# MathThyMod/GP_emu_UQSA

Hardware: AMD Instinct MI355X
Metric: log-marginal-likelihood evals/sec at n=16384 d=10 fp64; 1/2/4/8 GPU (higher is better)
Workload: dtype f64

## Files before the change

gp_emu_uqsa_amd/csrc/gpemu.hip:

```cpp
#include <hip/hip_runtime.h>

#include <algorithm>
#include <array>
#include <atomic>
#include <map>
#include <cmath>
#include <cstdio>
#include <cstdlib>
#include <cstring>
#include <limits>
#include <string>
#include <type_traits>
#include <utility>
#include <vector>

#include "../../include/gpemu.h"
#include "gpemu_kernels.hpp"
#include "gpemu_gemm_sched.hpp"
#include "gpemu_chol_sched.hpp"
#include "gpemu_objective.hpp"
#include "gpemu_chunk_pipe.hpp"
#include "gpemu_tiny.hpp"
#include "gpemu_snb.hpp"
#include "gpemu_ozaki.hpp"
#include "gpemu_pivchol.hpp"
#include "gpemu_imse.hpp"
#include "gpemu_postgrad.hpp"
#include "gpemu_postmean.hpp"
#include "gpemu_postmean_multi.hpp"
#include "gpemu_postgroup.hpp"
#include "gpemu_hm.hpp"
#include "gpemu_host_alloc.hpp"

using namespace gpe;

namespace {

thread_local std::string g_create_error;

constexpr int MAX_PROBS = 1 << 16;
constexpr int AUX_DESC_BASE = 1 << 15;
constexpr int ADHOC_DESC_BASE = MAX_PROBS - 64;

enum AdhocSlot {
  ADHOC_POST_V = ADHOC_DESC_BASE + 0,
  ADHOC_COV = ADHOC_DESC_BASE + 1,
  ADHOC_NOISE = ADHOC_DESC_BASE + 3,
  ADHOC_PIVCHOL = ADHOC_DESC_BASE + 4,
  ADHOC_POST_U = ADHOC_DESC_BASE + 5,
  ADHOC_IMSE = ADHOC_DESC_BASE + 7,
  ADHOC_TEST = ADHOC_DESC_BASE + 8,
  ADHOC_BENCH = ADHOC_DESC_BASE + 16,
};

constexpr int OZ_CHOL_MIN = 8192;
constexpr int OZ_CHOL_NEST_MIN = 12288;


struct Fact {
  long long n_pad = 0;
  int NB = 0;
  double* A = nullptr;
  double* B = nullptr;
  size_t cap = 0;
  double* logdet = nullptr;
  int* flags = nullptr;
  int* tflags = nullptr;
  bool aug = false;
  double* Faug = nullptr;
  double* part = nullptr;
  int* tcnt = nullptr;
  bool xdone[2] = {false, false};
  int xh = 0;
  int x11 = 0;
  bool t_ahead = false;
  void xclear(int h = 0) { xdone[0] = xdone[1] = t_ahead = false; x11 = 0; xh = h; }
  int desc_base = 0;
  Plan plan;
};

}

struct gpe_ctx {
  int device = 0;
  hipStream_t stream = nullptr;
  std::string err;

  long long n = 0, n_pad = 0;
  int d = 0, q = 0, NB = 0;
  bool has_r = false;

  double* dX = nullptr;
  double* dXw = nullptr;
  double* dF = nullptr;
  double* dr = nullptr;
  Fact tr;
  Fact aux;

  int* dinfo = nullptr;
  double* dinvdelta = nullptr;
  double* dZ = nullptr;
  double* dR2 = nullptr;
  double* dWa = nullptr;
  double* dskp = nullptr;
  size_t skp_cap = 0;
  double* dgpart = nullptr;
  double* dgram = nullptr;
  double* dT2 = nullptr;
  double* dcpart = nullptr;
  size_t cpart_cap = 0;
  size_t invd_cap = 0, csum_cap = 0, gram_cap = 0, t2_cap = 0;
  double* dcsum = nullptr;
  GemmProb* dprobs = nullptr;
  unsigned* dtiles = nullptr;
  size_t tiles_cap = 0;

  double* dW1 = nullptr;
  double* dW2 = nullptr;
  size_t w1_cap = 0, w2_cap = 0;
  double* dW3 = nullptr;
  size_t w3_cap = 0;
  double* dXs = nullptr;
  double* dXsw = nullptr;
  size_t xs_cap = 0, xsw_cap = 0;
  double* dsmall = nullptr;
  double* dtiny = nullptr;
  int tiny_ek = 0, tiny_eg = 0;
  bool tiny_dirty = true;
  double* dsnb = nullptr;
  long long snb_np = 0;
  int snb_hc = 0, snb_mf = 0;
  bool snb_dirty = true;
  double onel_tag = 0.0;
  int oz_on = 1, oz_nmod = OZ_MAXMOD;
  int oz_min_np = 6144;
  int oz_np2 = 0, oz_list_len = 0;
  long long oz_npad = 0;
  OzConst oz_c{};
  int8_t* dozp = nullptr;
  int8_t* dozr = nullptr;
  int* dozx = nullptr;
  unsigned* dozl = nullptr;
  double* dozt = nullptr;
  hipEvent_t ev_oz = nullptr;
  std::vector<OzTriPair> oz_tri;
  int oz_tri_min = 8192;
  double oz_lauum_ops = 0.0;
  int oz_chol = 1, oz_chol_min = OZ_CHOL_MIN;
  int tri_ahead_on = 1;
  hipEvent_t ev_l11 = nullptr, ev_schur = nullptr;
  OzTriPair oz_chol_q{};
  long long oz_chol_loff = 0;
  int oz_chol_llen = 0;
  double oz_chol_ops = 0.0;
  bool oz_chol_ready = false;
  int oz_nest = 1, oz_nest_min = OZ_CHOL_NEST_MIN;
  OzCholNest oz_nest_q{};
  long long oz_nest_loff = 0;
  int oz_nest_llen = 0;
  double oz_nest_ops = 0.0;
  bool oz_nest_ready = false;
  bool oz_l21_valid = false;
  std::vector<hipEvent_t> oev;
  size_t oev_used = 0;
  double oz_ms = 0.0, oz_launches = 0.0, oz_ops = 0.0, oz_flops64 = 0.0;
  int dbg_skip_wait = -1;
  size_t small_cap = 0;

  double* hpin = nullptr;
  size_t hpin_cap = 0;

  float* dX32 = nullptr;
  size_t x32_cap = 0;
  bool x32_valid = false;
  float* dK32 = nullptr;
  size_t k32_cap = 0;
  hipEvent_t ev_pipe[2] = {nullptr, nullptr};
  int8_t* dpxp = nullptr;
  int* dpxe = nullptr;
  int8_t* dpkp = nullptr;
  int* dpke = nullptr;
  int8_t* dpres = nullptr;
  unsigned* dpl = nullptr;
  size_t pxp_cap = 0, pxe_cap = 0, pkp_cap = 0, pke_cap = 0, pres_cap = 0, pl_cap = 0;
  int px_nmod = 0, pl_nti = 0, pl_ntj = 0, pl_len = 0;
  bool px_valid = false;

  double* dSU = nullptr;
  double* dSZ = nullptr;
  double* dSW = nullptr;
  double* dSpart = nullptr;
  double* dSout = nullptr;
  size_t su_cap = 0, sz_cap = 0, sw_cap = 0, spart_cap = 0, sout_cap = 0;

  double* dRn = nullptr;
  size_t rn_cap = 0;
  double* dVall = nullptr;
  double* dXall = nullptr;
  double* dTall = nullptr;
  size_t vall_cap = 0, xall_cap = 0, tall_cap = 0;
  double* dNU = nullptr;
  size_t nu_cap = 0;
  double* dPc = nullptr;
  double* dPcL = nullptr;
  size_t pc_cap = 0, pcl_cap = 0;
  double* dIm = nullptr;
  double* dImC = nullptr;
  size_t im_cap = 0, imc_cap = 0;
  double* dPg = nullptr;
  size_t pg_cap = 0;
  double* dPm = nullptr;
  size_t pm_cap = 0;
  long long mean_chunk = 65536;
  int mo_p = 0;
  double* dFm = nullptr;
  double* dZm = nullptr;
  double* dR2m = nullptr;
  double* dWm = nullptr;
  size_t fm_cap = 0, zm_cap = 0, r2m_cap = 0, wm_cap = 0;
  double* dPmm = nullptr;
  size_t pmm_cap = 0;
  double* dPgc = nullptr;
  size_t pgc_cap = 0;

// ... 517 lines not shown
  if (P <= SK_PMAX)
    hipLaunchKernelGGL(k_apply_small, g, dim3(256), 0, c->stream, Z, ldz, P, T, Pout, Y, ldy, nrows, abort_flag);
  else
    hipLaunchKernelGGL(k_apply_big, g, dim3(256), 0, c->stream, Z, ldz, P, T, Pout, Y, ldy, nrows, abort_flag);
  HIPCHK(c, hipGetLastError());
  return GPE_OK;
}

inline int gram_pairs(int P) {
  const int nch = (P + SK_PMAX - 1) / SK_PMAX;
  return nch * (nch + 1) / 2;
}

int gram(gpe_ctx* c, const double* Z, long long ldz, int P, int nrows, double* host_out) {
  const int nblk = (nrows + 255) / 256;
  const size_t need = (size_t)nblk * P * P;
  CHK(ensure_small(c, need + P * P));
  hipLaunchKernelGGL(k_gram, dim3(nblk, gram_pairs(P)), dim3(256), 0, c->stream, Z, ldz, P, nrows, c->dsmall,
                     c->dinfo);
  HIPCHK(c, hipGetLastError());
  hipLaunchKernelGGL(k_reduce_rows, dim3(P * P), dim3(256), 0, c->stream, c->dsmall, nblk, P * P,
                     c->dgram);
  HIPCHK(c, hipGetLastError());
  CHK(ensure_pinned(c, (size_t)P * P + 8));
  HIPCHK(c, hipMemcpyAsync(c->hpin, c->dgram, (size_t)P * P * sizeof(double), hipMemcpyDeviceToHost,
                           c->stream));
  HIPCHK(c, hipStreamSynchronize(c->stream));
  std::memcpy(host_out, c->hpin, (size_t)P * P * sizeof(double));
  return GPE_OK;
}

int gram_async(gpe_ctx* c, const double* Z, long long ldz, int P, int nrows) {
  const int nblk = (nrows + 255) / 256;
  const size_t need = (size_t)nblk * P * P;
  CHK(ensure_small(c, need + P * P));
  hipLaunchKernelGGL(k_gram, dim3(nblk, gram_pairs(P)), dim3(256), 0, c->stream, Z, ldz, P, nrows, c->dsmall,
                     c->dinfo);
  HIPCHK(c, hipGetLastError());
  hipLaunchKernelGGL(k_reduce_rows, dim3(P * P), dim3(256), 0, c->stream, c->dsmall, nblk, P * P,
                     c->dgram);
  HIPCHK(c, hipGetLastError());
  HIPCHK(c, hipMemcpyAsync(c->hpin, c->dgram, (size_t)P * P * sizeof(double), hipMemcpyDeviceToHost,
                           c->stream));
  return GPE_OK;
}

int read_info_logdet(gpe_ctx* c, const Fact& F, int* info, double* logdetA) {
  CHK(ensure_pinned(c, (size_t)F.NB + 8));
  HIPCHK(c, hipMemcpyAsync(c->hpin, F.logdet, F.NB * sizeof(double), hipMemcpyDeviceToHost, c->stream));
  HIPCHK(c, hipMemcpyAsync(c->hpin + F.NB, c->dinfo, sizeof(int), hipMemcpyDeviceToHost, c->stream));
  HIPCHK(c, hipStreamSynchronize(c->stream));
  std::memcpy(info, c->hpin + F.NB, sizeof(int));
  if (*info == GEMM_WAIT_TIMEOUT)
    return fail(c, GPE_ERR_HIP, "internal error: Cholesky panel wait timed out");
  double s = 0.0;
  for (int k = 0; k < F.NB; ++k) s += c->hpin[k];
  *logdetA = 2.0 * s;
  return GPE_OK;
}

int check_ready(gpe_ctx* c) {
  if (!c) return GPE_ERR_ARG;
  if (c->n <= 0) return fail(c, GPE_ERR_STATE, "gpe_set_data has not been called");
  HIPCHK(c, hipSetDevice(c->device));
  return GPE_OK;
}

void ev_rec(gpe_ctx* c, int i) {
  if (c->prof) hipEventRecord(c->ev[i], c->stream);
}

struct Cols {
  const double* F;
  int P;
  double* Z;
};
int z_from_factor(gpe_ctx* c, const Cols* cols = nullptr, bool cols_in_aug = false);
int trsv_lower(gpe_ctx* c, Fact& F, const double* R, long long ldr, int P, double* Y, long long ldy);

int factor_and_invert(gpe_ctx* c, int kernel, const double* delta, double nu, double s2,
                      double rscale, bool invert = true, bool objective = false, const Cols* cols = nullptr) {
  c->linv_valid = false;
  c->oz_l21_valid = false;
  HIPCHK(c, hipStreamSynchronize(c->stream2));
  HIPCHK(c, hipMemsetAsync(c->dinfo, 0, sizeof(int), c->stream));
  CHK(build_plan(c, c->tr));
  ev_rec(c, 0);
  CHK(scale_training(c, delta));
  CHK(kbuild(c, kernel, nu, s2, rscale));
  const int P = cols ? cols->P : c->q + 1;
  const bool aug = !invert && c->tr.plan.aug && P <= TILE;
  c->zaug_valid = aug && !cols;
  if (aug) {
    const long long tot = c->n_pad * TILE;
    hipLaunchKernelGGL(k_aug_init, dim3((unsigned)((tot + 255) / 256)), dim3(256), 0, c->stream,
                       cols ? cols->F : c->dF, c->n_pad, P, c->n_pad, c->tr.Faug);
    HIPCHK(c, hipGetLastError());
  }
  ev_rec(c, 1);
  CHK(build_plan(c, c->tr));
  CHK(potrf(c, c->tr, aug, objective && (invert || c->oz_chol >= 2), objective && invert,
            objective && (invert || c->oz_chol == 3)));
  if (kernel_fam(kernel) != FAM_GAUSS) {
    double coff, cdiag;
    kernel_consts(kernel, nu, true, &coff, &cdiag);
    const double floor_rel = 4.0 * (double)c->n_pad * std::numeric_limits<double>::epsilon();
    const double* r = (c->has_r && rscale != 0.0) ? c->dr : nullptr;
    hipLaunchKernelGGL(k_pivot_floor, dim3((unsigned)((c->n + 255) / 256)), dim3(256), 0, c->stream, c->tr.A,
                       c->n_pad, (int)c->n, floor_rel, s2 * cdiag, r, rscale, c->dinfo);
    HIPCHK(c, hipGetLastError());
  }
  ev_rec(c, 2);
  if (invert) {
    CHK(trtri(c, c->tr, true));
    c->linv_valid = true;
  }
  CHK(z_from_factor(c, cols, aug));
  ev_rec(c, 3);
  return GPE_OK;
}

int z_from_factor(gpe_ctx* c, const Cols* cols, bool cols_in_aug) {
  const int P = cols ? cols->P : c->q + 1;
  const double* F = cols ? cols->F : c->dF;
  double* Z = cols ? cols->Z : c->dZ;
  const long long np = c->n_pad;
  if (cols ? cols_in_aug : c->zaug_valid) {
    const long long tot = np * P;
    hipLaunchKernelGGL(k_aug_to_cols, dim3((unsigned)((tot + 255) / 256)), dim3(256), 0, c->stream,
                       c->tr.Faug, P, np, Z, np);
    HIPCHK(c, hipGetLastError());
    return GPE_OK;
  }
  if (c->linv_valid) return skinny(c, false, c->tr.B, np, c->NB, c->NB, true, F, np, P, Z, np);
  return trsv_lower(c, c->tr, F, np, P, Z, np);
}

int ensure_linv(gpe_ctx* c) {
  if (c->linv_valid) return GPE_OK;
  CHK(trtri(c, c->tr));
  c->linv_valid = true;
  c->x32_valid = false;
  c->px_valid = false;
  return GPE_OK;
}

int trsv_lower(gpe_ctx* c, Fact& F, const double* R, long long ldr, int P, double* Y, long long ldy) {
  CHK(ensure_xdiag(c, F));
  for (int c0 = 0; c0 < P; c0 += TS_PM) {
    const int pc = std::min(TS_PM, P - c0);
    HIPCHK(c, hipMemsetAsync(F.tflags, 0, 2 * sizeof(int), c->stream));
    hipLaunchKernelGGL(k_trsv_lower, dim3(F.NB), dim3(512), 0, c->stream, F.A, (long long)F.n_pad, F.B,
                       R + (long long)c0 * ldr, ldr, Y + (long long)c0 * ldy, ldy, pc, F.tflags, F.tflags + 1,
                       c->dinfo);
    HIPCHK(c, hipGetLastError());
  }
  return GPE_OK;
}

constexpr int OZ_MIN_NP = 6144, OZ_POST_MIN_NP = 4096, OZ_MAX_NP = 65536, OZ_POST_MAX_NP = 32768;
static_assert(OZ_MAX_NP % OZ_T == 0 && OZ_MAX_NP <= OZ_MAX_K && OZ_POST_MAX_NP <= OZ_MAX_K, "int8 sums too long");
bool oz_use(const gpe_ctx* c) { return c->oz_on && c->n_pad >= c->oz_min_np && c->n_pad <= OZ_MAX_NP; }

int oz_chol_split(const gpe_ctx* c, const Fact& F) {
  if (!c->oz_chol || !oz_use(c) || F.n_pad != c->n_pad || F.NB < 2) return 0;
  int h = 1;
  while (2 * h < F.NB) h *= 2;
  return (F.NB - h) * TILE >= c->oz_chol_min ? h : 0;
}

int oz_chol_nest_split(const gpe_ctx* c, const Fact& F, int h) {
  if (!c->oz_nest || h < 4 || (h / 2) % 2) return 0;
  return (F.NB - h / 2) * TILE >= c->oz_nest_min ? h / 2 : 0;
}

bool oz_tri_level(const gpe_ctx* c, const std::vector<std::array<int, 3>>& prs) {
  return oz_use(c) && !prs.empty() && (prs[0][1] - prs[0][0]) * TILE >= c->oz_tri_min;
}

int oz_prepare(gpe_ctx* c, Fact& F) {
  const int np2 = (int)(((c->n_pad + OZ_T - 1) / OZ_T) * OZ_T);
  if (c->n_pad == c->oz_npad && np2 == c->oz_np2 && c->oz_c.nmod == c->oz_nmod) return GPE_OK;
  c->oz_np2 = 0;
  c->oz_npad = 0;
  c->oz_chol_ready = false;
  c->oz_nest_ready = false;
  c->oz_l21_valid = false;
  CHK(build_plan(c, F));
  const int N = c->oz_nmod;
  size_t planes = (size_t)oz_plane_bytes(np2) * N;
  size_t resid = (size_t)oz_lauum_shape(np2).res_bytes() * N;
  size_t scratch = 0, nex = (size_t)np2;
  std::vector<unsigned> all = oz_lauum_shape(np2).list();
  c->oz_list_len = (int)all.size();
  c->oz_lauum_ops = oz_lauum_shape(np2).ops(N);
  c->oz_tri.clear();
  for (const auto& prs : F.plan.tri_pairs) {
    if (!oz_tri_level(c, prs)) continue;
    for (const auto& pr : prs) {
      const OzTriPair q = oz_tri_pair_plan(pr[0], pr[1], pr[2], N, all);
      planes = std::max(planes, q.planes_bytes(N));
      resid = std::max(resid, q.resid_bytes(N));
      scratch = std::max(scratch, (size_t)q.Pa * q.Pb);
      nex = std::max(nex, (size_t)(q.Pa + q.Pb));
      c->oz_tri.push_back(q);
    }
  }
  if (const int hs = (&F == &c->tr) ? F.plan.split_h : 0) {
    const OzTriPair* have = nullptr;
    for (const OzTriPair& q : c->oz_tri)
      if (q.t0 == 0 && q.h == hs && q.t1 == F.NB) have = &q;
    const OzTriPair q = have ? *have : oz_tri_pair_plan(0, hs, F.NB, N, all);
    const std::vector<unsigned> ls = q.shape_schur().list();
    c->oz_chol_q = q;
    c->oz_chol_loff = (long long)all.size();
    c->oz_chol_llen = (int)ls.size();
    all.insert(all.end(), ls.begin(), ls.end());
    c->oz_chol_ops = q.shape_schur().ops(N);
    planes = std::max(planes, (size_t)N * q.Pb * q.Pa);
    resid = std::max(resid, (size_t)q.shape_schur().res_bytes() * N);
    nex = std::max(nex, (size_t)q.Pb);
    c->oz_chol_ready = true;
    if (const int qs = F.plan.split_q) {
      const OzCholNest nq = oz_chol_nest_plan(qs, hs, F.NB);
      const std::vector<unsigned> ln = nq.shape().list();
      c->oz_nest_q = nq;
      c->oz_nest_loff = (long long)all.size();
      c->oz_nest_llen = (int)ln.size();
      all.insert(all.end(), ln.begin(), ln.end());
      c->oz_nest_ops = nq.shape().ops(N);
      planes = std::max(planes, nq.planes_bytes(N));
      resid = std::max(resid, nq.resid_bytes(N));
      nex = std::max(nex, (size_t)nq.Pb);
      c->oz_nest_ready = true;
    }
  }
  CHK(dalloc(c, &c->dozp, planes));
  CHK(dalloc(c, &c->dozr, resid));
  CHK(dalloc(c, &c->dozx, nex));
  CHK(dalloc(c, &c->dozt, scratch));
  CHK(dalloc(c, &c->dozl, all.size()));
  HIPCHK(c, hipMemcpy(c->dozl, all.data(), all.size() * sizeof(unsigned), hipMemcpyHostToDevice));
  c->oz_c = oz_consts(N, np2);
  c->oz_np2 = np2;
  c->oz_npad = c->n_pad;
  return GPE_OK;
}

int oz_gemm_crt(gpe_ctx* c, const OzConst& k, const OzProduct& p, double ops, double flops64,
                hipStream_t st = nullptr) {
  if (!st) st = c->stream;
  hipEvent_t e0 = nullptr, e1 = nullptr;
  if (c->prof) {
    while (c->oev_used + 2 > c->oev.size()) {
      hipEvent_t e;
      HIPCHK(c, hipEventCreate(&e));
      c->oev.push_back(e);
    }
    e0 = c->oev[c->oev_used];
    e1 = c->oev[c->oev_used + 1];
  }
  HIPCHK(c, oz_product_launch(st, k, p, e0, e1));
  if (c->prof) {
    c->oev_used += 2;
    c->oz_launches += 1.0;
    c->oz_ops += ops;
    c->oz_flops64 += flops64;
  }
  return GPE_OK;
}

int chol_schur(gpe_ctx* c, Fact& F, hipStream_t st, bool with_aug, int at) {
  const Plan& pl = F.plan;
  if (at != pl.split_h) {
    const OzCholNest& n = c->oz_nest_q;
    if (!c->oz_nest_ready || at != pl.split_q || n.q != at || n.h != pl.split_h)
      return fail(c, GPE_ERR_STATE, "internal error: nested split Cholesky without an int8 plan");
    if (with_aug) CHK(launch_gemm_range(c, pl.launches[pl.aug_q], st));
    const long long ld = F.n_pad;
    c->oz_l21_valid = false;
    oz_operand(st, c->oz_c, n.src(F.A + (long long)n.q * TILE, ld), n.Pb, n.K, c->dozx, c->dozp);
    HIPCHK(c, hipGetLastError());
    const OzShape s = n.shape();
    const OzOpnd l{c->dozp, (long long)n.Pb * n.K, n.K, 0};
    return oz_gemm_crt(c, c->oz_c,
                       OzProduct{s, l, l, c->dozl + c->oz_nest_loff, c->oz_nest_llen, c->dozr, s.res_bytes(),
                                 OzOut{c->dozx, c->dozx, F.A + (long long)n.q * TILE * (ld + 1), ld, n.Rb, n.cols, 1, -1.0, 1}},
                       c->oz_nest_ops, (double)n.cols * (2.0 * n.Rb - n.cols) * n.K, st);
  }
  const OzTriPair& q = c->oz_chol_q;
  if (!c->oz_chol_ready || q.h != pl.split_h) return fail(c, GPE_ERR_STATE, "internal error: split Cholesky without an int8 plan");
  if (with_aug) CHK(launch_gemm_range(c, pl.launches[pl.aug_mid], st));
  const long long ld = F.n_pad;
  oz_operand(st, c->oz_c, q.l21(F.A + (long long)q.h * TILE, ld), q.Pb, q.Pa, c->dozx, c->dozp);
  HIPCHK(c, hipGetLastError());
  const OzShape s = q.shape_schur();
  const OzOpnd l21{c->dozp, (long long)q.Pb * q.Pa, q.Pa, 0};
  CHK(oz_gemm_crt(c, c->oz_c,
                  OzProduct{s, l21, l21, c->dozl + c->oz_chol_loff, c->oz_chol_llen, c->dozr, s.res_bytes(),
                            OzOut{c->dozx, c->dozx, F.A + (long long)q.h * TILE * (ld + 1), ld, q.Rb, q.Rb, 1, -1.0, 1}},
                  c->oz_chol_ops, (double)q.Rb * q.Rb * q.Ra, st));
  c->oz_l21_valid = true;
  return GPE_OK;
}

int lauum_ozaki(gpe_ctx* c, Fact& F) {
  CHK(oz_prepare(c, F));
  const int np = (int)F.n_pad, np2 = c->oz_np2;
  c->oz_l21_valid = false;
  oz_operand_packed(c->stream, c->oz_c, F.B, (long long)F.n_pad, np, np2, c->dozx, c->dozp);
  const OzShape s = oz_lauum_shape(np2);
  const OzOpnd x{c->dozp, oz_plane_bytes(np2), 0, np2};
  return oz_gemm_crt(c, c->oz_c,
                     OzProduct{s, x, x, c->dozl, c->oz_list_len, c->dozr, s.res_bytes(),
                               OzOut{c->dozx, c->dozx, F.A, (long long)F.n_pad, np, np, 1, 1.0}},
                     c->oz_lauum_ops, (double)np * np * np / 3.0);
}

const OzTriPair* oz_pair(const gpe_ctx* c, int t0, int h, int t1) {
  for (const OzTriPair& q : c->oz_tri)
    if (q.t0 == t0 && q.h == h && q.t1 == t1) return &q;
  return nullptr;
}

int oz_l21(gpe_ctx* c, Fact& F, const OzTriPair& q, hipStream_t st) {
  c->oz_l21_valid = false;
  oz_operand(st, c->oz_c, q.l21(F.A + (long long)q.h * TILE + (long long)q.t0 * TILE * F.n_pad, F.n_pad), q.Pb, q.Pa,
             c->dozx, c->dozp);
  HIPCHK(c, hipGetLastError());
  return GPE_OK;
}

int oz_l21_ahead(gpe_ctx* c, Fact& F, int t0, int h, int t1) {
  CHK(oz_prepare(c, F));
  const OzTriPair* q = oz_pair(c, t0, h, t1);
  if (!q) return fail(c, GPE_ERR_STATE, "internal error: TRTRI pair without an int8 plan");
  if (!c->ev_oz) HIPCHK(c, hipEventCreateWithFlags(&c->ev_oz, hipEventDisableTiming));
  HIPCHK(c, hipEventRecord(c->ev_fork, c->stream));
  HIPCHK(c, hipStreamWaitEvent(c->stream2, c->ev_fork, 0));
  CHK(oz_l21(c, F, *q, c->stream2));
  HIPCHK(c, hipEventRecord(c->ev_oz, c->stream2));
  return GPE_OK;
}

int trtri_pair_ozaki(gpe_ctx* c, Fact& F, int t0, int h, int t1, int l21, int part) {
  CHK(oz_prepare(c, F));
  const OzTriPair* qp = oz_pair(c, t0, h, t1);
  if (!qp) return fail(c, GPE_ERR_STATE, "internal error: TRTRI pair without an int8 plan");
  const long long ld = F.n_pad;
  auto tile = [&](double* M, int i, int j) { return M + (long long)i * TILE + (long long)j * TILE * ld; };
  if (l21 == 1) HIPCHK(c, hipStreamWaitEvent(c->stream, c->ev_oz, 0));
  if (part != 1) c->oz_l21_valid = false;
  int rc = GPE_OK;
  oz_tri_pair_launches(c->stream, c->oz_c, *qp, c->dozl, tile(F.A, h, t0), tile(F.B, t0, t0), tile(F.B, h, h),
                       tile(F.B, h, t0), ld, c->dozt, c->dozp, c->dozr, c->dozx, l21 != 0,
                       [&](const OzProduct& p, double ops, double fl) {
                         if (rc == GPE_OK) rc = oz_gemm_crt(c, c->oz_c, p, ops, fl);
                       }, part);
  CHK(rc);
  HIPCHK(c, hipGetLastError());
  return GPE_OK;
}

}

bool create_priority_stream(hipStream_t* st) {
  int lo = 0, hi = 0;
  if (hipDeviceGetStreamPriorityRange(&lo, &hi) != hipSuccess) return false;
  return hipStreamCreateWithPriority(st, hipStreamNonBlocking, hi) == hipSuccess;
}

extern "C" {

#ifdef GEMM_TRACE
int gpe_debug_trace(uint64_t* out, int32_t n) {
  if (n > 8 * 4096) n = 8 * 4096;
  return hipMemcpyFromSymbol(out, HIP_SYMBOL(gemm_trace), (size_t)n * 8) == hipSuccess ? 0 : -2;
}
#endif

#ifdef GEMM_TTRACE
int gpe_debug_ttrace(uint64_t* out, int32_t n) {
  if (n > 8 * (int)GEMM_TTRACE_MAX) n = 8 * (int)GEMM_TTRACE_MAX;
  return hipMemcpyFromSymbol(out, HIP_SYMBOL(gemm_ttrace), (size_t)n * 8) == hipSuccess ? 0 : -2;
}
int gpe_debug_ttrace_count(int32_t reset) {
  unsigned n = 0;
  if (hipMemcpyFromSymbol(&n, HIP_SYMBOL(gemm_ttrace_n), sizeof(n)) != hipSuccess) return -2;
  if (reset) {
    const unsigned z = 0;
    if (hipMemcpyToSymbol(HIP_SYMBOL(gemm_ttrace_n), &z, sizeof(z)) != hipSuccess) return -2;
    void* tt = nullptr;
    if (hipGetSymbolAddress(&tt, HIP_SYMBOL(gemm_ttrace)) != hipSuccess ||
        hipMemset(tt, 0, sizeof(unsigned long long) * 8 * GEMM_TTRACE_MAX) != hipSuccess) return -2;
  }
  return (int)n;
}
#endif

int gpe_abi_version(void) { return GPE_ABI_VERSION; }

#ifndef GPE_SOURCE_HASH
#define GPE_SOURCE_HASH "unknown"
#endif
const char* gpe_build_id(void) { return GPE_SOURCE_HASH; }

int gpe_device_count(void) {
  int n = 0;
  if (hipGetDeviceCount(&n) != hipSuccess) return 0;
  return n;
}

int gpe_device_synchronize(int32_t device) {
  if (hipSetDevice(device) != hipSuccess) return GPE_ERR_HIP;
  return hipDeviceSynchronize() == hipSuccess ? GPE_OK : GPE_ERR_HIP;
}

gpe_ctx* gpe_create(int32_t device) {
  int ndev = 0;
  hipError_t e = hipGetDeviceCount(&ndev);
  if (e != hipSuccess || ndev <= 0) {
    g_create_error = std::string("no HIP device available: ") + hipGetErrorString(e);
    return nullptr;
  }
  if (device < 0 || device >= ndev) {
    g_create_error = "device index out of range";
    return nullptr;
  }
  gpe_ctx* c = new gpe_ctx();
  c->device = device;
  c->aux.desc_base = AUX_DESC_BASE;
  {
    const char* ea = std::getenv("GPEMU_AUG");
    c->tr.aug = !(ea && std::string(ea) == "0");
  }
  {
    const char* e2 = std::getenv("GPEMU_POTRF");
    if (e2) {
      const std::string m(e2);
      c->sched.group = m == "group" || m == "auto";
      c->potrf_mode = m == "group" ? 1 : (m == "auto" ? 0 : 2);
    }
    if (const char* eg = std::getenv("GPEMU_GROUP_P0")) c->sched.grp_p0 = std::max(1, std::atoi(eg));
    if (const char* eg = std::getenv("GPEMU_GROUP_STRIDE")) c->sched.grp_stride = std::max(0, std::atoi(eg));
    if (const char* ep = std::getenv("GPEMU_CHOL_PRIO")) c->chol_prio = std::atoi(ep) != 0;
    if (const char* et = std::getenv("GPEMU_TINY")) c->tiny = std::atoi(et) != 0;
    if (const char* ed = std::getenv("GPEMU_DEBUG_SKIP_WAIT")) c->dbg_skip_wait = std::atoi(ed);
    if (const char* em = std::getenv("GPEMU_MEAN_CHUNK")) c->mean_chunk = std::max(1, std::atoi(em) / 128) * 128LL;
    if (const char* eo = std::getenv("GPEMU_OZAKI")) c->oz_on = std::atoi(eo) != 0;
    if (const char* en = std::getenv("GPEMU_OZAKI_MIN_NP")) c->oz_min_np = std::max(512, std::atoi(en));
    if (const char* em = std::getenv("GPEMU_OZAKI_MODULI")) c->oz_nmod = std::max(8, std::min(OZ_MAXMOD, std::atoi(em)));
    if (const char* et = std::getenv("GPEMU_OZAKI_TRI_MIN")) c->oz_tri_min = std::max(512, std::atoi(et));
    if (const char* ec = std::getenv("GPEMU_OZAKI_CHOL")) c->oz_chol = std::max(0, std::min(3, std::atoi(ec)));
    if (const char* ec = std::getenv("GPEMU_OZAKI_CHOL_MIN")) c->oz_chol_min = std::max(256, std::atoi(ec));
    if (const char* ec = std::getenv("GPEMU_OZAKI_CHOL_NEST")) c->oz_nest = std::atoi(ec) != 0;
    if (const char* ec = std::getenv("GPEMU_OZAKI_CHOL_NEST_MIN")) c->oz_nest_min = std::max(256, std::atoi(ec));
    if (const char* ea = std::getenv("GPEMU_TRTRI_AHEAD")) c->tri_ahead_on = std::atoi(ea) != 0;
    if (const char* es = std::getenv("GPEMU_POTRF_SB")) {
      c->sched.sb = std::max(1, std::min(8, std::atoi(es)));
      if (const char* colon = std::strchr(es, ':')) c->sched.sb_min = std::max(0, std::atoi(colon + 1));
    }
    if (const char* e3 = std::getenv("GPEMU_POTRF_W")) {
      c->sched.groups.clear();
      std::string spec(e3);
      size_t pos = 0;
      while (pos < spec.size()) {
        size_t end = spec.find(',', pos);
        if (end == std::string::npos) end = spec.size();
        const std::string item = spec.substr(pos, end - pos);
        const size_t colon = item.find(':');
        const int w = std::atoi(item.substr(0, colon).c_str());
        const int lim = colon == std::string::npos ? 0 : std::atoi(item.substr(colon + 1).c_str());
        if (w >= 1 && w <= 8) c->sched.groups.push_back({w, lim});
        pos = end + 1;
      }
    }
  }
  if (hipSetDevice(device) != hipSuccess || hipStreamCreateWithFlags(&c->stream, hipStreamNonBlocking) != hipSuccess ||
      !create_priority_stream(&c->stream2) ||
      hipEventCreateWithFlags(&c->ev_fork, hipEventDisableTiming) != hipSuccess ||
      hipEventCreateWithFlags(&c->ev_join, hipEventDisableTiming) != hipSuccess ||
      hipEventCreateWithFlags(&c->ev_l11, hipEventDisableTiming) != hipSuccess ||
      hipEventCreateWithFlags(&c->ev_schur, hipEventDisableTiming) != hipSuccess ||
      hipEventCreateWithFlags(&c->ev_host, hipEventDisableTiming) != hipSuccess) {
    g_create_error = "failed to initialise device/stream";
    delete c;
    return nullptr;
  }
  bool ok = dalloc(c, &c->dinfo, 12) == GPE_OK && dalloc(c, &c->dprobs, MAX_PROBS) == GPE_OK &&
            ensure_shape_bufs(c, GPE_MAX_DIMS, GPE_MAX_COLS) == GPE_OK;
  for (int i = 0; i < 16 && ok; ++i) ok = hipEventCreate(&c->ev[i]) == hipSuccess;
  if (ok) {
    const int gl = G_LDS_DOUBLES * (int)sizeof(double);
    ok = hipFuncSetAttribute((const void*)k_gemm<false, false, false, true>, hipFuncAttributeMaxDynamicSharedMemorySize, gl) == hipSuccess &&
         hipFuncSetAttribute((const void*)k_gemm<true, false, false, true>, hipFuncAttributeMaxDynamicSharedMemorySize, gl) == hipSuccess &&
         hipFuncSetAttribute((const void*)k_gemm<true, true, false, true>, hipFuncAttributeMaxDynamicSharedMemorySize, gl) == hipSuccess &&
         hipFuncSetAttribute((const void*)k_gemm<false, true, false, true>, hipFuncAttributeMaxDynamicSharedMemorySize, gl) == hipSuccess &&
         hipFuncSetAttribute((const void*)k_gemm<false, false, true, true>, hipFuncAttributeMaxDynamicSharedMemorySize, gl) == hipSuccess &&
         hipFuncSetAttribute((const void*)k_gemm<false, false>, hipFuncAttributeMaxDynamicSharedMemorySize, gl) == hipSuccess &&
         hipFuncSetAttribute((const void*)k_gemm<true, false>, hipFuncAttributeMaxDynamicSharedMemorySize, gl) == hipSuccess &&
         hipFuncSetAttribute((const void*)k_gemm<true, true>, hipFuncAttributeMaxDynamicSharedMemorySize, gl) == hipSuccess &&
         hipFuncSetAttribute((const void*)k_gemm<false, true>, hipFuncAttributeMaxDynamicSharedMemorySize, gl) == hipSuccess &&
         hipFuncSetAttribute((const void*)k_gemm<false, false, true>, hipFuncAttributeMaxDynamicSharedMemorySize, gl) == hipSuccess &&
         hipFuncSetAttribute((const void*)k_xasm, hipFuncAttributeMaxDynamicSharedMemorySize,
                             (int)(DB_LDS_DOUBLES * sizeof(double))) == hipSuccess;
    const int tl = (G_LDS_LAUNCH_DOUBLES + 2 * TILE * TINY_ZP) * (int)sizeof(double);
    const RegWidths w;
    ok = ok && onel_lds_attr<FAM_GAUSS>(w, tl, SNB_LDS_DOUBLES * 8) && onel_lds_attr<FAM_MATERN32>(w, tl, SNB_LDS_DOUBLES * 8) &&
         onel_lds_attr<FAM_MATERN52>(w, tl, SNB_LDS_DOUBLES * 8);
    if (!ok) c->err = "hipFuncSetAttribute(max dynamic LDS) failed";
  }
  if (!ok) {
    g_create_error = c->err;
    gpe_destroy(c);
    return nullptr;
  }
  return c;
}

void gpe_destroy(gpe_ctx* c) {
  if (!c) return;
  (void)hipSetDevice(c->device);
  if (c->stream) hipStreamSynchronize(c->stream);
  double* bufs[] = {c->dSU, c->dSZ, c->dSW, c->dSpart, c->dSout,
                    c->dX, c->dXw, c->dF, c->dr, c->tr.A, c->tr.B, c->tr.logdet, c->aux.A, c->aux.B,
                    c->aux.logdet, c->dinvdelta, c->dZ,
                    c->dR2, c->dWa, c->dskp, c->dgpart, c->dgram, c->dT2, c->dcpart, c->dcsum,
                    c->dW1, c->dW2, c->dW3, c->dXs, c->dXsw, c->dsmall, c->dtiny, c->dsnb, c->dRn, c->dNU,
                    c->dVall, c->dXall, c->dTall, c->dPc, c->dPcL, c->dIm, c->dImC, c->dPg, c->dPm, c->dPgc,
                    c->dFm, c->dZm, c->dR2m, c->dWm, c->dPmm};
  for (double* b : bufs)
    if (b) hipFree(b);
  if (c->dinfo) hipFree(c->dinfo);
  if (c->dX32) hipFree(c->dX32);
  if (c->dK32) hipFree(c->dK32);
  for (void* b : {(void*)c->dpxp, (void*)c->dpxe, (void*)c->dpkp, (void*)c->dpke, (void*)c->dpres, (void*)c->dpl})
    if (b) hipFree(b);
  if (c->tr.flags) hipFree(c->tr.flags);
  if (c->aux.flags) hipFree(c->aux.flags);
  for (Fact* F : {&c->tr, &c->aux}) {
    if (F->part) hipFree(F->part);
    if (F->tcnt) hipFree(F->tcnt);
  }
  if (c->tr.tflags) hipFree(c->tr.tflags);
  if (c->dozp) hipFree(c->dozp);
  if (c->dozr) hipFree(c->dozr);
  if (c->dozx) hipFree(c->dozx);
  if (c->dozl) hipFree(c->dozl);
  if (c->dozt) hipFree(c->dozt);
  if (c->ev_oz) hipEventDestroy(c->ev_oz);
  for (hipEvent_t e : c->oev) hipEventDestroy(e);
  if (c->tr.Faug) hipFree(c->tr.Faug);
  if (c->aux.tflags) hipFree(c->aux.tflags);
  if (c->dprobs) hipFree(c->dprobs);
  if (c->dtiles) hipFree(c->dtiles);
  if (c->hpin) hipHostFree(c->hpin);
  for (auto& e : c->ev)
    if (e) hipEventDestroy(e);
  for (auto& e : c->gev) (void)hipEventDestroy(e);
  if (c->ev_fork) (void)hipEventDestroy(c->ev_fork);
  for (hipEvent_t e : c->ev_pipe)
    if (e) (void)hipEventDestroy(e);
  if (c->ev_join) (void)hipEventDestroy(c->ev_join);
  if (c->ev_l11) (void)hipEventDestroy(c->ev_l11);
  if (c->ev_schur) (void)hipEventDestroy(c->ev_schur);
  if (c->ev_host) (void)hipEventDestroy(c->ev_host);
  if (c->stream2) {
    (void)hipStreamSynchronize(c->stream2);
    (void)hipStreamDestroy(c->stream2);
  }
  if (c->stream) (void)hipStreamDestroy(c->stream);
  delete c;
}

const char* gpe_last_error(const gpe_ctx* c) {
  if (!c) return g_create_error.c_str();
  return c->err.c_str();
}

int gpe_set_data(gpe_ctx* c, int64_t n, int32_t d, int32_t q, const double* X, const double* f,
                 const double* H, const double* r) {
  if (!c) return GPE_ERR_ARG;
  if (n <= 0 || d <= 0 || q <= 0 || !X || !f || !H) return fail(c, GPE_ERR_ARG, "bad data arguments");
  if (n > (1LL << 20)) return fail(c, GPE_ERR_UNSUPPORTED, "n too large");
  HIPCHK(c, hipSetDevice(c->device));
  HIPCHK(c, hipStreamSynchronize(c->stream));
  CHK(ensure_shape_bufs(c, d, q + 1));
  const long long n_pad = ((n + TILE - 1) / TILE) * TILE;
  const bool resize = (n_pad != c->n_pad) || (d != c->d) || (q != c->q);
  c->n = n; c->d = d; c->q = q; c->n_pad = n_pad; c->NB = (int)(n_pad / TILE);
  c->mo_p = 0;
  c->factor_valid = false;
  c->ainv_valid = false;
  c->x32_valid = false;
  c->px_valid = false;
  c->zaug_valid = false;
  c->linv_valid = false;
  c->oz_l21_valid = false;
  if (resize) {
    CHK(ensure_fact(c, c->tr, n_pad));
    CHK(dalloc(c, &c->dX, (size_t)n_pad * d));
    CHK(dalloc(c, &c->dXw, (size_t)n_pad * d));
    CHK(dalloc(c, &c->dF, (size_t)n_pad * (q + 1)));
    CHK(dalloc(c, &c->dr, (size_t)n_pad));
    const size_t cols = (size_t)std::max(SK_PMAX, q + 1);
    CHK(dalloc(c, &c->dZ, (size_t)n_pad * cols));
    CHK(dalloc(c, &c->dR2, (size_t)n_pad * cols));
    CHK(dalloc(c, &c->dWa, (size_t)n_pad * cols));
    const size_t cp = (size_t)c->NB * (c->NB + 1) / 2 * (d + 3) * 4;
    CHK(dalloc(c, &c->dcpart, cp));
    c->cpart_cap = cp;
  }
  const size_t nx = (size_t)n_pad * d, nf = (size_t)n_pad * (q + 1);
  CHK(ensure_pinned(c, std::max(nx, nf) + n_pad));
  std::memset(c->hpin, 0, nx * sizeof(double));
  std::memcpy(c->hpin, X, (size_t)n * d * sizeof(double));
  HIPCHK(c, hipMemcpy(c->dX, c->hpin, nx * sizeof(double), hipMemcpyHostToDevice));
  std::memset(c->hpin, 0, nf * sizeof(double));
  for (long long i = 0; i < n; ++i) {
    c->hpin[i] = f[i];
    for (int p = 0; p < q; ++p) c->hpin[i + (long long)(p + 1) * n_pad] = H[i * q + p];
  }
  HIPCHK(c, hipMemcpy(c->dF, c->hpin, nf * sizeof(double), hipMemcpyHostToDevice));
  c->has_r = (r != nullptr);
  std::memset(c->hpin, 0, n_pad * sizeof(double));
  if (r) std::memcpy(c->hpin, r, (size_t)n * sizeof(double));
  HIPCHK(c, hipMemcpy(c->dr, c->hpin, n_pad * sizeof(double), hipMemcpyHostToDevice));
  return GPE_OK;
}

int gpe_set_profiling(gpe_ctx* c, int32_t on) {
  if (!c) return GPE_ERR_ARG;
  c->prof = on != 0;
  return GPE_OK;
}

int gpe_phase_times(gpe_ctx* c, double* ms_out, int32_t n) {
  if (!c || !ms_out) return GPE_ERR_ARG;
  for (int i = 0; i < n && i < 8; ++i) ms_out[i] = c->phase_ms[i];
  return GPE_OK;
}

int gpe_ozaki_stats(gpe_ctx* c, double* ms_out, double* launches_out, double* int8_ops_out, double* fp64_flops_out) {
  if (!c) return GPE_ERR_ARG;
  if (ms_out) *ms_out = c->oz_ms;
  if (launches_out) *launches_out = c->oz_launches;
  if (int8_ops_out) *int8_ops_out = c->oz_ops;
  if (fp64_flops_out) *fp64_flops_out = c->oz_flops64;
  return GPE_OK;
}

int gpe_gemm_stats(gpe_ctx* c, double* ms_out, double* launches_out, double* flops_out) {
  if (!c) return GPE_ERR_ARG;
  if (ms_out) *ms_out = c->gemm_ms;
  if (launches_out) *launches_out = c->gemm_launches;
  if (flops_out) *flops_out = c->gemm_flops;
  return GPE_OK;
}

}

namespace {

template <class Args>
int onel_prologue(gpe_ctx* c, const ObjArgs& o, int kernel, const double* hp, bool want_grad, size_t pinned, Args& a) {
  const int d = c->d;
  const int bad = inv_length_scales(hp, d, a.invd);
  if (bad >= 0) return fail(c, GPE_NOT_PD, bad_length_scale(bad));
  for (int k = d; k < TINY_DM; ++k) a.invd[k] = 0.0;
  c->linv_valid = false;
  c->zaug_valid = false;
  c->tr.xclear();
  HIPCHK(c, hipStreamSynchronize(c->stream2));
  CHK(ensure_pinned(c, pinned));
  a.X = c->dX; a.F = c->dF; a.xw = c->dXw; a.small = c->hpin;
  a.r = (c->has_r && o.rscale != 0.0) ? c->dr : nullptr;
  a.rdiag = (o.gp4ml && !kernel_alt(kernel) && c->has_r) ? c->dr : nullptr;
  a.n = (int)c->n; a.d = d; a.P = c->q + 1; a.want_grad = want_grad ? 1 : 0; a.mucm = o.gp4ml ? 0 : 1;
  a.s2 = o.s2; a.rscale = o.rscale;
  a.dbg_skip = c->dbg_skip_wait;
  a.tag = ++c->onel_tag;
  kernel_consts(kernel, o.nu, true, &a.coff, &a.cdiag);
  a.floor_rel = 4.0 * (double)c->n_pad * std::numeric_limits<double>::epsilon();
  return GPE_OK;
}

int onel_epilogue(gpe_ctx* c, const ObjArgs& o, int kernel, int n_hp, bool want_grad, const OneLaunchResult& r,
                  bool std_r, double* llh_out, double* grad_out, double* sigma2_out) {
  HIPCHK(c, hipGetLastError());
  HIPCHK(c, hipStreamSynchronize(c->stream));
  CHK(r.status(&c->err));
  const SmallAlgebra sa = small_from_gram(std::vector<double>(r.h, r.h + (size_t)r.P * r.P), r.P);
  if (!sa.ok) return fail(c, GPE_NOT_PD, Q_NOT_PD);
  const ObjValue v = objective_value(sa, r.logdetA(), (double)c->n, c->q, o.gp4ml, o.s2);
  *llh_out = v.llh;
  if (sigma2_out) *sigma2_out = v.sig2;
  if (want_grad) {
    if (r.q_refused()) return fail(c, GPE_NOT_PD, Q_NOT_PD);
    double red[TINY_DM + 3];
    CHK(r.sums(red, &c->err));
    objective_grad(red, r.d, kernel, o.nu, o.fitnug, o.gp4ml, v.gscale, o.s2, n_hp, grad_out, std_r);
  }
  if (c->prof) {
    ev_rec(c, 7);
    HIPCHK(c, hipStreamSynchronize(c->stream));
    float ms = 0.f;
    (void)hipEventElapsedTime(&ms, c->ev[0], c->ev[7]);
    for (int i = 0; i < 8; ++i) c->phase_ms[i] = 0.0;
    c->phase_ms[6] = ms;
  }
  return GPE_OK;
}

int tiny_objective(gpe_ctx* c, const ObjArgs& o, int kernel, const double* hp, int n_hp, bool want_grad,
                   double* llh_out, double* grad_out, double* sigma2_out) {
  const int d = c->d, P = c->q + 1;
  TinyArgs a;
  CHK(onel_prologue(c, o, kernel, hp, want_grad, (size_t)P * P + 2 * d + 64 + TINY_NH * 64, a));
  constexpr size_t tiny_doubles = 36 * DB_BS + TILE * 32;
  if (!c->dtiny) CHK(dalloc(c, &c->dtiny, tiny_doubles));
  if (c->tiny_dirty || c->tiny_ek > (1 << 26)) {
    HIPCHK(c, hipMemsetAsync(c->dinfo + 1, 0, (TINY_SYNC_INTS + 1) * sizeof(int), c->stream));
    c->tiny_ek = c->tiny_eg = 0;
    c->tiny_dirty = false;
  }
  ev_rec(c, 0);
  a.L = c->tr.A; a.Xo = c->tr.B; a.Z = c->dZ; a.abort_flag = c->dinfo + 1 + TINY_SYNC_INTS;
  a.K = c->tr.A; a.Xp = c->dtiny; a.Wg = c->dtiny + 36 * DB_BS; a.sync = c->dinfo + 1;
  a.ek = ++c->tiny_ek;
  a.eg = want_grad ? ++c->tiny_eg : c->tiny_eg;
  const size_t lds = (G_LDS_LAUNCH_DOUBLES + 2 * TILE * TINY_ZP) * sizeof(double);
  c->hpin[P * P + 1] = -2.0;
  c->tiny_dirty = true;
  with_fam(kernel_fam(kernel), [&](auto F) { launch_tiny_fam<decltype(F)::value>(d, lds, c->stream, a); });
  CHK(onel_epilogue(c, o, kernel, n_hp, want_grad, OneLaunchResult{c->hpin, P, d, 1, TINY_NH, a.tag, "k_tiny"},
                    a.rdiag != nullptr, llh_out, grad_out, sigma2_out));
  c->tiny_dirty = false;
  return GPE_OK;
}

int snb_objective(gpe_ctx* c, const ObjArgs& o, int kernel, const double* hp, int n_hp, bool want_grad,
                  double* llh_out, double* grad_out, double* sigma2_out) {
  const int d = c->d, P = c->q + 1, NB = c->NB;
  const long long np = c->n_pad;
  SnbArgs a;
  CHK(onel_prologue(c, o, kernel, hp, want_grad, (size_t)P * P + NB + 2 * d + 64 + SNB_NH * 64, a));
  if (c->snb_np != np) {
    c->snb_np = 0;
    CHK(dalloc(c, &c->dsnb, (size_t)np * np + 3 * 32 * (size_t)np + TINY_DM * TINY_ZP + TILE * TILE));
    c->snb_np = np;
  }
  if (c->snb_dirty || c->snb_hc > (1 << 24)) {
    HIPCHK(c, hipMemsetAsync(c->dinfo + 8, 0, (SNB_SYNC_INTS + 1) * sizeof(int), c->stream));
    c->snb_hc = c->snb_mf = 0;
    c->snb_dirty = false;
  }
  ev_rec(c, 0);
  a.A = c->tr.A; a.Lb = c->tr.B; a.Xt = c->dsnb;
  a.Zt = a.Xt + np * np; a.Zo = a.Zt + 32 * np; a.Wg = a.Zo + 32 * np; a.T2g = a.Wg + 32 * np;
  a.Xscr = a.T2g + TINY_DM * TINY_ZP;
  a.sync = c->dinfo + 8; a.abort_flag = c->dinfo + 8 + SNB_SYNC_INTS;
  a.np = (int)np; a.NB = NB;
  a.hcb = c->snb_hc; a.mfb = c->snb_mf;
  const size_t lds = SNB_LDS_DOUBLES * sizeof(double);
  c->hpin[P * P + NB] = -2.0;
  c->snb_dirty = true;
  with_fam(kernel_fam(kernel), [&](auto F) { launch_snb_fam<decltype(F)::value>(d, lds, c->stream, a); });
  CHK(onel_epilogue(c, o, kernel, n_hp, want_grad, OneLaunchResult{c->hpin, P, d, NB, SNB_NH, a.tag, "k_snb"},
                    a.rdiag != nullptr, llh_out, grad_out, sigma2_out));
  c->snb_hc += want_grad ? 4 * NB - 1 : 2 * NB;
  c->snb_mf += NB + (want_grad ? 1 : 0);
  c->snb_dirty = false;
  return GPE_OK;
}

int objective_phase_times(gpe_ctx* c) {
  if (!c->prof) return GPE_OK;
  HIPCHK(c, hipStreamSynchronize(c->stream));
  float ms;
  const int pairs[7][2] = {{0, 1}, {1, 2}, {2, 3}, {4, 5}, {3, 4}, {5, 7}, {0, 7}};
  for (int i = 0; i < 7; ++i) {
    ms = 0.f;
    (void)hipEventElapsedTime(&ms, c->ev[pairs[i][0]], c->ev[pairs[i][1]]);
    c->phase_ms[i] = ms;
  }
  double g = 0.0;
  for (size_t i = 0; i + 1 < c->gev_used; i += 2) {
    ms = 0.f;
    (void)hipEventElapsedTime(&ms, c->gev[i], c->gev[i + 1]);
    g += ms;
  }
  c->gemm_ms = g;
  g = 0.0;
  for (size_t i = 0; i + 1 < c->oev_used; i += 2) {
    ms = 0.f;
    (void)hipEventElapsedTime(&ms, c->oev[i], c->oev[i + 1]);
    g += ms;
  }
  c->oz_ms = g;
  return GPE_OK;
}

}

extern "C" {

int gpe_objective(gpe_ctx* c, int32_t variant, int32_t kernel, const double* hp, int32_t n_hp,
                  double nu_fixed, int32_t want_grad, double* llh_out, double* grad_out,
                  double* sigma2_out) {
  CHK(check_ready(c));
  const InflightGuard inflight(c->device);
  if (!hp || !llh_out) return fail(c, GPE_ERR_ARG, "null output");
  const int d = c->d, q = c->q;
  ObjArgs o;
  CHK(objective_args(variant, kernel, d, hp, n_hp, nu_fixed, &o, &c->err));
  if (!kernel_ok(kernel)) return fail(c, GPE_ERR_ARG, "bad kernel");
  if (want_grad && !grad_out) return fail(c, GPE_ERR_ARG, "grad_out is NULL");
  c->factor_valid = false;
  c->ainv_valid = false;
  c->x32_valid = false;
  c->px_valid = false;
  if (c->prof) {
    c->gev_used = 0;
    c->gemm_launches = c->gemm_flops = c->gemm_ms = 0.0;
    c->oev_used = 0;
    c->oz_ms = c->oz_launches = c->oz_ops = c->oz_flops64 = 0.0;
  }
  const bool one_launch = c->tiny;
  if (one_launch && c->NB == 1 && d <= TINY_DM && q + 1 <= TINY_DM)
    return tiny_objective(c, o, kernel, hp, n_hp, want_grad != 0, llh_out, grad_out, sigma2_out);
  if (one_launch && c->NB >= 2 && c->NB <= SNB_MAXNB && d <= TINY_DM && q + 1 <= TINY_DM)
    return snb_objective(c, o, kernel, hp, n_hp, want_grad != 0, llh_out, grad_out, sigma2_out);

  CHK(factor_and_invert(c, kernel, hp, o.nu, o.s2, o.rscale, want_grad != 0, true));
  const int P = q + 1;
  const long long np = c->n_pad;
  const int NBt = c->tr.NB;
  CHK(ensure_pinned(c, (size_t)P * P + NBt + 64));
  CHK(gram_async(c, c->dZ, np, P, (int)np));
  HIPCHK(c, hipMemcpyAsync(c->hpin + P * P, c->tr.logdet, NBt * sizeof(double), hipMemcpyDeviceToHost, c->stream));
  HIPCHK(c, hipMemcpyAsync(c->hpin + P * P + NBt, c->dinfo, sizeof(int), hipMemcpyDeviceToHost, c->stream));
  HIPCHK(c, hipEventRecord(c->ev_host, c->stream));
  ev_rec(c, 4);
  if (want_grad) CHK(oz_use(c) ? lauum_ozaki(c, c->tr) : lauum(c, c->tr));
  ev_rec(c, 5);
  HIPCHK(c, hipEventSynchronize(c->ev_host));
  std::vector<double> G(c->hpin, c->hpin + (size_t)P * P);
  int info = 0;
  std::memcpy(&info, c->hpin + P * P + NBt, sizeof(int));
  if (info == GEMM_WAIT_TIMEOUT) return fail(c, GPE_ERR_HIP, "internal error: Cholesky panel wait timed out");
  double logdetA = 0.0;
  for (int k = 0; k < NBt; ++k) logdetA += c->hpin[P * P + k];
  logdetA *= 2.0;
  if (info != 0) return fail(c, GPE_NOT_PD, not_pd_pivot(info));
  const SmallAlgebra sa = small_from_gram(G, P);
  if (!sa.ok) return fail(c, GPE_NOT_PD, Q_NOT_PD);
  const ObjValue v = objective_value(sa, logdetA, (double)c->n, q, o.gp4ml, o.s2);
  *llh_out = v.llh;
  if (sigma2_out) *sigma2_out = v.sig2;
  if (!want_grad) {
    ev_rec(c, 6);
    ev_rec(c, 7);
    goto done;
  }
  {
    CHK(ensure_pinned(c, (size_t)P * P + 8));
    const std::vector<double> T2 = small_t2(sa, q, v.cfac);
    std::memcpy(c->hpin, T2.data(), T2.size() * sizeof(double));
    HIPCHK(c, hipMemcpyAsync(c->dT2, c->hpin, T2.size() * sizeof(double), hipMemcpyHostToDevice, c->stream));
    CHK(apply_small(c, c->dZ, np, P, c->dT2, P, c->dR2, np, (int)np, c->dinfo));
    CHK(skinny(c, true, c->tr.B, np, c->NB, c->NB, true, c->dR2, np, P, c->dWa, np));
    ev_rec(c, 6);
    const double* rdiag = (o.gp4ml && !kernel_alt(kernel) && c->has_r) ? c->dr : nullptr;
    const int nblk = c->NB * (c->NB + 1) / 2;
    int cs = 1;
    if (!(d > 32 || P > 33))
      while (cs < 4 && nblk * cs * 2 <= 512) cs *= 2;
    const dim3 gc(nblk * cs);
    with_fam(kernel_fam(kernel), [&](auto F) { launch_contract<decltype(F)::value>(c, d, P, gc, nblk, rdiag, cs, c->dWa); });
    HIPCHK(c, hipGetLastError());
    hipLaunchKernelGGL(k_reduce_rows, dim3(d + 3), dim3(256), 0, c->stream, c->dcpart, nblk * cs, d + 3, c->dcsum);
    HIPCHK(c, hipGetLastError());
    ev_rec(c, 7);
    HIPCHK(c, hipMemcpyAsync(c->hpin, c->dcsum, (d + 3) * sizeof(double), hipMemcpyDeviceToHost, c->stream));
    HIPCHK(c, hipStreamSynchronize(c->stream));
    objective_grad(c->hpin, d, kernel, o.nu, o.fitnug, o.gp4ml, v.gscale, o.s2, n_hp, grad_out, rdiag != nullptr);
  }
done:
  return objective_phase_times(c);
}

int gpe_set_outputs(gpe_ctx* c, int32_t p, const double* F) {
  CHK(check_ready(c));
  const int q = c->q;
  const long long n = c->n, np = c->n_pad;
  if (p < 1 || p > PMM_MAXP || !F) return fail(c, GPE_ERR_ARG, "bad outputs (1 <= p <= 64, F not NULL)");
  if (n < (long long)p + q + 3) return fail(c, GPE_ERR_ARG, "p outputs need n >= p + q + 3 training points");
  HIPCHK(c, hipStreamSynchronize(c->stream));
  c->mo_p = 0;
  const int P = p + q;
  const size_t cols = (size_t)np * std::max(SK_PMAX, P);
  CHK(ensure_shape_bufs(c, c->d, P));
  CHK(grow_buf(c, &c->dFm, &c->fm_cap, (size_t)np * P));
  CHK(grow_buf(c, &c->dZm, &c->zm_cap, cols));
  CHK(grow_buf(c, &c->dR2m, &c->r2m_cap, cols));
  CHK(grow_buf(c, &c->dWm, &c->wm_cap, cols));
  const size_t nf = (size_t)np * p;
  CHK(ensure_pinned(c, nf));
  std::memset(c->hpin, 0, nf * sizeof(double));
  for (long long i = 0; i < n; ++i)
    for (int a = 0; a < p; ++a) c->hpin[i + (long long)a * np] = F[i * p + a];
  HIPCHK(c, hipMemcpy(c->dFm, c->hpin, nf * sizeof(double), hipMemcpyHostToDevice));
  HIPCHK(c, hipMemcpy(c->dFm + nf, c->dF + np, (size_t)np * q * sizeof(double), hipMemcpyDeviceToDevice));
  c->mo_p = p;
  return GPE_OK;
}

int gpe_objective_multi(gpe_ctx* c, int32_t kernel, const double* hp, int32_t n_hp, double nu_fixed,
                        int32_t want_grad, double* llh_out, double* grad_out, double* Sigma_out, double* B_out) {
  CHK(check_ready(c));
  if (!c->mo_p) return fail(c, GPE_ERR_STATE, "gpe_set_outputs has not been called for this data");
  const InflightGuard inflight(c->device);
  if (!hp || !llh_out || !Sigma_out) return fail(c, GPE_ERR_ARG, "null output");
  const int d = c->d, q = c->q, p = c->mo_p, P = p + q;
  ObjArgs o;
  CHK(objective_args(GPE_MUCM, kernel, d, hp, n_hp, nu_fixed, &o, &c->err));
  if (!kernel_ok(kernel)) return fail(c, GPE_ERR_ARG, "bad kernel");
  if (want_grad && !grad_out) return fail(c, GPE_ERR_ARG, "grad_out is NULL");
  c->factor_valid = false;
  c->ainv_valid = false;
  c->x32_valid = false;
  c->px_valid = false;
  if (c->prof) {
    c->gev_used = 0;
    c->gemm_launches = c->gemm_flops = c->gemm_ms = 0.0;
    c->oev_used = 0;
    c->oz_ms = c->oz_launches = c->oz_ops = c->oz_flops64 = 0.0;
  }
  const Cols cols{c->dFm, P, c->dZm};
  CHK(factor_and_invert(c, kernel, hp, o.nu, o.s2, o.rscale, want_grad != 0, true, &cols));
  const long long np = c->n_pad;
  const int NBt = c->tr.NB;
  CHK(ensure_pinned(c, (size_t)P * P + NBt + 64));
  CHK(gram_async(c, c->dZm, np, P, (int)np));
  HIPCHK(c, hipMemcpyAsync(c->hpin + P * P, c->tr.logdet, NBt * sizeof(double), hipMemcpyDeviceToHost, c->stream));
  HIPCHK(c, hipMemcpyAsync(c->hpin + P * P + NBt, c->dinfo, sizeof(int), hipMemcpyDeviceToHost, c->stream));
  HIPCHK(c, hipEventRecord(c->ev_host, c->stream));
  ev_rec(c, 4);
  if (want_grad) CHK(oz_use(c) ? lauum_ozaki(c, c->tr) : lauum(c, c->tr));
  ev_rec(c, 5);
  HIPCHK(c, hipEventSynchronize(c->ev_host));
  const std::vector<double> G(c->hpin, c->hpin + (size_t)P * P);
  int info = 0;
  std::memcpy(&info, c->hpin + P * P + NBt, sizeof(int));
  if (info == GEMM_WAIT_TIMEOUT) return fail(c, GPE_ERR_HIP, "internal error: Cholesky panel wait timed out");
  double logdetA = 0.0;
  for (int k = 0; k < NBt; ++k) logdetA += c->hpin[P * P + k];
  logdetA *= 2.0;
  if (info != 0) return fail(c, GPE_NOT_PD, not_pd_pivot(info));
  const SmallMulti sm = small_multi_from_gram(G, p, q);
  if (!sm.ok()) return fail(c, GPE_NOT_PD, sm.refused == 1 ? Q_NOT_PD : S_NOT_PD);
  const ObjValueMulti v = objective_value_multi(sm, logdetA, (double)c->n);
  *llh_out = v.llh;
  std::memcpy(Sigma_out, v.Sigma.data(), v.Sigma.size() * sizeof(double));
  if (B_out) std::memcpy(B_out, sm.B.data(), sm.B.size() * sizeof(double));
  if (!want_grad) {
    ev_rec(c, 6);
    ev_rec(c, 7);
    return objective_phase_times(c);
  }
  CHK(ensure_pinned(c, (size_t)P * P + 8));
  const std::vector<double> T2 = small_multi_t2(sm, v.cfac);
  std::memcpy(c->hpin, T2.data(), T2.size() * sizeof(double));
  HIPCHK(c, hipMemcpyAsync(c->dT2, c->hpin, T2.size() * sizeof(double), hipMemcpyHostToDevice, c->stream));
  CHK(apply_small(c, c->dZm, np, P, c->dT2, P, c->dR2m, np, (int)np, c->dinfo));
  CHK(skinny(c, true, c->tr.B, np, c->NB, c->NB, true, c->dR2m, np, P, c->dWm, np));
  ev_rec(c, 6);
  const int nblk = c->NB * (c->NB + 1) / 2;
  int cs = 1;
  if (!(d > 32 || P > 33))
    while (cs < 4 && nblk * cs * 2 <= 512) cs *= 2;
  const dim3 gc(nblk * cs);
  with_fam(kernel_fam(kernel),
           [&](auto F) { launch_contract<decltype(F)::value>(c, d, P, gc, nblk, nullptr, cs, c->dWm); });
  HIPCHK(c, hipGetLastError());
  hipLaunchKernelGGL(k_reduce_rows, dim3(d + 3), dim3(256), 0, c->stream, c->dcpart, nblk * cs, d + 3, c->dcsum);
  HIPCHK(c, hipGetLastError());
  ev_rec(c, 7);
  HIPCHK(c, hipMemcpyAsync(c->hpin, c->dcsum, (d + 3) * sizeof(double), hipMemcpyDeviceToHost, c->stream));
  HIPCHK(c, hipStreamSynchronize(c->stream));
  objective_grad(c->hpin, d, kernel, o.nu, o.fitnug, false, v.gscale, 1.0, n_hp, grad_out, false);
  return objective_phase_times(c);
}

int gpe_factor(gpe_ctx* c, int32_t kernel, const double* delta, double nu, double s2, double r_scale) {
  CHK(check_ready(c));
  if (!delta) return fail(c, GPE_ERR_ARG, "null delta");
  if (!kernel_ok(kernel)) return fail(c, GPE_ERR_ARG, "bad kernel");
  c->factor_valid = false;
  c->ainv_valid = false;
  c->x32_valid = false;
  c->px_valid = false;
  CHK(factor_and_invert(c, kernel, delta, nu, s2, r_scale, false, c->oz_chol == 3));
  int info = 0;
  double logdet = 0.0;
  CHK(read_info_logdet(c, c->tr, &info, &logdet));
  if (info != 0) return fail(c, GPE_NOT_PD, not_pd_pivot(info));
  c->factor_valid = true;
  c->x32_valid = false;
  c->px_valid = false;
  c->f_kernel = kernel;
  c->f_delta.assign(delta, delta + c->d);
  c->f_nu = nu;
  c->f_rscale = r_scale;
  return GPE_OK;
}

static int posterior_nmod(int np2, bool f32) {
  if (!f32) return OZ_MAXMOD;
  int bits = 24;
// ... 1509 lines not shown
  HIPCHK(c, hipMemcpy(F.A, c->hpin, tot * sizeof(double), hipMemcpyHostToDevice));
  HIPCHK(c, hipMemsetAsync(c->dinfo, 0, sizeof(int), c->stream));
  CHK(potrf(c, F));
  int info = 0;
  double logdet = 0.0;
  CHK(read_info_logdet(c, F, &info, &logdet));
  if (info != 0) return fail(c, GPE_NOT_PD, not_pd_pivot(info));
  if (logdet_out) *logdet_out = logdet;
  auto fetch_lower = [&](const double* dsrc, double* out, bool full_sym) -> int {
    HIPCHK(c, hipMemcpy(c->hpin, dsrc, tot * sizeof(double), hipMemcpyDeviceToHost));
    for (long long i = 0; i < m; ++i)
      for (long long j = 0; j < m; ++j) {
        double v;
        if (j <= i) v = c->hpin[i + j * mp];
        else v = full_sym ? c->hpin[j + i * mp] : 0.0;
        out[i * m + j] = v;
      }
    return GPE_OK;
  };
  if (L_out) CHK(fetch_lower(F.A, L_out, false));
  if (Linv_out || Ainv_out) {
    CHK(trtri(c, F));
    if (Linv_out) {
      HIPCHK(c, hipStreamSynchronize(c->stream));
      CHK(fetch_lower(F.B, Linv_out, false));
    }
    if (Ainv_out) {
      CHK(lauum(c, F));
      HIPCHK(c, hipStreamSynchronize(c->stream));
      CHK(fetch_lower(F.A, Ainv_out, true));
    }
  }
  HIPCHK(c, hipStreamSynchronize(c->stream));
  return GPE_OK;
}

int gpe_test_gemm(gpe_ctx* c, int32_t trans_a, int32_t trans_b, int64_t M, int64_t N, int64_t K,
                  const double* A, const double* B, double* C, double alpha, double beta) {
  if (!c) return GPE_ERR_ARG;
  if (M <= 0 || N <= 0 || K <= 0 || M % TILE || N % TILE || K % GK || !A || !B || !C)
    return fail(c, GPE_ERR_ARG, "gpe_test_gemm: M, N must be multiples of 128 and K of 16");
  HIPCHK(c, hipSetDevice(c->device));
  double *da = nullptr, *db = nullptr, *dc = nullptr;
  int rc = dalloc(c, &da, (size_t)M * K);
  if (rc == GPE_OK) rc = dalloc(c, &db, (size_t)K * N);
  if (rc == GPE_OK) rc = dalloc(c, &dc, (size_t)M * N);
  if (rc == GPE_OK) {
    std::vector<double> ha((size_t)M * K), hb((size_t)K * N), hc((size_t)M * N);
    long long lda, ldb;
    if (trans_a) { for (long long m = 0; m < M; ++m) for (long long k = 0; k < K; ++k) ha[k + m * K] = A[m * K + k]; lda = K; }
    else { for (long long m = 0; m < M; ++m) for (long long k = 0; k < K; ++k) ha[m + k * M] = A[m * K + k]; lda = M; }
    if (trans_b) { for (long long k = 0; k < K; ++k) for (long long n = 0; n < N; ++n) hb[k + n * K] = B[k * N + n]; ldb = K; }
    else { for (long long k = 0; k < K; ++k) for (long long n = 0; n < N; ++n) hb[n + k * N] = B[k * N + n]; ldb = N; }
    for (long long m = 0; m < M; ++m) for (long long n = 0; n < N; ++n) hc[m + n * M] = C[m * N + n];
    copy_checked(c, rc, da, ha.data(), ha.size() * sizeof(double), hipMemcpyHostToDevice);
    copy_checked(c, rc, db, hb.data(), hb.size() * sizeof(double), hipMemcpyHostToDevice);
    copy_checked(c, rc, dc, hc.data(), hc.size() * sizeof(double), hipMemcpyHostToDevice);
    const GemmProb p = mkprob(da, lda, db, ldb, dc, M, (int)(M / TILE), (int)(N / TILE), (int)K, 0, alpha, beta);
    const GemmKind kind = gemm_kind(trans_a != 0, trans_b != 0);
    GemmLaunch L{};
    if (rc == GPE_OK) rc = adhoc_gemm(c, ADHOC_TEST, {{kind, p}}, &L, true);
    HIPCHK(c, hipMemsetAsync(c->dinfo, 0, sizeof(int), c->stream));
    if (rc == GPE_OK) rc = launch_gemm_range(c, L);
    if (rc == GPE_OK) {
      hipError_t e = hipStreamSynchronize(c->stream);
      if (e != hipSuccess) rc = fail(c, GPE_ERR_HIP, hipGetErrorString(e));
    }
    if (rc == GPE_OK) {
      copy_checked(c, rc, hc.data(), dc, hc.size() * sizeof(double), hipMemcpyDeviceToHost);
      for (long long m = 0; m < M; ++m) for (long long n = 0; n < N; ++n) C[m * N + n] = hc[m + n * M];
    }
  }
  if (da) (void)hipFree(da);
  if (db) (void)hipFree(db);
  if (dc) (void)hipFree(dc);
  return rc;
}

struct OzTestBufs {
  double *sa = nullptr, *sb = nullptr, *C = nullptr;
  int *exa = nullptr, *exb = nullptr;
  int8_t *pa = nullptr, *pb = nullptr, *res = nullptr;
  unsigned* list = nullptr;
  ~OzTestBufs() {
    for (void* p : {(void*)sa, (void*)sb, (void*)C, (void*)exa, (void*)exb, (void*)pa, (void*)pb, (void*)res, (void*)list})
      if (p) (void)hipFree(p);
  }
};

static long long oz_test_extent(const gpe_oz_operand& o, int R, int Kv) {
  if (!o.src || o.len <= 0 || o.offset < 0 || o.ld < 1 || R < 1 || Kv < 1) return 0;
  const long long ext = o.trans ? (long long)(Kv - 1) * o.ld + R : (long long)(R - 1) * o.ld + Kv;
  return ext <= o.len - o.offset ? ext : 0;
}

static int oz_test_operand(gpe_ctx* c, const gpe_oz_operand& o, const OzConst& k, int P, int Kp, double** dsrc, int** dex,
                           int8_t** dpl) {
  CHK(dalloc(c, dsrc, (size_t)o.len));
  CHK(dalloc(c, dex, (size_t)P));
  CHK(dalloc(c, dpl, (size_t)k.nmod * P * Kp));
  HIPCHK(c, hipMemcpy(*dsrc, o.src, (size_t)o.len * sizeof(double), hipMemcpyHostToDevice));
  oz_operand(c->stream, k, OzSrc{*dsrc + o.offset, (long long)o.ld, o.R, o.Kv, o.mask, o.trans != 0}, P, Kp, *dex, *dpl);
  HIPCHK(c, hipGetLastError());
  return GPE_OK;
}

static int oz_test_product(gpe_ctx* c, const gpe_oz_operand& a, const gpe_oz_operand* b, gpe_oz_params p, double* C,
                           int32_t* exa_out, int32_t* exb_out, int8_t* res_out) {
  const auto bad = [&](const char* what) { return fail(c, GPE_ERR_ARG, std::string("gpe_test_oz_product: ") + what); };
  if (p.nmod < 6 || p.nmod > OZ_MAXMOD) return bad("nmod outside [6, 16]");
  if (res_out && (p.res_mod < 0 || p.res_mod >= p.nmod)) return bad("res_mod is not a modulus number");
  if (a.R < 1 || a.R > (1 << 20)) return bad("bad operand rows");
  const int Pa = (a.R + OZ_T - 1) / OZ_T * OZ_T;
  int Pb = Pa;
  if (p.packed) {
    if (a.R % TILE || (a.offset & 1) || (a.ld & 1) || a.ld < a.R || !oz_test_extent(a, 1, 1) ||
        (long long)(a.R - 1) * a.ld + a.R > a.len - a.offset)
      return bad("packed: X is R x R, R a multiple of 128, ld >= R and offset even, inside src");
    p.K = Pa; p.kbeg = 1; p.kend = 0; p.kdiv = 1; p.ti0 = 0; p.tri = 1; p.lower128 = 1;
    p.rows = p.cols = a.R;
    b = nullptr;
  } else {
    if (p.K < OZ_SK || p.K % OZ_SK || p.K > OZ_MAX_K) return bad("K is not a multiple of 64 in [64, 2^17 - 128]");
    if (a.mask < 0 || a.mask > 2 || a.Kv > p.K || !oz_test_extent(a, a.R, a.Kv)) return bad("operand A outside its source");
    if (b) {
      if (b->R < 1 || b->R > (1 << 20) || b->mask < 0 || b->mask > 2 || b->Kv > p.K || !oz_test_extent(*b, b->R, b->Kv))
        return bad("operand B outside its source");
      Pb = (b->R + OZ_T - 1) / OZ_T * OZ_T;
    }
    if (p.kbeg < 0 || p.kbeg > 3 || p.kend < 0 || p.kend > 1 || p.kdiv < 1) return bad("bad kbeg / kend / kdiv");
    if (p.ti0 < 0 || p.ti0 >= Pa / OZ_T) return bad("ti0 past the last tile row");
    if (p.tri && Pb < Pa && p.ti0 != 0) return bad("tri: B has fewer tile rows than A and ti0 > 0");
  }
  if (p.rows <= OZ_T * p.ti0 || p.rows > Pa || p.cols < 1 || p.cols > Pb) return bad("rows / cols outside the product");
  if (!C || p.ldc < 1 || p.c_len < 1 || (long long)(p.rows - 1 - OZ_T * p.ti0) + (long long)(p.cols - 1) * p.ldc >= p.c_len)
    return bad("C too small for rows x cols at ldc");
  const int K = p.K, ti0 = p.ti0, nti = Pa / OZ_T - ti0, ntj = Pb / OZ_T;
  const OzConst k = oz_consts(p.nmod, K);
  const OzShape s{nti, p.tri ? (Pb < Pa ? ntj : 0) : ntj, ti0, p.tri ? 1 : 0, K, p.kbeg, p.kend, p.kdiv};
  OzTestBufs d;
  hipStream_t st = c->stream;
  OzOpnd oa, ob;
  if (p.packed) {
    CHK(dalloc(c, &d.sa, (size_t)a.len));
    CHK(dalloc(c, &d.exa, (size_t)Pa));
    CHK(dalloc(c, &d.pa, (size_t)k.nmod * oz_plane_bytes(Pa)));
    HIPCHK(c, hipMemcpy(d.sa, a.src, (size_t)a.len * sizeof(double), hipMemcpyHostToDevice));
    oz_operand_packed(st, k, d.sa + a.offset, (long long)a.ld, a.R, Pa, d.exa, d.pa);
    HIPCHK(c, hipGetLastError());
    oa = ob = OzOpnd{d.pa, oz_plane_bytes(Pa), 0, Pa};
  } else {
    CHK(oz_test_operand(c, a, k, Pa, K, &d.sa, &d.exa, &d.pa));
    oa = ob = OzOpnd{d.pa, (long long)Pa * K, K, 0};
    if (b) {
      CHK(oz_test_operand(c, *b, k, Pb, K, &d.sb, &d.exb, &d.pb));
      ob = OzOpnd{d.pb, (long long)Pb * K, K, 0};
    }
  }
  const std::vector<unsigned> list = s.list();
  const long long rb = s.res_bytes();
  CHK(dalloc(c, &d.list, list.size()));
  CHK(dalloc(c, &d.res, (size_t)k.nmod * rb));
  CHK(dalloc(c, &d.C, (size_t)p.c_len));
  HIPCHK(c, hipMemcpy(d.list, list.data(), list.size() * sizeof(unsigned), hipMemcpyHostToDevice));
  HIPCHK(c, hipMemcpy(d.C, C, (size_t)p.c_len * sizeof(double), hipMemcpyHostToDevice));
  HIPCHK(c, hipMemsetAsync(d.res, 0, (size_t)k.nmod * rb, st));
  const OzOut out{d.exa, b ? d.exb : d.exa, d.C, (long long)p.ldc, p.rows, p.cols, p.lower128 ? 1 : 0, p.alpha, p.acc ? 1 : 0};
  CHK(oz_gemm_crt(c, k, OzProduct{s, oa, ob, d.list, (int)list.size(), d.res, rb, out}, 0.0, 0.0));
  HIPCHK(c, hipStreamSynchronize(st));
  HIPCHK(c, hipMemcpy(C, d.C, (size_t)p.c_len * sizeof(double), hipMemcpyDeviceToHost));
  if (exa_out) HIPCHK(c, hipMemcpy(exa_out, d.exa, (size_t)Pa * sizeof(int), hipMemcpyDeviceToHost));
  if (exb_out) HIPCHK(c, hipMemcpy(exb_out, b ? d.exb : d.exa, (size_t)Pb * sizeof(int), hipMemcpyDeviceToHost));
  if (res_out) {
    std::vector<int8_t> h((size_t)rb);
    HIPCHK(c, hipMemcpy(h.data(), d.res + (long long)p.res_mod * rb, (size_t)rb, hipMemcpyDeviceToHost));
    std::memset(res_out, 0, (size_t)nti * OZ_T * Pb);
    for (const unsigned ent : list) {
      if (ent == 0xffffffffu) continue;
      const int ti = (int)(ent >> 16), tj = (int)(ent & 0xffffu);
      const int8_t* t = h.data() + s.res_tile(ti, tj) * (OZ_T * OZ_T);
      for (int u = 0; u < OZ_T * OZ_T / 16; ++u) {
        const int wave = u >> 10, blk = (u >> 6) & 15, lane = u & 63;
        const long long gm = OZ_T * (ti - ti0) + (wave >> 1) * 128 + 32 * (blk >> 2) + (lane & 31);
        const long long gn0 = OZ_T * tj + (wave & 1) * 128 + 32 * (blk & 3) + 4 * (lane >> 5);
        for (int q = 0; q < 16; ++q) res_out[gm * Pb + gn0 + (q & 3) + 8 * (q >> 2)] = t[(long long)u * 16 + q];
      }
    }
  }
  return GPE_OK;
}

int gpe_test_oz_product(gpe_ctx* c, const gpe_oz_operand* a, const gpe_oz_operand* b, const gpe_oz_params* p, double* C,
                        int32_t* exa_out, int32_t* exb_out, int8_t* res_out) {
  if (!c) return GPE_ERR_ARG;
  if (!a || !p) return fail(c, GPE_ERR_ARG, "gpe_test_oz_product: NULL operand or parameters");
  HIPCHK(c, hipSetDevice(c->device));
  const bool prof = c->prof;
  c->prof = false;
  const int rc = oz_test_product(c, *a, b, *p, C, exa_out, exb_out, res_out);
  c->prof = prof;
  return rc;
}

static int oz_test_planes(gpe_ctx* c, const gpe_oz_operand& a, int packed, int K, int nmod, int32_t* ex_out, int8_t* planes_out) {
  const auto bad = [&](const char* what) { return fail(c, GPE_ERR_ARG, std::string("gpe_test_oz_planes: ") + what); };
  if (nmod < 6 || nmod > OZ_MAXMOD) return bad("nmod outside [6, 16]");
  if (a.R < 1 || a.R > (1 << 20)) return bad("bad operand rows");
  if (!ex_out || !planes_out) return bad("NULL output");
  const int P = (a.R + OZ_T - 1) / OZ_T * OZ_T;
  if (packed) {
    if (a.R % TILE || (a.offset & 1) || (a.ld & 1) || a.ld < a.R || !oz_test_extent(a, 1, 1) ||
        (long long)(a.R - 1) * a.ld + a.R > a.len - a.offset)
      return bad("packed: X is R x R, R a multiple of 128, ld >= R and offset even, inside src");
    K = P;
  } else {
    if (K < OZ_SK || K % OZ_SK || K > OZ_MAX_K) return bad("K is not a multiple of 64 in [64, 2^17 - 128]");
    if (a.mask < 0 || a.mask > 2 || a.Kv > K || !oz_test_extent(a, a.R, a.Kv)) return bad("operand outside its source");
  }
  const OzConst k = oz_consts(nmod, K);
  OzTestBufs d;
  if (packed) {
    const long long pb = oz_plane_bytes(P);
    CHK(dalloc(c, &d.sa, (size_t)a.len));
    CHK(dalloc(c, &d.exa, (size_t)P));
    CHK(dalloc(c, &d.pa, (size_t)nmod * pb));
    HIPCHK(c, hipMemcpy(d.sa, a.src, (size_t)a.len * sizeof(double), hipMemcpyHostToDevice));
    HIPCHK(c, hipMemsetAsync(d.pa, 0x55, (size_t)nmod * pb, c->stream));
    oz_operand_packed(c->stream, k, d.sa + a.offset, (long long)a.ld, a.R, P, d.exa, d.pa);
    HIPCHK(c, hipGetLastError());
    HIPCHK(c, hipStreamSynchronize(c->stream));
    std::vector<int8_t> h((size_t)nmod * pb);
    HIPCHK(c, hipMemcpy(h.data(), d.pa, h.size(), hipMemcpyDeviceToHost));
    std::memset(planes_out, 0, (size_t)nmod * P * P);
    for (int l = 0; l < nmod; ++l)
      for (int j = 0; j < P; ++j) {
        const int r0 = j / OZ_T * OZ_T;
        std::memcpy(planes_out + ((size_t)l * P + j) * P + r0,
                    h.data() + (size_t)l * pb + oz_panel_off(j / OZ_T, P) + (long long)(j - r0) * (P - r0), (size_t)(P - r0));
      }
  } else {
    CHK(dalloc(c, &d.sa, (size_t)a.len));
    CHK(dalloc(c, &d.exa, (size_t)P));
    CHK(dalloc(c, &d.pa, (size_t)nmod * P * K));
    HIPCHK(c, hipMemcpy(d.sa, a.src, (size_t)a.len * sizeof(double), hipMemcpyHostToDevice));
    HIPCHK(c, hipMemsetAsync(d.pa, 0x55, (size_t)nmod * P * K, c->stream));
    oz_operand(c->stream, k, OzSrc{d.sa + a.offset, (long long)a.ld, a.R, a.Kv, a.mask, a.trans != 0}, P, K, d.exa, d.pa);
    HIPCHK(c, hipGetLastError());
    HIPCHK(c, hipStreamSynchronize(c->stream));
    HIPCHK(c, hipMemcpy(planes_out, d.pa, (size_t)nmod * P * K, hipMemcpyDeviceToHost));
  }
  HIPCHK(c, hipMemcpy(ex_out, d.exa, (size_t)P * sizeof(int), hipMemcpyDeviceToHost));
  return GPE_OK;
}

int gpe_test_oz_planes(gpe_ctx* c, const gpe_oz_operand* a, int32_t packed, int32_t K, int32_t nmod, int32_t* ex_out,
                       int8_t* planes_out) {
  if (!c) return GPE_ERR_ARG;
  if (!a) return fail(c, GPE_ERR_ARG, "gpe_test_oz_planes: NULL operand");
  HIPCHK(c, hipSetDevice(c->device));
  return oz_test_planes(c, *a, packed, K, nmod, ex_out, planes_out);
}

struct GemmGroupBufs {
  gpe_ctx* c;
  GemmProb* ctx_probs;
  unsigned* ctx_tiles;
  bool prof;
  std::vector<double*> dev, keep;
  GemmProb* probs = nullptr;
  unsigned* tiles = nullptr;
  double* part = nullptr;
  int* tcnt = nullptr;
  explicit GemmGroupBufs(gpe_ctx* ctx) : c(ctx), ctx_probs(ctx->dprobs), ctx_tiles(ctx->dtiles), prof(ctx->prof) {}
  ~GemmGroupBufs() {
    c->dprobs = ctx_probs;
    c->dtiles = ctx_tiles;
    c->prof = prof;
    for (double* p : dev) if (p) (void)hipFree(p);
    for (double* p : keep) if (p) (void)hipFree(p);
    for (void* p : {(void*)probs, (void*)tiles, (void*)part, (void*)tcnt}) if (p) (void)hipFree(p);
  }
};
// ... 445 lines not shown
```

gp_emu_uqsa_amd/csrc/gpemu_ozaki.hpp:

```cpp
#pragma once
#include <algorithm>
#include <array>
#include <cmath>
#include <cstdlib>
#include <cstring>
#include <type_traits>
#include <utility>
#include <vector>

namespace gpe {

constexpr int OZ_T = 256;
constexpr int OZ_SK = 64;
constexpr int OZ_NBUF = 4;
constexpr int OZ_OPND = OZ_T * OZ_SK;
constexpr int OZ_LDS = OZ_NBUF * 2 * OZ_OPND;
constexpr int OZ_MAXMOD = 16;
constexpr int OZ_MAX_K = (1 << 17) - 128;

struct OzConst {
  int m[OZ_MAXMOD];
  int c16[OZ_MAXMOD];
  float inv[OZ_MAXMOD];
  int wlo[OZ_MAXMOD];
  int whi[OZ_MAXMOD];
  double rhi[OZ_MAXMOD];
  double rlo[OZ_MAXMOD];
  double Md;
  int nmod;
  int beta;
};

typedef int oz_v4i __attribute__((ext_vector_type(4)));
typedef int oz_v16i __attribute__((ext_vector_type(16)));

constexpr int OZ_EX_NAN = -(1 << 20), OZ_IL_BAD = 1 << 29;
__device__ __forceinline__ double oz_pmax(double a, double b) { return (a > b || a != a) ? a : b; }
__device__ __forceinline__ int oz_ex_of(double mx, int beta) {
  return !(mx <= 1.7976931348623157e308) ? OZ_EX_NAN : (mx > 0.0 ? (beta - 1) - ilogb(mx) : 0);
}

__host__ __device__ __forceinline__ long long oz_panel_off(int cb, int np2) {
  return (long long)OZ_T * ((long long)cb * np2 - (long long)OZ_T * cb * (cb - 1) / 2);
}
__host__ __device__ __forceinline__ long long oz_plane_bytes(int np2) { return oz_panel_off(np2 / OZ_T, np2); }

struct OzDigits {
  int lo, hi;
};
__host__ __device__ __forceinline__ OzDigits oz_digits(double x) {
  const unsigned long long c = 0x0080808080808080ull;
  const unsigned long long b = ((unsigned long long)(long long)x + c) ^ c;
  return OzDigits{(int)(unsigned)b, (int)(unsigned)(b >> 32)};
}
__host__ __device__ __forceinline__ int oz_dot4(int a, int b, int c) {
#if __HIP_DEVICE_COMPILE__
  return __builtin_amdgcn_sdot4(a, b, c, false);
#else
  for (int i = 0; i < 4; ++i) c += (int)(int8_t)((unsigned)a >> (8 * i)) * (int)(int8_t)((unsigned)b >> (8 * i));
  return c;
#endif
}
__host__ __device__ __forceinline__ int oz_mul24(int a, int b) {
#if __HIP_DEVICE_COMPILE__
  return __mul24(a, b);
#else
  const int a24 = (int)((unsigned)a << 8) >> 8, b24 = (int)((unsigned)b << 8) >> 8;
  return (int)((unsigned)a24 * (unsigned)b24);
#endif
}
__host__ __device__ __forceinline__ int oz_float_bits(float f) {
#if __HIP_DEVICE_COMPILE__
  return __float_as_int(f);
#else
  int i;
  std::memcpy(&i, &f, sizeof i);
  return i;
#endif
}
__host__ __device__ __forceinline__ int oz_digit_sum(OzDigits d, int wlo, int whi) {
  return oz_dot4(d.lo, wlo, oz_dot4(d.hi, whi, 0));
}
__host__ __device__ __forceinline__ unsigned oz_reduce(int t, float inv, int nm) {
#pragma clang fp contract(off)
  const float qf = (float)t * inv + 12582912.0f;
  return (unsigned)(oz_mul24(oz_float_bits(qf), nm) + t);
}
__host__ __device__ __forceinline__ unsigned oz_pack4(unsigned v0, unsigned v1, unsigned v2, unsigned v3) {
#if __HIP_DEVICE_COMPILE__
  return __builtin_amdgcn_perm(__builtin_amdgcn_perm(v3, v2, 0x0c0c0400u), __builtin_amdgcn_perm(v1, v0, 0x0c0c0400u),
                               0x05040100u);
#else
  return (v0 & 0xffu) | (v1 & 0xffu) << 8 | (v2 & 0xffu) << 16 | v3 << 24;
#endif
}
__host__ __device__ inline void oz_residues(double x, const OzConst& cst, int8_t* out) {
  const OzDigits d = oz_digits(x);
  for (int l = 0; l < cst.nmod; ++l)
    out[l] = (int8_t)(oz_reduce(oz_digit_sum(d, cst.wlo[l], cst.whi[l]), cst.inv[l], -cst.m[l]) & 0xffu);
}
__host__ __device__ __forceinline__ uint2 oz_residues8(const OzDigits (&d)[8], const OzConst& cst, int l) {
  const int wlo = cst.wlo[l], whi = cst.whi[l], nm = -cst.m[l];
  const float inv = cst.inv[l];
  unsigned v[8];
#pragma unroll
  for (int u = 0; u < 8; ++u) v[u] = oz_reduce(oz_digit_sum(d[u], wlo, whi), inv, nm);
  return make_uint2(oz_pack4(v[0], v[1], v[2], v[3]), oz_pack4(v[4], v[5], v[6], v[7]));
}

static __global__ void __launch_bounds__(256) k_oz_colexp(const double* __restrict__ X, long long ldx, int np,
                                                          int np2, int beta, int* __restrict__ ex) {
  const int lane = threadIdx.x & 63, j = blockIdx.x * 4 + (threadIdx.x >> 6);
  if (j >= np2) return;
  double mx = 0.0;
  if (j < np)
    for (int k = j + lane; k < np; k += 64) mx = oz_pmax(mx, fabs(X[k + (long long)j * ldx]));
  for (int off = 32; off > 0; off >>= 1) mx = oz_pmax(mx, __shfl_xor(mx, off, 64));
  if (lane == 0) ex[j] = oz_ex_of(mx, beta);
}

constexpr int OZ_SPLIT_ROWS = 8;
static __global__ void __launch_bounds__(256) k_oz_split(const double* __restrict__ X, long long ldx, int np,
                                                         int np2, const int* __restrict__ ex, int8_t* __restrict__ planes,
                                                         long long plane_bytes, OzConst cst) {
  const int j = blockIdx.x;
  const int cb = j / OZ_T, r0 = cb * OZ_T;
  const int k0 = r0 + OZ_SPLIT_ROWS * ((int)blockIdx.y * 256 + (int)threadIdx.x);
  if (k0 >= np2) return;
  const int e = ex[j];
  const long long ld = np2 - r0;
  int8_t* dst = planes + oz_panel_off(cb, np2) + (long long)(j - r0) * ld + (k0 - r0);
  if (j >= np || k0 >= np || k0 + OZ_SPLIT_ROWS <= j || e == OZ_EX_NAN) {
    for (int l = 0; l < cst.nmod; ++l) *reinterpret_cast<uint2*>(dst + (long long)l * plane_bytes) = make_uint2(0u, 0u);
    return;
  }
  double xs[OZ_SPLIT_ROWS];
  if (k0 + OZ_SPLIT_ROWS <= np && k0 >= j) {
#pragma unroll
    for (int u = 0; u < OZ_SPLIT_ROWS; u += 2) {
      const double2 v = *reinterpret_cast<const double2*>(X + k0 + u + (long long)j * ldx);
      xs[u] = v.x;
      xs[u + 1] = v.y;
    }
  } else {
#pragma unroll
    for (int u = 0; u < OZ_SPLIT_ROWS; ++u) {
      const int k = k0 + u;
      xs[u] = (k >= j && k < np) ? X[k + (long long)j * ldx] : 0.0;
    }
  }
  OzDigits d[OZ_SPLIT_ROWS];
#pragma unroll
  for (int u = 0; u < OZ_SPLIT_ROWS; ++u) d[u] = oz_digits(rint(ldexp(xs[u], e)));
  for (int l = 0; l < cst.nmod; ++l) *reinterpret_cast<uint2*>(dst + (long long)l * plane_bytes) = oz_residues8(d, cst, l);
}

__device__ __forceinline__ void oz_glds16(const int8_t* src, int8_t* dst) {
  __builtin_amdgcn_global_load_lds((const __attribute__((address_space(1))) void*)src,
                                   (__attribute__((address_space(3))) void*)dst, 16, 0, 0);
}
__device__ __forceinline__ const int8_t* oz_uniform(const int8_t* p) {
  const unsigned long long u = (unsigned long long)p;
  const unsigned lo = __builtin_amdgcn_readfirstlane((unsigned)u), hi = __builtin_amdgcn_readfirstlane((unsigned)(u >> 32));
  return (const int8_t*)(((unsigned long long)hi << 32) | lo);
}
template <int N> __device__ __forceinline__ void oz_vmwait() { asm volatile("s_waitcnt vmcnt(%0)" :: "n"(N) : "memory"); }

struct OzOpnd {
  const int8_t* p;
  long long plane_bytes;
  long long ld;
  int np2;
};
__device__ __forceinline__ const int8_t* oz_tile_rows(const OzOpnd& o, int t, int k, long long& ld) {
  if (o.ld == 0) {
    ld = o.np2 - OZ_T * t;
    return o.p + oz_panel_off(t, o.np2) + (k - OZ_T * t);
  }
  ld = o.ld;
  return o.p + (long long)OZ_T * t * o.ld + k;
}

struct OzGemm {
  OzOpnd a, b;
  const unsigned* list;
  int list_len;
  int K, kbeg, kend;
  int tri, ntj;
  int8_t* res;
  long long res_bytes;
  int kdiv = 1;
  int ti0 = 0;
};
__host__ __device__ __forceinline__ long long oz_res_tile(int tri, int ntj, int ti, int tj) {
  if (!tri) return (long long)ti * ntj + tj;
  if (ntj > 0 && ti >= ntj) return (long long)ntj * (ntj + 1) / 2 + (long long)(ti - ntj) * ntj + tj;
  return (long long)ti * (ti + 1) / 2 + tj;
}
__host__ __device__ __forceinline__ void oz_k_range(int kbeg, int kend, int kdiv, int K, int ti, int tj, int& kb, int& ke) {
  kb = kbeg == 1 ? OZ_T * ti : (kbeg == 2 ? OZ_T * tj : (kbeg == 3 ? 128 * ((2 * ti) / kdiv) : 0));
  ke = kend == 1 ? (K < OZ_T * (ti + 1) ? K : OZ_T * (ti + 1)) : K;
}

__device__ __forceinline__ void oz_vmwait_stages(int stages) {
  static_assert(OZ_NBUF <= 5, "one case per stage that can be in flight");
  if (stages >= 4) oz_vmwait<32>();
  else if (stages == 3) oz_vmwait<24>();
  else if (stages == 2) oz_vmwait<16>();
  else if (stages == 1) oz_vmwait<8>();
  else oz_vmwait<0>();
}

template <bool M256>
__device__ __forceinline__ void oz_store_residues(const oz_v16i (&acc)[4][4], int m, int c16, float inv, int8_t* out) {
#pragma clang fp contract(off)
  const int cm = c16 - 65536, nm = -m;
#pragma unroll
  for (int i = 0; i < 4; ++i)
#pragma unroll
    for (int j = 0; j < 4; ++j) {
      unsigned v[16];
#pragma unroll
      for (int r = 0; r < 16; ++r) {
        const int a = acc[i][j][r];
        if constexpr (M256) {
          v[r] = (unsigned)a;
        } else {
          const int t = __mul24(a >> 16, cm) + a;
          const float qf = (float)t * inv + 12582912.0f;
          v[r] = (unsigned)(__mul24(__float_as_int(qf), nm) + t);
        }
      }
      oz_v4i w;
#pragma unroll
      for (int u = 0; u < 4; ++u) {
        const unsigned lo = __builtin_amdgcn_perm(v[4 * u + 1], v[4 * u], 0x0c0c0400u);
        const unsigned hi = __builtin_amdgcn_perm(v[4 * u + 3], v[4 * u + 2], 0x0c0c0400u);
        w[u] = (int)__builtin_amdgcn_perm(hi, lo, 0x05040100u);
      }
      *reinterpret_cast<oz_v4i*>(out + (long long)(4 * i + j) * 64 * 16) = w;
    }
}

static __global__ void __launch_bounds__(256, 1) k_oz_gemm(OzGemm g, OzConst cst) {
  extern __shared__ __attribute__((aligned(16))) double lds_d[];
  int8_t* lds = reinterpret_cast<int8_t*>(lds_d);
  const int l = (int)blockIdx.x / g.list_len;
  const unsigned ent = g.list[(int)blockIdx.x - l * g.list_len];
  if (ent == 0xffffffffu) return;
  const int ti = (int)(ent >> 16), tj = (int)(ent & 0xffffu);
  int kb, ke;
  oz_k_range(g.kbeg, g.kend, g.kdiv, g.K, ti, tj, kb, ke);
  const int tid = threadIdx.x, lane = tid & 63;
  const int wave = __builtin_amdgcn_readfirstlane(tid >> 6);
  const int wm = (wave >> 1) * 128, wn = (wave & 1) * 128;
  OzOpnd oa = g.a, ob = g.b;
  oa.p += (long long)l * oa.plane_bytes;
  ob.p += (long long)l * ob.plane_bytes;
  long long lda, ldb;
  const int kp = (lane & 3) ^ ((lane >> 4) & 3);
  const int8_t* ua = oz_tile_rows(oa, ti, kb, lda);
  const int8_t* ub = oz_tile_rows(ob, tj, kb, ldb);
  unsigned va[4], vb[4];
#pragma unroll
  for (int p = 0; p < 4; ++p) {
    const unsigned row = (unsigned)(16 * wave + (lane >> 2) + 64 * p);
    va[p] = row * (unsigned)lda + 16u * (unsigned)kp;
    vb[p] = row * (unsigned)ldb + 16u * (unsigned)kp;
  }
  auto load1 = [&](int s, int u) {
    int8_t* dst = lds + ((unsigned)s % OZ_NBUF) * 2 * OZ_OPND + (u & 1) * OZ_OPND + 16 * (wave + 4 * (u >> 1)) * OZ_SK;
    const int8_t* src = oz_uniform(((u & 1) ? ub : ua) + (long long)s * OZ_SK);
    oz_glds16(src + ((u & 1) ? vb[u >> 1] : va[u >> 1]), dst);
  };
  oz_v16i acc[4][4];
#pragma unroll
  for (int i = 0; i < 4; ++i)
#pragma unroll
    for (int j = 0; j < 4; ++j) acc[i][j] = oz_v16i{};
  const int ns = max(0, ke - kb) / OZ_SK;
  const int r32 = lane & 31, h = lane >> 5, sw = (r32 >> 2) & 3;
  auto frag1 = [&](int s, int ks, int u, oz_v4i (&af)[4], oz_v4i (&bf)[4]) {
    const int8_t* As = lds + ((unsigned)s % OZ_NBUF) * 2 * OZ_OPND;
    const int8_t* Bs = As + OZ_OPND;
    const int slot = ((2 * ks + h) ^ sw) * 16;
    if (u < 4) af[u] = *reinterpret_cast<const oz_v4i*>(As + (wm + 32 * u + r32) * OZ_SK + slot);
    else bf[u - 4] = *reinterpret_cast<const oz_v4i*>(Bs + (wn + 32 * (u - 4) + r32) * OZ_SK + slot);
  };
  auto frags = [&](int s, int ks, oz_v4i (&af)[4], oz_v4i (&bf)[4]) {
#pragma unroll
    for (int u = 0; u < 8; ++u) frag1(s, ks, u, af, bf);
  };
  auto mfmas = [&](const oz_v4i (&af)[4], const oz_v4i (&bf)[4]) {
#pragma unroll
    for (int i = 0; i < 4; ++i)
#pragma unroll
      for (int j = 0; j < 4; ++j) acc[i][j] = __builtin_amdgcn_mfma_i32_32x32x32_i8(bf[j], af[i], acc[i][j], 0, 0, 0);
  };
  if (ns > 0) {
    oz_v4i ca[4], cb[4], na[4], nb[4];
    auto kstep = [&](const oz_v4i (&xa)[4], const oz_v4i (&xb)[4], auto READ, int rs, int rks, oz_v4i (&ya)[4],
                     oz_v4i (&yb)[4], auto LOAD, int ls, int u0) {
      mfmas(xa, xb);
      if constexpr (decltype(READ)::value) {
        frags(rs, rks, ya, yb);
#pragma unroll
        for (int u = 0; u < 8; ++u) {
          __builtin_amdgcn_sched_group_barrier(0x008, 1, 0);
          __builtin_amdgcn_sched_group_barrier(0x100, 1, 0);
        }
      } else {
        __builtin_amdgcn_sched_group_barrier(0x008, 8, 0);
      }
      if constexpr (decltype(LOAD)::value) {
#pragma unroll
        for (int u = 0; u < 4; ++u) {
          load1(ls, u0 + u);
          __builtin_amdgcn_sched_group_barrier(0x008, 1, 0);
          __builtin_amdgcn_sched_group_barrier(0x020, 1, 0);
          __builtin_amdgcn_sched_group_barrier(0x008, 1, 0);
        }
      } else {
        __builtin_amdgcn_sched_group_barrier(0x008, 8, 0);
      }
      __builtin_amdgcn_sched_barrier(0);
    };
    auto step = [&](int s, auto NEXT, auto LOADA, auto LOADB) {
      kstep(ca, cb, std::true_type{}, s, 1, na, nb, LOADA, s + OZ_NBUF - 1, 4);
      if constexpr (decltype(NEXT)::value) {
        if constexpr (decltype(LOADB)::value) oz_vmwait<8 * (OZ_NBUF - 2)>();
        else oz_vmwait_stages(ns - s - 2);
        asm volatile("s_waitcnt lgkmcnt(0)" ::: "memory");
        __builtin_amdgcn_s_barrier();
        __builtin_amdgcn_sched_barrier(0);
      }
      kstep(na, nb, NEXT, s + 1, 0, ca, cb, LOADB, s + OZ_NBUF, 0);
    };
    constexpr std::true_type Y{};
    constexpr std::false_type N{};
    if (ns < OZ_NBUF) {
      for (int s = 0; s < ns; ++s)
#pragma unroll
        for (int u = 0; u < 8; ++u) load1(s, u);
      oz_vmwait_stages(ns - 1);
    } else {
#pragma unroll
      for (int s = 0; s < OZ_NBUF; ++s)
#pragma unroll
        for (int u = 0; u < (s == OZ_NBUF - 1 ? 4 : 8); ++u) load1(s, u);
      oz_vmwait<8 * (OZ_NBUF - 2) + 4>();
    }
    asm volatile("s_waitcnt lgkmcnt(0)" ::: "memory");
    __builtin_amdgcn_s_barrier();
    frags(0, 0, ca, cb);
    int s = 0;
    for (; s + OZ_NBUF < ns; ++s) step(s, Y, Y, Y);
    if (ns >= OZ_NBUF) step(s++, Y, Y, N);
    for (; s + 1 < ns; ++s) step(s, Y, N, N);
    if (s < ns) step(s, N, N, N);
  }
  const int m = cst.m[l];
  int8_t* out = g.res + (long long)l * g.res_bytes +
                (oz_res_tile(g.tri, g.ntj, ti, tj) - oz_res_tile(g.tri, g.ntj, g.ti0, 0)) * (OZ_T * OZ_T) +
                ((long long)(wave * 16) * 64 + lane) * 16;
  if (m == 256) oz_store_residues<true>(acc, m, 0, 0.0f, out);
  else oz_store_residues<false>(acc, m, cst.c16[l], cst.inv[l], out);
}

struct OzCrt {
  const int8_t* res;
  long long res_bytes;
  int tri, ntj;
  const int* exr;
  const int* exc;
  double* C;
  long long ldc;
  int rows, cols, lower128;
  double alpha;
  int ti0 = 0;
  int acc = 0;
};
template <int NM>
static __global__ void __launch_bounds__(256) k_oz_crt(OzCrt g, OzConst cst) {
  const int nmod = NM ? NM : cst.nmod;
  const int t = (int)blockIdx.x >> 4;
  const int u = ((int)blockIdx.x & 15) * 256 + (int)threadIdx.x;
  int ti, tj;
  if (g.tri) {
    const int ta = t + (int)oz_res_tile(1, g.ntj, g.ti0, 0), cap = g.ntj * (g.ntj + 1) / 2;
    if (g.ntj > 0 && ta >= cap) {
      ti = g.ntj + (ta - cap) / g.ntj;
      tj = (ta - cap) % g.ntj;
    } else {
      ti = g.ti0;
      while ((ti + 1) * (ti + 2) / 2 <= ta) ++ti;
      tj = ta - ti * (ti + 1) / 2;
    }
  } else {
    ti = g.ti0 + t / g.ntj;
    tj = t % g.ntj;
  }
  const int wave = u >> 10, blk = (u >> 6) & 15, lane = u & 63;
  const int i = blk >> 2, j = blk & 3;
  const int gm = OZ_T * ti + (wave >> 1) * 128 + 32 * i + (lane & 31);
  const int gn0 = OZ_T * tj + (wave & 1) * 128 + 32 * j + 4 * (lane >> 5);
  if (gm >= g.rows || gn0 >= g.cols) return;
  const int8_t* src = g.res + (long long)t * (OZ_T * OZ_T) + (long long)u * 16;
  oz_v4i w[OZ_MAXMOD];
#pragma unroll
  for (int l = 0; l < OZ_MAXMOD; ++l)
    if (l < nmod) w[l] = *reinterpret_cast<const oz_v4i*>(src + (long long)l * g.res_bytes);
  const int em = g.exr[gm];
  oz_v4i ec[4];
  const bool ec16 = (reinterpret_cast<uintptr_t>(g.exc) & 15) == 0;
#pragma unroll
  for (int q = 0; q < 4; ++q) {
    const int gn = gn0 + 8 * q;
    if (ec16 && gn + 3 < g.cols) {
      ec[q] = *reinterpret_cast<const oz_v4i*>(g.exc + gn);
    } else {
#pragma unroll
      for (int i = 0; i < 4; ++i) ec[q][i] = gn + i < g.cols ? g.exc[gn + i] : 0;
    }
  }
  double shi[16], slo[16];
#pragma unroll
  for (int r = 0; r < 16; ++r) shi[r] = slo[r] = 0.0;
#pragma unroll
  for (int l = 0; l < OZ_MAXMOD; ++l)
    if (l < nmod) {
      const double rh = cst.rhi[l], rl = cst.rlo[l];
#pragma unroll
      for (int r = 0; r < 16; ++r) {
        const double cv = (double)(int)(int8_t)((unsigned)w[l][r >> 2] >> (8 * (r & 3)));
        shi[r] = fma(cv, rh, shi[r]);
        slo[r] = fma(cv, rl, slo[r]);
      }
    }
  const double sc = g.alpha * cst.Md;
#pragma unroll
  for (int r = 0; r < 16; ++r) {
    const int gn = gn0 + (r & 3) + 8 * (r >> 2);
    if (gn >= g.cols || (g.lower128 && (gm >> 7) < (gn >> 7))) continue;
    const double v = (shi[r] - rint(shi[r])) + slo[r];
    const int en = ec[r >> 2][r & 3];
    double* dst = g.C + (gm - OZ_T * g.ti0 + (long long)gn * g.ldc);
    const double s = ldexp(sc, -(em + en));
    if (em == OZ_EX_NAN || en == OZ_EX_NAN) *dst = __builtin_nan("");
    else *dst = g.acc ? fma(v, s, *dst) : v * s;
  }
}

__device__ __forceinline__ bool oz_keep(int mask, int r, int k) {
  return mask == 1 ? k >= r : (mask == 2 ? k <= r : true);
}

template <bool TRANS>
static __global__ void __launch_bounds__(256) k_oz_rowexp(const double* __restrict__ src, long long ld, int R, int Rp,
                                                          int Kv, int mask, int beta, int* __restrict__ ex) {
  if constexpr (!TRANS) {
    const int lane = threadIdx.x & 63, r = blockIdx.x * 4 + (threadIdx.x >> 6);
    if (r >= Rp) return;
    double mx = 0.0;
    if (r < R)
      for (int k = lane; k < Kv; k += 64)
        if (oz_keep(mask, r, k)) mx = oz_pmax(mx, fabs(src[k + (long long)r * ld]));
    for (int off = 32; off > 0; off >>= 1) mx = oz_pmax(mx, __shfl_xor(mx, off, 64));
    if (lane == 0) ex[r] = oz_ex_of(mx, beta);
  } else {
    __shared__ double red[4][64];
    const int rl = threadIdx.x & 63, q = threadIdx.x >> 6, r = blockIdx.x * 64 + rl;
    const int k0 = blockIdx.y * 256;
    double mx = 0.0;
    if (r < R)
#pragma unroll 8
      for (int u = 0; u < 64; ++u) {
        const int k = k0 + 4 * u + q;
        if (k < Kv && oz_keep(mask, r, k)) mx = oz_pmax(mx, fabs(src[r + (long long)k * ld]));
      }
    red[q][rl] = mx;
    __syncthreads();
    if (q == 0 && r < R) {
      mx = oz_pmax(oz_pmax(red[0][rl], red[1][rl]), oz_pmax(red[2][rl], red[3][rl]));
      if (!(mx <= 1.7976931348623157e308)) atomicMax(ex + r, OZ_IL_BAD);
      else if (mx > 0.0) atomicMax(ex + r, ilogb(mx) + 2048);
    }
  }
}
static __global__ void __launch_bounds__(256) k_oz_il_to_ex(int* __restrict__ ex, int Rp, int beta) {
  const int r = blockIdx.x * 256 + threadIdx.x;
  if (r < Rp) ex[r] = ex[r] >= OZ_IL_BAD ? OZ_EX_NAN : (ex[r] > 0 ? (beta - 1) - (ex[r] - 2048) : 0);
}

template <bool TRANS>
static __global__ void __launch_bounds__(256) k_oz_split_rect(const double* __restrict__ src, long long ld, int R,
                                                              int Kv, int mask, const int* __restrict__ ex,
                                                              int8_t* __restrict__ planes, long long plane_bytes,
                                                              long long ldp, int Kp, OzConst cst) {
  if constexpr (!TRANS) {
    const int r = blockIdx.x;
    const int k0 = ((int)blockIdx.y * 256 + (int)threadIdx.x) * 8;
    if (k0 >= Kp) return;
    const int e = ex[r];
    const double* p = src + k0 + (long long)r * ld;
    const int side = mask == 1 ? (k0 >= r ? 1 : (k0 + 7 < r ? 0 : 2))
                   : (mask == 2 ? (k0 + 7 <= r ? 1 : (k0 > r ? 0 : 2)) : 1);
    int8_t* dst = planes + (long long)r * ldp + k0;
    if (side == 0 || r >= R || k0 >= Kv || e == OZ_EX_NAN) {
      for (int l = 0; l < cst.nmod; ++l) *reinterpret_cast<uint2*>(dst + (long long)l * plane_bytes) = make_uint2(0u, 0u);
      return;
    }
    double xs[8];
    if (k0 + 8 <= Kv && side == 1 && ((reinterpret_cast<uintptr_t>(p) & 15) == 0)) {
#pragma unroll
      for (int u = 0; u < 8; u += 2) {
        const double2 v = *reinterpret_cast<const double2*>(p + u);
        xs[u] = v.x;
        xs[u + 1] = v.y;
      }
    } else {
#pragma unroll
      for (int u = 0; u < 8; ++u) {
        const int k = k0 + u;
        xs[u] = (k < Kv && oz_keep(mask, r, k)) ? p[u] : 0.0;
      }
    }
    OzDigits d[8];
#pragma unroll
    for (int u = 0; u < 8; ++u) d[u] = oz_digits(rint(ldexp(xs[u], e)));
    for (int l = 0; l < cst.nmod; ++l) *reinterpret_cast<uint2*>(dst + (long long)l * plane_bytes) = oz_residues8(d, cst, l);
  } else {
    constexpr int PL = 4;
    __shared__ __attribute__((aligned(16))) unsigned tr[PL][64 * 20];
    const int lane = threadIdx.x & 63, rp = lane & 31, kg = (int)threadIdx.x >> 5;
    const int wr = (int)threadIdx.x >> 2, wp = (int)threadIdx.x & 3;
    int8_t* dst = planes + ((long long)blockIdx.x * 64 + wr) * ldp + (long long)blockIdx.y * 64 + 16 * wp;
    {
      const int rb = (int)blockIdx.x * 64, kb = (int)blockIdx.y * 64;
      if (rb >= R || kb >= Kv || (mask == 1 && kb + 63 < rb) || (mask == 2 && kb > rb + 63)) {
        for (int l = 0; l < cst.nmod; ++l) *reinterpret_cast<uint4*>(dst + (long long)l * plane_bytes) = make_uint4(0u, 0u, 0u, 0u);
        return;
      }
    }
    const int r = (int)blockIdx.x * 64 + 2 * rp;
    const int k0 = (int)blockIdx.y * 64 + 8 * kg;
    const int e0 = ex[r], e1 = ex[r + 1];
    double x0[8], x1[8];
    const double* p = src + r + (long long)k0 * ld;
    const bool vec = r + 1 < R && ((reinterpret_cast<uintptr_t>(src + r) & 15) == 0) && (ld & 1) == 0;
#pragma unroll
    for (int u = 0; u < 8; ++u) {
      const int k = k0 + u;
      double a = 0.0, b = 0.0;
      if (k < Kv) {
        if (vec) {
          const double2 v = *reinterpret_cast<const double2*>(p + (long long)u * ld);
          a = v.x;
          b = v.y;
        } else {
          if (r < R) a = p[(long long)u * ld];
          if (r + 1 < R) b = p[(long long)u * ld + 1];
        }
      }
      x0[u] = oz_keep(mask, r, k) ? a : 0.0;
      x1[u] = oz_keep(mask, r + 1, k) ? b : 0.0;
    }
    OzDigits d0[8], d1[8];
#pragma unroll
    for (int u = 0; u < 8; ++u) {
      d0[u] = oz_digits(e0 == OZ_EX_NAN ? 0.0 : rint(ldexp(x0[u], e0)));
      d1[u] = oz_digits(e1 == OZ_EX_NAN ? 0.0 : rint(ldexp(x1[u], e1)));
    }
    for (int l0 = 0; l0 < cst.nmod; l0 += PL) {
      if (l0 > 0) __syncthreads();
#pragma unroll
      for (int q = 0; q < PL; ++q)
        if (l0 + q < cst.nmod) {
          *reinterpret_cast<uint2*>(tr[q] + (2 * rp) * 20 + 2 * kg) = oz_residues8(d0, cst, l0 + q);
          *reinterpret_cast<uint2*>(tr[q] + (2 * rp + 1) * 20 + 2 * kg) = oz_residues8(d1, cst, l0 + q);
        }
      __syncthreads();
#pragma unroll
      for (int q = 0; q < PL; ++q)
        if (l0 + q < cst.nmod)
          *reinterpret_cast<uint4*>(dst + (long long)(l0 + q) * plane_bytes) =
              *reinterpret_cast<const uint4*>(tr[q] + wr * 20 + 4 * wp);
    }
  }
}


inline OzConst oz_consts(int nmod, int np2) {
  static const int mods[OZ_MAXMOD] = {256, 253, 251, 247, 241, 239, 233, 229, 227, 223, 217, 211, 199, 197, 193, 191};
  OzConst k{};
  k.nmod = nmod;
  double log2M = 0.0, Md = 1.0;
  for (int l = 0; l < nmod; ++l) {
    log2M += std::log2((double)mods[l]);
    Md *= (double)mods[l];
  }
  k.Md = Md;
  k.beta = std::min(53, (int)std::floor((log2M - 1.0 - std::log2((double)np2) - 1e-9) / 2.0));
  for (int l = 0; l < nmod; ++l) {
    const int m = mods[l];
    k.m[l] = m;
    k.c16[l] = 65536 % m;
    k.inv[l] = 1.0f / (float)m;
    unsigned w[2] = {0u, 0u};
    for (int i = 0, p = 1; i < 7; ++i, p = (p * 256) % m) {
      const int wc = p > m / 2 ? p - m : p;
      w[i >> 2] |= ((unsigned)wc & 0xffu) << (8 * (i & 3));
    }
    k.wlo[l] = (int)w[0];
    k.whi[l] = (int)w[1];
    long long Mm = 1;
    for (int j = 0; j < nmod; ++j)
      if (j != l) Mm = (Mm * (mods[j] % m)) % m;
    int y = 1;
    while ((Mm * y) % m != 1) ++y;
    const long long num = (long long)y << 41;
    const long long Q = num / m, R = num - Q * m;
    k.rhi[l] = std::ldexp((double)Q, -41);
    k.rlo[l] = std::ldexp((double)R / (double)m, -41);
  }
  return k;
}

template <class W>
std::vector<unsigned> oz_list(int nti, int ntj, bool lower, W work, int ti0 = 0) {
  static const std::pair<int, int> blk = [] {
    int r = 8, c = 4;
    if (const char* e = std::getenv("GPEMU_OZ_BLOCK")) {
      const int rr = std::atoi(e);
      const char* x = std::strchr(e, 'x');
      if (rr > 0 && x && std::atoi(x + 1) > 0) { r = rr; c = std::atoi(x + 1); }
    }
    return std::make_pair(r, c);
  }();
  const int OZ_BR = blk.first, OZ_BC = blk.second;
  struct Blk { double w; std::vector<unsigned> t; };
  std::vector<Blk> blks;
  for (int r0 = ti0; r0 < ti0 + nti; r0 += OZ_BR)
    for (int c0 = 0; c0 < ntj && (!lower || c0 <= r0 + OZ_BR - 1); c0 += OZ_BC) {
      Blk b{0.0, {}};
      for (int ti = r0; ti < std::min(ti0 + nti, r0 + OZ_BR); ++ti)
        for (int tj = c0; tj < std::min(std::min(lower ? ti + 1 : ntj, ntj), c0 + OZ_BC); ++tj) {
          b.t.push_back(((unsigned)ti << 16) | (unsigned)tj);
          b.w += work(ti, tj);
        }
      if (!b.t.empty()) blks.push_back(std::move(b));
    }
  std::stable_sort(blks.begin(), blks.end(), [](const Blk& x, const Blk& y) { return x.w / x.t.size() > y.w / y.t.size(); });
  std::vector<std::vector<unsigned>> bins(8);
  std::vector<double> load(8, 0.0);
  for (const Blk& b : blks) {
    const int x = (int)(std::min_element(load.begin(), load.end()) - load.begin());
    load[x] += b.w;
    bins[x].insert(bins[x].end(), b.t.begin(), b.t.end());
  }
  size_t longest = 0;
  for (auto& b : bins) longest = std::max(longest, b.size());
  std::vector<unsigned> list(8 * longest, 0xffffffffu);
  for (int x = 0; x < 8; ++x)
    for (size_t q = 0; q < bins[x].size(); ++q) list[8 * q + x] = bins[x][q];
  return list;
}


struct OzSrc {
  const double* src;
  long long ld;
  int R, Kv, mask;
  bool trans;
};
inline void oz_operand_exp(hipStream_t st, const OzConst& k, const OzSrc& o, int P, int* ex) {
  if (o.trans) {
    (void)hipMemsetAsync(ex, 0, (size_t)P * sizeof(int), st);
    hipLaunchKernelGGL(k_oz_rowexp<true>, dim3(P / 64, (o.Kv + 255) / 256), dim3(256), 0, st, o.src, o.ld, o.R, P, o.Kv,
                       o.mask, k.beta, ex);
    hipLaunchKernelGGL(k_oz_il_to_ex, dim3((P + 255) / 256), dim3(256), 0, st, ex, P, k.beta);
  } else {
    hipLaunchKernelGGL(k_oz_rowexp<false>, dim3(P / 4), dim3(256), 0, st, o.src, o.ld, o.R, P, o.Kv, o.mask, k.beta, ex);
  }
}
inline void oz_operand_split(hipStream_t st, const OzConst& k, const OzSrc& o, int P, int Kp, const int* ex, int8_t* planes) {
  if (o.trans)
    hipLaunchKernelGGL(k_oz_split_rect<true>, dim3(P / 64, Kp / 64), dim3(256), 0, st, o.src, o.ld, o.R, o.Kv, o.mask, ex,
                       planes, (long long)P * Kp, (long long)Kp, Kp, k);
  else
    hipLaunchKernelGGL(k_oz_split_rect<false>, dim3(P, (Kp + 2047) / 2048), dim3(256), 0, st, o.src, o.ld, o.R, o.Kv,
                       o.mask, ex, planes, (long long)P * Kp, (long long)Kp, Kp, k);
}
inline void oz_operand(hipStream_t st, const OzConst& k, const OzSrc& o, int P, int Kp, int* ex, int8_t* planes) {
  oz_operand_exp(st, k, o, P, ex);
  oz_operand_split(st, k, o, P, Kp, ex, planes);
}
inline void oz_operand_packed(hipStream_t st, const OzConst& k, const double* X, long long ldx, int np, int np2, int* ex,
                              int8_t* planes) {
  hipLaunchKernelGGL(k_oz_colexp, dim3((np2 + 3) / 4), dim3(256), 0, st, X, ldx, np, np2, k.beta, ex);
  hipLaunchKernelGGL(k_oz_split, dim3(np2, (np2 + 256 * OZ_SPLIT_ROWS - 1) / (256 * OZ_SPLIT_ROWS)), dim3(256), 0, st, X,
                     ldx, np, np2, ex, planes, oz_plane_bytes(np2), k);
}

struct OzShape {
  int nti, ntj, ti0, tri, K, kbeg, kend, kdiv;
  static OzShape lower(int nti, int ti0, int K, int kbeg, int kdiv = 1) { return {nti, 0, ti0, 1, K, kbeg, 0, kdiv}; }
  static OzShape lower_capped(int nti, int cap, int K) { return {nti, cap < nti ? cap : 0, 0, 1, K, 0, 0, 1}; }
  static OzShape rect(int nti, int ntj, int K, int kbeg, int kend) { return {nti, ntj, 0, 0, K, kbeg, kend, 1}; }
  int row_tiles(int ti) const { return tri ? (ntj > 0 ? std::min(ti + 1, ntj) : ti + 1) : ntj; }
  int klen(int ti, int tj) const {
    int kb, ke;
    oz_k_range(kbeg, kend, kdiv, K, ti, tj, kb, ke);
    return std::max(0, ke - kb);
  }
  std::vector<unsigned> list() const {
    return oz_list(nti, tri && ntj == 0 ? ti0 + nti : ntj, tri != 0, [&](int ti, int tj) { return (double)klen(ti, tj); }, ti0);
  }
  long long res_tile(int ti, int tj) const { return oz_res_tile(tri, ntj, ti, tj) - oz_res_tile(tri, ntj, ti0, 0); }
  long long tiles() const { return tri ? oz_res_tile(1, ntj, ti0 + nti, 0) - oz_res_tile(1, ntj, ti0, 0) : (long long)nti * ntj; }
  long long res_bytes() const { return tiles() * OZ_T * OZ_T; }
  double ops(int N) const {
    double s = 0.0;
    for (int ti = ti0; ti < ti0 + nti; ++ti)
      for (int tj = 0; tj < row_tiles(ti); ++tj) s += klen(ti, tj);
    return 2.0 * OZ_T * OZ_T * s * N;
  }
};

inline OzShape oz_lauum_shape(int np2) { return OzShape::lower(np2 / OZ_T, 0, np2, 1); }
inline OzShape oz_slab_shape(int a0, int a1, int Kp, int P) {
  return OzShape::lower((a1 + 1) / 2 - a0 / 2, a0 / 2, Kp, 3, P);
}

struct OzOut {
  const int* exr;
  const int* exc;
  double* C;
  long long ldc;
  int rows, cols, lower128;
  double alpha;
  int acc = 0;
};
struct OzProduct {
  OzShape s;
  OzOpnd a, b;
  const unsigned* list;
  int list_len;
  int8_t* res;
  long long res_bytes;
  OzOut out;
};
inline hipError_t oz_product_launch(hipStream_t st, const OzConst& k, const OzProduct& p, hipEvent_t e0 = nullptr,
                                    hipEvent_t e1 = nullptr) {
  const OzShape& s = p.s;
  const int ntj = s.ntj;
  const OzGemm g{p.a, p.b, p.list, p.list_len, s.K, s.kbeg, s.kend, s.tri, ntj, p.res, p.res_bytes, s.kdiv, s.ti0};
  const OzOut& o = p.out;
  const OzCrt r{p.res, p.res_bytes, s.tri, ntj, o.exr, o.exc, o.C, o.ldc, o.rows, o.cols, o.lower128, o.alpha, s.ti0, o.acc};
  hipError_t e;
  if (e0 && (e = hipEventRecord(e0, st)) != hipSuccess) return e;
  hipLaunchKernelGGL(k_oz_gemm, dim3((unsigned)(k.nmod * g.list_len)), dim3(256), OZ_LDS, st, g, k);
  if (e1 && (e = hipEventRecord(e1, st)) != hipSuccess) return e;
  if (k.nmod == OZ_MAXMOD) hipLaunchKernelGGL(k_oz_crt<OZ_MAXMOD>, dim3((unsigned)(s.tiles() * 16)), dim3(256), 0, st, r, k);
  else hipLaunchKernelGGL(k_oz_crt<0>, dim3((unsigned)(s.tiles() * 16)), dim3(256), 0, st, r, k);
  return hipGetLastError();
}

inline std::vector<std::array<int, 3>> trtri_level_pairs(int NB, int s) {
  std::vector<std::array<int, 3>> prs;
  for (int t0 = 0; t0 < NB; t0 += s) {
    const int h = t0 + s / 2;
    if (h >= NB) continue;
    prs.push_back({t0, h, std::min(t0 + s, NB)});
  }
  return prs;
}

inline std::vector<std::array<int, 3>> trtri_side_pairs(const std::vector<std::array<int, 3>>& prs, int hs, int side) {
  std::vector<std::array<int, 3>> out;
  for (const auto& pr : prs)
    if (!(pr[0] < hs && pr[2] > hs) && (pr[0] >= hs) == (side == 1)) out.push_back(pr);
  return out;
}

struct OzTriPair {
  int t0, h, t1, Ra, Rb, Pa, Pb;
  long long la_off, lb_off;
  int la_len, lb_len;
  double ops_a, ops_b;
  OzShape shape_a() const { return OzShape::rect(Pb / OZ_T, Pa / OZ_T, Pa, 2, 0); }
  OzShape shape_b() const { return OzShape::rect(Pb / OZ_T, Pa / OZ_T, Pb, 0, 1); }
  OzShape shape_schur() const { return OzShape::lower(Pb / OZ_T, 0, Pa, 0); }
  size_t planes_bytes(int N) const { return (size_t)N * Pa * (Pa + Pb); }
  size_t resid_bytes(int N) const { return (size_t)N * shape_a().res_bytes(); }
  OzSrc l21(const double* L21, long long ld) const { return {L21, ld, Rb, Ra, 0, true}; }
};
inline OzTriPair oz_tri_pair_plan(int t0, int h, int t1, int N, std::vector<unsigned>& lists) {
  OzTriPair q;
  q.t0 = t0; q.h = h; q.t1 = t1;
  q.Ra = (h - t0) * TILE;
  q.Rb = (t1 - h) * TILE;
  q.Pa = (q.Ra + OZ_T - 1) / OZ_T * OZ_T;
  q.Pb = (q.Rb + OZ_T - 1) / OZ_T * OZ_T;
  const std::vector<unsigned> la = q.shape_a().list(), lb = q.shape_b().list();
  q.ops_a = q.shape_a().ops(N);
  q.ops_b = q.shape_b().ops(N);
  q.la_off = (long long)lists.size();
  q.la_len = (int)la.size();
  lists.insert(lists.end(), la.begin(), la.end());
  q.lb_off = (long long)lists.size();
  q.lb_len = (int)lb.size();
  lists.insert(lists.end(), lb.begin(), lb.end());
  return q;
}

struct OzCholNest {
  int q, h, NB, Rb, Pb, K, cols;
  OzShape shape() const { return OzShape::lower_capped(Pb / OZ_T, (h - q) / 2, K); }
  OzSrc src(const double* Lq0, long long ld) const { return {Lq0, ld, Rb, K, 0, true}; }
  size_t planes_bytes(int N) const { return (size_t)N * Pb * K; }
  size_t resid_bytes(int N) const { return (size_t)N * shape().res_bytes(); }
};
inline OzCholNest oz_chol_nest_plan(int q, int h, int NB) {
  OzCholNest n;
  n.q = q; n.h = h; n.NB = NB;
  n.Rb = (NB - q) * TILE;
  n.Pb = (n.Rb + OZ_T - 1) / OZ_T * OZ_T;
  n.K = q * TILE;
  n.cols = (h - q) * TILE;
  return n;
}

template <class GC>
void oz_tri_pair_launches(hipStream_t st, const OzConst& k, const OzTriPair& q, const unsigned* lists, const double* L21,
                          const double* X11, const double* X22, double* X21, long long ld, double* T, int8_t* planes,
                          int8_t* res, int* ex, bool l21_done, GC gc, int part = 0) {
  int* exA = ex;
  int* exB = ex + q.Pb;
  int8_t* PA = planes;
  const long long rb = q.shape_a().res_bytes();
  if (part != 2) {
    const long long pA = (long long)q.Pb * q.Pa, pB = (long long)q.Pa * q.Pa;
    int8_t* PB = planes + (size_t)k.nmod * pA;
    if (!l21_done) oz_operand(st, k, q.l21(L21, ld), q.Pb, q.Pa, exA, PA);
    oz_operand(st, k, OzSrc{X11, ld, q.Ra, q.Ra, 1, false}, q.Pa, q.Pa, exB, PB);
    gc(OzProduct{q.shape_a(), OzOpnd{PA, pA, q.Pa, 0}, OzOpnd{PB, pB, q.Pa, 0}, lists + q.la_off, q.la_len, res, rb,
                 OzOut{exA, exB, T, (long long)q.Pb, q.Rb, q.Ra, 0, 1.0}},
       q.ops_a, (double)q.Ra * q.Ra * q.Rb);
  }
  if (part != 1) {
    const long long pA = (long long)q.Pb * q.Pb, pB = (long long)q.Pa * q.Pb;
    int8_t* PB = planes + (size_t)k.nmod * pA;
    const OzSrc x22{X22, ld, q.Rb, q.Rb, 2, true}, t{T, (long long)q.Pb, q.Ra, q.Rb, 0, false};
    oz_operand_exp(st, k, x22, q.Pb, exA);
    oz_operand_exp(st, k, t, q.Pa, exB);
    oz_operand_split(st, k, x22, q.Pb, q.Pb, exA, PA);
    oz_operand_split(st, k, t, q.Pa, q.Pb, exB, PB);
    gc(OzProduct{q.shape_b(), OzOpnd{PA, pA, q.Pb, 0}, OzOpnd{PB, pB, q.Pb, 0}, lists + q.lb_off, q.lb_len, res, rb,
                 OzOut{exA, exB, X21, ld, q.Rb, q.Ra, 0, -1.0}},
       q.ops_b, (double)q.Rb * q.Rb * q.Ra);
  }
}

}
```

gp_emu_uqsa_amd/native.py:

```python
from __future__ import annotations

import ctypes as _ct
import hashlib as _hashlib
import os as _os
import threading as _threading

import numpy as _np

_HERE = _os.path.dirname(_os.path.abspath(__file__))
_DEFAULT_LIB = _os.path.join(_HERE, "libgpemu.so")
LIB_PATH = _os.environ.get("GPEMU_LIB", _DEFAULT_LIB)

GPE_OK = 0
GPE_NOT_PD = 1
KERNEL_STD = 0
KERNEL_ALT_NUG = 1
KERNEL_MATERN32 = 0x10
KERNEL_MATERN52 = 0x20
GP4ML = 0
MUCM = 1

_D = _ct.POINTER(_ct.c_double)
_VP = _ct.c_void_p

class OzOperand(_ct.Structure):
    _fields_ = [("src", _D), ("len", _ct.c_int64), ("offset", _ct.c_int64), ("ld", _ct.c_int64),
                ("trans", _ct.c_int32), ("R", _ct.c_int32), ("Kv", _ct.c_int32), ("mask", _ct.c_int32)]


class OzParams(_ct.Structure):
    _fields_ = [(n, _ct.c_int32) for n in ("packed", "K", "kbeg", "kend", "kdiv", "ti0", "tri", "lower128", "acc",
                                           "nmod", "rows", "cols", "res_mod")] + \
               [("ldc", _ct.c_int64), ("c_len", _ct.c_int64), ("alpha", _ct.c_double)]


class GemmGroupProb(_ct.Structure):
    _fields_ = [(n, _ct.c_int32) for n in ("a_buf", "b_buf", "c_buf", "mt", "nt", "K", "flags", "kti_mul",
                                           "kti_off")] + \
               [(n, _ct.c_int64) for n in ("a_off", "lda", "b_off", "ldb", "c_off", "ldc")] + \
               [("alpha", _ct.c_double), ("beta", _ct.c_double)]


class GemmGroupLaunch(_ct.Structure):
    _fields_ = [(n, _ct.c_int32) for n in ("kind", "split", "listed", "reps")]


G_CLOWER, G_KBEG_TI, G_KEND_TI = 1, 2, 4

SIGNATURES = {
    "gpe_test_gemm_group": (_ct.c_int, [_VP, _ct.c_int32, _ct.POINTER(_D), _ct.POINTER(_ct.c_int64), _ct.c_int32,
                                        _ct.POINTER(GemmGroupProb), _ct.POINTER(GemmGroupLaunch),
                                        _ct.POINTER(_ct.c_int32), _ct.POINTER(_ct.c_int32),
                                        _ct.POINTER(_ct.c_uint32), _ct.c_int64]),
    "gpe_test_oz_product": (_ct.c_int, [_VP, _ct.POINTER(OzOperand), _ct.POINTER(OzOperand),
                                        _ct.POINTER(OzParams), _D, _ct.POINTER(_ct.c_int32),
                                        _ct.POINTER(_ct.c_int32), _ct.POINTER(_ct.c_int8)]),
    "gpe_test_oz_planes": (_ct.c_int, [_VP, _ct.POINTER(OzOperand), _ct.c_int32, _ct.c_int32, _ct.c_int32,
                                       _ct.POINTER(_ct.c_int32), _ct.POINTER(_ct.c_int8)]),
    "gpe_abi_version": (_ct.c_int, []),
    "gpe_build_id": (_ct.c_char_p, []),
    "gpe_device_count": (_ct.c_int, []),
    "gpe_device_synchronize": (_ct.c_int, [_ct.c_int32]),
    "gpe_create": (_VP, [_ct.c_int32]),
    "gpe_destroy": (None, [_VP]),
    "gpe_last_error": (_ct.c_char_p, [_VP]),
    "gpe_set_data": (_ct.c_int, [_VP, _ct.c_int64, _ct.c_int32, _ct.c_int32, _D, _D, _D, _D]),
    "gpe_objective": (_ct.c_int, [_VP, _ct.c_int32, _ct.c_int32, _D, _ct.c_int32, _ct.c_double,
                                  _ct.c_int32, _D, _D, _D]),
    "gpe_factor": (_ct.c_int, [_VP, _ct.c_int32, _D, _ct.c_double, _ct.c_double, _ct.c_double]),
    "gpe_beta": (_ct.c_int, [_VP, _D]),
    "gpe_loo": (_ct.c_int, [_VP, _ct.c_double, _D, _D, _D]),
    "gpe_posterior": (_ct.c_int, [_VP, _ct.c_int64, _D, _D, _D, _ct.c_double, _ct.c_int32, _ct.c_int32,
                                  _D, _D]),
    "gpe_posterior_grad": (_ct.c_int, [_VP, _ct.c_int64, _D, _D, _D, _ct.POINTER(_ct.c_int32), _D, _ct.c_double,
                                       _D, _D, _D, _D]),
    "gpe_posterior_mean": (_ct.c_int, [_VP, _ct.c_int64, _D, _D, _D, _D]),
    "gpe_set_outputs": (_ct.c_int, [_VP, _ct.c_int32, _D]),
    "gpe_objective_multi": (_ct.c_int, [_VP, _ct.c_int32, _D, _ct.c_int32, _ct.c_double, _ct.c_int32, _D, _D, _D,
                                        _D]),
    "gpe_beta_multi": (_ct.c_int, [_VP, _D]),
    "gpe_posterior_mean_multi": (_ct.c_int, [_VP, _ct.c_int64, _D, _D, _D, _D]),
    "gpe_posterior_groups": (_ct.c_int, [_VP, _ct.c_int64, _ct.c_int32, _D, _D, _D, _ct.c_double, _D, _D]),
    "gpe_noise_sample": (_ct.c_int, [_VP, _ct.c_int64, _D, _D, _D, _ct.c_double, _D, _ct.c_double,
                                     _D, _ct.c_int32, _D, _D, _D]),
    "gpe_posterior_pivchol": (_ct.c_int, [_VP, _ct.c_int64, _D, _D, _D, _ct.c_double, _D, _ct.c_double,
                                          _ct.c_int64, _ct.c_double, _D, _ct.POINTER(_ct.c_int64), _D, _D,
                                          _ct.POINTER(_ct.c_int64)]),
    "gpe_posterior_imse": (_ct.c_int, [_VP, _ct.c_int64, _ct.c_int64, _D, _D, _D, _ct.c_double, _D, _ct.c_double,
                                       _D, _ct.c_int64, _ct.c_double, _D, _ct.POINTER(_ct.c_int64), _D, _D, _D,
                                       _ct.POINTER(_ct.c_int64)]),
    "gpe_hm_destroy": (None, [_VP]),
    "gpe_hm_last_error": (_ct.c_char_p, [_VP]),
    "gpe_hm_add": (_ct.c_int, [_VP, _VP, _ct.c_int32, _ct.POINTER(_ct.c_int32), _ct.c_int32,
                               _ct.POINTER(_ct.c_int32), _D, _D, _ct.c_double]),
    "gpe_hm_count": (_ct.c_int, [_VP]),
    "gpe_hm_implausibility": (_ct.c_int, [_VP, _ct.c_int64, _ct.c_int32, _D, _D, _D, _ct.c_int32, _D, _D, _D]),
    "gpe_solve": (_ct.c_int, [_VP, _ct.c_int32, _D, _D]),
    "gpe_sense_pairs": (_ct.c_int, [_VP, _ct.c_int32, _D, _D, _ct.c_int32, _D, _D, _D]),
    "gpe_gauss_transform": (_ct.c_int, [_VP, _ct.c_int64, _ct.c_int32, _ct.POINTER(_ct.c_int32), _D, _D, _D,
                                        _D]),
    "gpe_kernel_var": (_ct.c_int, [_VP, _ct.c_int32, _D, _ct.c_int32, _ct.c_double, _ct.c_int32,
                                   _ct.c_int64, _D, _D, _ct.c_double, _D]),
    "gpe_kernel_covar": (_ct.c_int, [_VP, _ct.c_int32, _D, _ct.c_int32, _ct.c_double, _ct.c_int64,
                                     _D, _ct.c_int64, _D, _D]),
    "gpe_kernel_grad": (_ct.c_int, [_VP, _D, _ct.c_int32, _ct.c_int64, _D, _D, _ct.c_double, _ct.c_double, _D]),
    "gpe_kernel_grad_k": (_ct.c_int, [_VP, _ct.c_int32, _D, _ct.c_int32, _ct.c_int64, _D, _D, _ct.c_double,
                                      _ct.c_double, _D]),
    "gpe_lhc_maximin": (_ct.c_int, [_VP, _ct.c_int32, _ct.c_int64, _ct.c_int32, _D, _ct.c_int64, _D,
                                    _ct.POINTER(_ct.c_int64)]),
    "gpe_cholesky": (_ct.c_int, [_VP, _ct.c_int64, _D, _D, _D, _D, _D]),
    "gpe_test_gemm": (_ct.c_int, [_VP, _ct.c_int32, _ct.c_int32, _ct.c_int64, _ct.c_int64,
                                  _ct.c_int64, _D, _D, _D, _ct.c_double, _ct.c_double]),
    "gpe_bench_gemm": (_ct.c_int, [_VP, _ct.c_int32, _ct.c_int32, _ct.c_int32, _ct.c_int32,
                                   _ct.c_int32, _ct.c_int32, _ct.c_double, _ct.c_int32, _D]),
    "gpe_set_profiling": (_ct.c_int, [_VP, _ct.c_int32]),
    "gpe_phase_times": (_ct.c_int, [_VP, _D, _ct.c_int32]),
    "gpe_gemm_stats": (_ct.c_int, [_VP, _D, _D, _D]),
    "gpe_ozaki_stats": (_ct.c_int, [_VP, _D, _D, _D, _D]),
    "gpe_dist_unique_id": (_ct.c_int, [_ct.c_char_p, _ct.c_int32]),
    "gpe_dist_create": (_VP, [_ct.c_int32, _ct.c_int32, _ct.c_int32, _ct.c_char_p]),
    "gpe_dist_destroy": (None, [_VP]),
    "gpe_dist_last_error": (_ct.c_char_p, [_VP]),
    "gpe_dist_set_data": (_ct.c_int, [_VP, _ct.c_int64, _ct.c_int32, _ct.c_int32, _D, _D, _D, _D]),
    "gpe_dist_objective": (_ct.c_int, [_VP, _ct.c_int32, _ct.c_int32, _D, _ct.c_int32, _ct.c_double,
                                       _ct.c_int32, _D, _D, _D]),
    "gpe_dist_owner": (_ct.c_int32, [_ct.c_int32, _ct.c_int32]),
    "gpe_dist_local_rows": (_ct.c_int32, [_ct.c_int64, _ct.c_int32, _ct.c_int32, _ct.c_int32]),
    "gpe_dist_times": (_ct.c_int, [_VP, _D, _D]),
    "gpe_dist_rank_bytes": (_ct.c_int, [_VP, _ct.c_int32, _ct.POINTER(_ct.c_int64)]),
}

HANDLE_SIGNATURES = {
    "gpe_hm_create": (_VP, [_ct.c_int32]),
}

UNIQUE_ID_BYTES = 128


class NativeUnavailable(RuntimeError):
    """libgpemu.so is missing or no HIP device is visible (no CPU fallback)."""


class NotPositiveDefinite(ArithmeticError):
    """Cholesky met a non-positive / NaN pivot (the reference's LinAlgError)."""


_lib = None
_lib_lock = _threading.Lock()


def load_library(path: str | None = None):
    global _lib
    with _lib_lock:
        if _lib is not None and path is None:
            return _lib
        p = path or LIB_PATH
        if not _os.path.exists(p):
            raise NativeUnavailable(
                f"{p} not found: build it with `python -c 'import __graft_entry__ as g; g.build()'`")
        lib = _ct.CDLL(p)
        for name, (res, args) in list(SIGNATURES.items()) + list(HANDLE_SIGNATURES.items()):
            fn = getattr(lib, name)
            fn.restype = res
            fn.argtypes = args
        from . import buildinfo
        want = buildinfo.source_hash() if p == _DEFAULT_LIB else None
        have = lib.gpe_build_id().decode()
        if want is not None and have != want:
            raise NativeUnavailable(
                f"{p} was built from other sources (build id {have[:12]}, sources {want[:12]}): "
                "rebuild it with `python -c 'import __graft_entry__ as g; g.build()'`")
        if path is None:
            _lib = lib
        return lib


def build_id() -> str:
    return load_library().gpe_build_id().decode()


def _ptr(a):
    if a is None:
        return None
    return a.ctypes.data_as(_D)


def _f64(a, shape=None):
    arr = _np.ascontiguousarray(a, dtype=_np.float64)
    if shape is not None:
        arr = arr.reshape(shape)
    return arr


class Context:

    def __init__(self, device: int = 0):
        self.lib = load_library()
        if self.lib.gpe_device_count() <= 0:
            raise NativeUnavailable("no HIP device visible to libgpemu.so")
        h = self.lib.gpe_create(int(device))
        if not h:
# ... 315 lines not shown
            X = X.reshape(-1, 1)
        m, d = X.shape
        delta = _f64(delta).ravel()
        rr = None if r is None or _np.isscalar(r) else _f64(r, (m,))
        out = _np.zeros((m, m))
        self._check(self.lib.gpe_kernel_var(self._h, int(kernel), _ptr(delta), d, float(nu),
                                            1 if predict else 0, m, _ptr(X), _ptr(rr),
                                            float(r_scale), _ptr(out)), "gpe_kernel_var")
        return out

    def kernel_covar(self, kernel, delta, nu, XT, XV):
        XT = _f64(XT)
        XV = _f64(XV)
        if XT.ndim == 1:
            XT = XT.reshape(-1, 1)
        if XV.ndim == 1:
            XV = XV.reshape(-1, 1)
        n, d = XT.shape
        m = XV.shape[0]
        delta = _f64(delta).ravel()
        out = _np.zeros((n, m))
        self._check(self.lib.gpe_kernel_covar(self._h, int(kernel), _ptr(delta), d, float(nu), n,
                                              _ptr(XT), m, _ptr(XV), _ptr(out)), "gpe_kernel_covar")
        return out

    def kernel_grad(self, delta, X, col, col_scale, pre):
        X = _f64(X)
        if X.ndim == 1:
            X = X.reshape(-1, 1)
        m, d = X.shape
        delta = _f64(delta).ravel()
        cc = None if col is None else _f64(col, (m,))
        out = _np.zeros((m, m))
        self._check(self.lib.gpe_kernel_grad(self._h, _ptr(delta), d, m, _ptr(X), _ptr(cc),
                                             float(col_scale), float(pre), _ptr(out)), "gpe_kernel_grad")
        return out

    def kernel_grad_k(self, kernel, delta, X, col, col_scale, pre):
        X = _f64(X)
        if X.ndim == 1:
            X = X.reshape(-1, 1)
        m, d = X.shape
        delta = _f64(delta).ravel()
        cc = None if col is None else _f64(col, (m,))
        out = _np.zeros((m, m))
        self._check(self.lib.gpe_kernel_grad_k(self._h, int(kernel), _ptr(delta), d, m, _ptr(X), _ptr(cc),
                                               float(col_scale), float(pre), _ptr(out)), "gpe_kernel_grad_k")
        return out

    def lhc_maximin(self, designs, fextra=None):
        designs = _f64(designs)
        N, n, dim = designs.shape
        fe = None if fextra is None else _f64(fextra).reshape(-1, dim)
        ne = 0 if fe is None else fe.shape[0]
        out = _np.zeros(N, dtype=_np.int64)
        self._check(self.lib.gpe_lhc_maximin(self._h, N, n, dim, _ptr(designs), ne, _ptr(fe),
                                             out.ctypes.data_as(_ct.POINTER(_ct.c_int64))), "gpe_lhc_maximin")
        return out

    def cholesky(self, A, want=("L",)):
        A = _f64(A)
        m = A.shape[0]
        outs = {k: _np.zeros((m, m)) for k in want if k in ("L", "Linv", "Ainv")}
        ld = _ct.c_double(0.0)
        self._check(self.lib.gpe_cholesky(self._h, m, _ptr(A), _ptr(outs.get("L")),
                                          _ptr(outs.get("Linv")), _ptr(outs.get("Ainv")),
                                          _ct.byref(ld)), "gpe_cholesky")
        outs["logdet"] = ld.value
        return outs

    def test_gemm(self, A, B, C, alpha=1.0, beta=0.0, trans_a=0, trans_b=0):
        A = _f64(A)
        B = _f64(B)
        C = _f64(C).copy()
        M, K = A.shape
        N = B.shape[1]
        self._check(self.lib.gpe_test_gemm(self._h, int(trans_a), int(trans_b), M, N, K, _ptr(A),
                                           _ptr(B), _ptr(C), float(alpha), float(beta)),
                    "gpe_test_gemm")
        return C

    def test_oz_product(self, a, b=None, *, C, ldc, packed=False, K=0, kbeg=0, kend=0, kdiv=1, ti0=0,
                        tri=False, lower128=False, alpha=1.0, acc=False, nmod=16, rows=0, cols=0,
                        res_mod=None):
        keep = []

        def opnd(o):
            src = _np.ascontiguousarray(o["src"], dtype=_np.float64).ravel()
            keep.append(src)
            return OzOperand(_ptr(src), src.size, int(o.get("offset", 0)), int(o["ld"]), int(o.get("trans", 0)),
                             int(o.get("R", 0)), int(o.get("Kv", 0)), int(o.get("mask", 0)))

        oa = opnd(a)
        ob = opnd(b) if b is not None else None
        pad = lambda r: (r + 255) // 256 * 256
        Pa = pad(oa.R)
        Pb = pad(ob.R) if ob is not None else Pa
        Cc = _np.array(C, dtype=_np.float64).ravel()
        p = OzParams(int(bool(packed)), int(K), int(kbeg), int(kend), int(kdiv), int(ti0), int(bool(tri)),
                     int(bool(lower128)), int(bool(acc)), int(nmod), int(rows), int(cols),
                     -1 if res_mod is None else int(res_mod), int(ldc), Cc.size, float(alpha))
        exa = _np.zeros(max(Pa, 1), dtype=_np.int32)
        exb = _np.zeros(max(Pb, 1), dtype=_np.int32)
        res = None if res_mod is None else _np.zeros((max(Pa - 256 * int(ti0), 1), max(Pb, 1)), dtype=_np.int8)
        i32 = _ct.POINTER(_ct.c_int32)
        self._check(self.lib.gpe_test_oz_product(
            self._h, _ct.byref(oa), _ct.byref(ob) if ob is not None else None, _ct.byref(p), _ptr(Cc),
            exa.ctypes.data_as(i32), exb.ctypes.data_as(i32),
            None if res is None else res.ctypes.data_as(_ct.POINTER(_ct.c_int8))), "gpe_test_oz_product")
        return {"C": Cc, "exa": exa, "exb": exb, "res": res}

    def test_oz_planes(self, a, *, packed=False, K=0, nmod=16):
        src = _np.ascontiguousarray(a["src"], dtype=_np.float64).ravel()
        oa = OzOperand(_ptr(src), src.size, int(a.get("offset", 0)), int(a["ld"]), int(a.get("trans", 0)),
                       int(a.get("R", 0)), int(a.get("Kv", 0)), int(a.get("mask", 0)))
        P = (oa.R + 255) // 256 * 256
        ex = _np.zeros(max(P, 1), dtype=_np.int32)
        planes = _np.zeros((int(nmod), max(P, 1), max(P if packed else int(K), 1)), dtype=_np.int8)
        self._check(self.lib.gpe_test_oz_planes(
            self._h, _ct.byref(oa), int(bool(packed)), int(K), int(nmod), ex.ctypes.data_as(_ct.POINTER(_ct.c_int32)),
            planes.ctypes.data_as(_ct.POINTER(_ct.c_int8))), "gpe_test_oz_planes")
        return {"ex": ex, "planes": planes}

    def test_gemm_group(self, bufs, probs, *, kind, split=False, listed=False, reps=1):
        out = [_np.array(b, dtype=_np.float64).ravel() for b in bufs]
        ptrs = (_D * len(out))(*[_ptr(b) for b in out])
        lens = (_ct.c_int64 * len(out))(*[b.size for b in out])
        ps = (GemmGroupProb * max(len(probs), 1))()
        cap = 0
        for q, p in zip(ps, probs):
            (q.a_buf, q.a_off, q.lda), (q.b_buf, q.b_off, q.ldb), (q.c_buf, q.c_off, q.ldc) = \
                [tuple(int(v) for v in p[k]) for k in ("a", "b", "c")]
            q.mt, q.nt, q.K, q.flags = int(p["mt"]), int(p["nt"]), int(p["K"]), int(p.get("flags", 0))
            q.kti_mul, q.kti_off = int(p.get("kti_mul", 1)), int(p.get("kti_off", 0))
            q.alpha, q.beta = float(p.get("alpha", 1.0)), float(p.get("beta", 0.0))
            if 0 < q.mt <= 4096 and 0 < q.nt <= 4096:
                cap += q.mt * (q.mt + 1) // 2 if q.flags & G_CLOWER else q.mt * q.nt
        gl = GemmGroupLaunch(int(kind), int(split), int(listed), int(reps))
        ksplit = _np.zeros(max(len(probs), 1), dtype=_np.int32)
        info = _np.zeros(3, dtype=_np.int32)
        tiles = _np.zeros(max(cap, 1), dtype=_np.uint32)
        i32 = _ct.POINTER(_ct.c_int32)
        self._check(self.lib.gpe_test_gemm_group(
            self._h, len(out), ptrs, lens, len(probs), ps, _ct.byref(gl), ksplit.ctypes.data_as(i32),
            info.ctypes.data_as(i32), tiles.ctypes.data_as(_ct.POINTER(_ct.c_uint32)), cap), "gpe_test_gemm_group")
        return {"bufs": out, "ksplit": ksplit[:len(probs)], "listed": bool(info[0]), "cdef": bool(info[1]),
                "workgroups": int(info[2]), "tiles": tiles[:cap].copy() if info[0] else None}

    def bench_gemm(self, mt, nt, K, trans_a=0, trans_b=0, lower=False, beta=1.0, reps=5):
        ms = _ct.c_double()
        self._check(self.lib.gpe_bench_gemm(self._h, int(trans_a), int(trans_b), int(mt), int(nt),
                                            int(K), 1 if lower else 0, float(beta), int(reps),
                                            _ct.byref(ms)), "gpe_bench_gemm")
        return ms.value

    def set_profiling(self, on=True):
        self._check(self.lib.gpe_set_profiling(self._h, 1 if on else 0), "gpe_set_profiling")

    def phase_times(self):
        out = _np.zeros(8)
        self._check(self.lib.gpe_phase_times(self._h, _ptr(out), 8), "gpe_phase_times")
        keys = ["kbuild", "cholesky", "trtri", "inverse", "skinny", "contract", "total"]
        return dict(zip(keys, out[:7].tolist()))

    def gemm_stats(self):
        ms, nl, fl = _ct.c_double(), _ct.c_double(), _ct.c_double()
        self._check(self.lib.gpe_gemm_stats(self._h, _ct.byref(ms), _ct.byref(nl), _ct.byref(fl)),
                    "gpe_gemm_stats")
        return {"ms": ms.value, "launches": nl.value, "flops": fl.value}

    def ozaki_stats(self):
        ms, nl, ops, fl = _ct.c_double(), _ct.c_double(), _ct.c_double(), _ct.c_double()
        self._check(self.lib.gpe_ozaki_stats(self._h, _ct.byref(ms), _ct.byref(nl), _ct.byref(ops), _ct.byref(fl)),
                    "gpe_ozaki_stats")
        return {"ms": ms.value, "launches": nl.value, "int8_ops": ops.value, "fp64_flops": fl.value}


_default_ctx = None
_ctx_lock = _threading.Lock()


_tls = _threading.local()
_extra_ctxs: list = []


class EmulatorSet:

    MAX_N, MAX_D, MAX_Q, MAX_EMUL = 512, 32, 16, 32

    def __init__(self, device: int = 0):
        self.lib = load_library()
        if self.lib.gpe_device_count() <= 0:
            raise NativeUnavailable("no HIP device visible to libgpemu.so")
        h = self.lib.gpe_hm_create(int(device))
        if not h:
            raise NativeUnavailable("gpe_hm_create failed: " + self.lib.gpe_hm_last_error(None).decode())
        self._h = h
        self.device = device
        self._maxact = -1

    def close(self):
        if getattr(self, "_h", None):
            self.lib.gpe_hm_destroy(self._h)
            self._h = None

    def __del__(self):
        try:
            self.close()
        except Exception:
            pass

    def __len__(self):
        return int(self.lib.gpe_hm_count(self._h))

    def _check(self, rc, what):
        if rc == GPE_OK:
            return
        msg = self.lib.gpe_hm_last_error(self._h).decode()
        if rc == GPE_NOT_PD:
            raise NotPositiveDefinite(f"{what}: {msg}")
        err = RuntimeError(f"{what} failed ({rc}): {msg}")
        err.status = rc
        raise err

    def add(self, ctx, active, hdim, hval, beta, sigma):
        i32 = _ct.POINTER(_ct.c_int32)
        active = _np.ascontiguousarray(active, dtype=_np.int32).ravel()
        hdim = _np.ascontiguousarray(hdim, dtype=_np.int32).ravel()
        hval = _f64(hval).ravel()
        beta = _f64(beta).ravel()
        if not (hdim.size == hval.size == beta.size):
            raise ValueError("hdim, hval and beta have one entry per basis column")
        rc = self.lib.gpe_hm_add(self._h, ctx._h, active.size, active.ctypes.data_as(i32), hdim.size,
                                 hdim.ctypes.data_as(i32), _ptr(hval), _ptr(beta), float(sigma))
        if rc < 0 or (rc == GPE_NOT_PD and self.lib.gpe_hm_last_error(self._h)):
            self._check(rc, "gpe_hm_add")
        return rc

    def implausibility(self, Xs, z, var_extra, maxno=1, parts=False):
        Xs = _f64(Xs)
        if Xs.ndim == 1:
            Xs = Xs.reshape(-1, 1)
        m, D = Xs.shape
        p = len(self)
        z = _f64(z).ravel()
        ve = _f64(var_extra).ravel()
        if z.size != p or ve.size != p:
            raise ValueError("z and var_extra have one entry per emulator of the set")
        maxno = int(maxno)
        imax = _np.zeros((m, max(maxno, 1)))
        mean = _np.zeros((p, m)) if parts else None
        var = _np.zeros((p, m)) if parts else None
        self._check(self.lib.gpe_hm_implausibility(self._h, m, D, _ptr(Xs), _ptr(z), _ptr(ve), maxno, _ptr(imax),
                                                   _ptr(mean), _ptr(var)), "gpe_hm_implausibility")
        return (imax, mean, var) if parts else imax


def default_context() -> Context:
    bound = getattr(_tls, "ctx", None)
# ... 126 lines not shown
```

include/gpemu.h:

```cpp
#ifndef GPEMU_H
#define GPEMU_H

#include <stdint.h>

#ifdef __cplusplus
extern "C" {
#endif

#define GPE_ABI_VERSION 10

enum gpe_status {
    GPE_OK = 0,
    GPE_NOT_PD = 1,
    GPE_ERR_ARG = -1,
    GPE_ERR_HIP = -2,
    GPE_ERR_ALLOC = -3,
    GPE_ERR_STATE = -4,
    GPE_ERR_UNSUPPORTED = -5
};

enum gpe_kernel {
    GPE_KERNEL_STD = 0,
    GPE_KERNEL_ALT_NUG = 1,
    GPE_KERNEL_MATERN32 = 0x10,
// ... 36 lines not shown
int gpe_posterior_grad(gpe_ctx* ctx, int64_t m, const double* Xs, const double* Hs,
                       const double* dHs, const int32_t* hdim, const double* beta, double sigma,
                       double* mean_out, double* var_out, double* dmean_out, double* dvar_out);

int gpe_posterior_mean(gpe_ctx* ctx, int64_t m, const double* Xs, const double* Hs,
                       const double* beta, double* mean_out);


int gpe_set_outputs(gpe_ctx* ctx, int32_t p, const double* F);

int gpe_objective_multi(gpe_ctx* ctx, int32_t kernel, const double* hp, int32_t n_hp, double nu_fixed,
                        int32_t want_grad, double* llh_out, double* grad_out, double* Sigma_out,
                        double* B_out);

int gpe_beta_multi(gpe_ctx* ctx, double* B_out);

int gpe_posterior_mean_multi(gpe_ctx* ctx, int64_t m, const double* Xs, const double* Hs,
                             const double* B, double* mean_out);

int gpe_posterior_groups(gpe_ctx* ctx, int64_t m, int32_t G, const double* Xs, const double* Hs,
                         const double* beta, double sigma, double* mean_out, double* cov_out);

typedef struct gpe_hm gpe_hm;

gpe_hm* gpe_hm_create(int32_t device);
void gpe_hm_destroy(gpe_hm* set);
const char* gpe_hm_last_error(const gpe_hm* set);

int gpe_hm_add(gpe_hm* set, gpe_ctx* ctx, int32_t d, const int32_t* active, int32_t q,
               const int32_t* hdim, const double* hval, const double* beta, double sigma);
int gpe_hm_count(const gpe_hm* set);

int gpe_hm_implausibility(gpe_hm* set, int64_t m, int32_t D, const double* Xs, const double* z,
                          const double* var_extra, int32_t maxno, double* imax_out,
                          double* mean_out, double* var_out);


int gpe_solve(gpe_ctx* ctx, int32_t ncols, const double* B, double* X);

int gpe_sense_pairs(gpe_ctx* ctx, int32_t J, const double* w, const double* u, int32_t p,
                    const double* Z, double* trace_out, double* quad_out);

int gpe_gauss_transform(gpe_ctx* ctx, int64_t m, int32_t ns, const int32_t* dims,
                        const double* c, const double* Y, const double* a, double* out);

int gpe_kernel_var(gpe_ctx* ctx, int32_t kernel, const double* delta, int32_t d,
                   double nu, int32_t predict, int64_t m, const double* X,
                   const double* r, double r_scale, double* A_out);

int gpe_kernel_grad(gpe_ctx* ctx, const double* delta, int32_t d, int64_t m, const double* X,
                    const double* col, double col_scale, double pre, double* G_out);

int gpe_kernel_grad_k(gpe_ctx* ctx, int32_t kernel, const double* delta, int32_t d, int64_t m,
                      const double* X, const double* col, double col_scale, double pre,
                      double* G_out);

int gpe_lhc_maximin(gpe_ctx* ctx, int32_t N, int64_t n, int32_t dim, const double* designs,
                    int64_t ne, const double* fextra, int64_t* idx_out);

int gpe_kernel_covar(gpe_ctx* ctx, int32_t kernel, const double* delta, int32_t d,
                     double nu, int64_t n, const double* XT, int64_t m,
                     const double* XV, double* C_out);

int gpe_cholesky(gpe_ctx* ctx, int64_t m, const double* A, double* L_out,
                 double* Linv_out, double* Ainv_out, double* logdet_out);

int gpe_test_gemm(gpe_ctx* ctx, int32_t trans_a, int32_t trans_b, int64_t M, int64_t N,
                  int64_t K, const double* A, const double* B, double* C,
                  double alpha, double beta);

typedef struct gpe_oz_operand {
    const double* src;
    int64_t len, offset, ld;
    int32_t trans, R, Kv, mask;
} gpe_oz_operand;
typedef struct gpe_oz_params {
    int32_t packed, K, kbeg, kend, kdiv, ti0, tri, lower128, acc, nmod, rows, cols, res_mod;
    int64_t ldc, c_len;
    double alpha;
} gpe_oz_params;
int gpe_test_oz_product(gpe_ctx* ctx, const gpe_oz_operand* a, const gpe_oz_operand* b,
                        const gpe_oz_params* p, double* C, int32_t* exa_out, int32_t* exb_out,
                        int8_t* res_out);

int gpe_test_oz_planes(gpe_ctx* ctx, const gpe_oz_operand* a, int32_t packed, int32_t K,
                       int32_t nmod, int32_t* ex_out, int8_t* planes_out);

enum { GPE_G_CLOWER = 1, GPE_G_KBEG_TI = 2, GPE_G_KEND_TI = 4 };
typedef struct gpe_gemm_group_prob {
    int32_t a_buf, b_buf, c_buf;
    int32_t mt, nt, K, flags, kti_mul, kti_off;
    int64_t a_off, lda, b_off, ldb, c_off, ldc;
    double alpha, beta;
} gpe_gemm_group_prob;
typedef struct gpe_gemm_group_launch {
    int32_t kind, split, listed, reps;
} gpe_gemm_group_launch;
int gpe_test_gemm_group(gpe_ctx* ctx, int32_t nbuf, double* const* bufs, const int64_t* lens,
                        int32_t nprob, const gpe_gemm_group_prob* probs,
                        const gpe_gemm_group_launch* launch, int32_t* ksplit_out,
                        int32_t* info_out, uint32_t* tiles_out, int64_t tiles_cap);

int gpe_bench_gemm(gpe_ctx* ctx, int32_t trans_a, int32_t trans_b, int32_t mt, int32_t nt,
                   int32_t K, int32_t lower, double beta, int32_t reps, double* ms_out);

int gpe_noise_sample(gpe_ctx* ctx, int64_t m, const double* Xs, const double* Hs,
                     const double* beta, double sigma, const double* r_new, double r_scale,
                     const double* t, int32_t s, const double* U, double* mean_out,
                     double* z_out);

int gpe_posterior_pivchol(gpe_ctx* ctx, int64_t m, const double* Xs, const double* Hs,
                          const double* beta, double sigma, const double* r_new, double r_scale,
                          int64_t k, double tol, double* mean_out, int64_t* piv_out,
                          double* pivvar_out, double* L_out, int64_t* rank_out);

int gpe_posterior_imse(gpe_ctx* ctx, int64_t m, int64_t mc, const double* Xs, const double* Hs,
                       const double* beta, double sigma, const double* r_new, double r_scale,
                       const double* w, int64_t k, double tol, double* mean_out,
                       int64_t* piv_out, double* gain_out, double* pivvar_out,
                       double* imse0_out, int64_t* rank_out);

int gpe_set_profiling(gpe_ctx* ctx, int32_t on);
int gpe_phase_times(gpe_ctx* ctx, double* ms_out, int32_t n);

int gpe_gemm_stats(gpe_ctx* ctx, double* ms_out, double* launches_out,
                   double* flops_out);

int gpe_ozaki_stats(gpe_ctx* ctx, double* ms_out, double* launches_out, double* int8_ops_out,
                    double* fp64_flops_out);

#ifdef __cplusplus
}
#endif

#endif
```

Measured before the change: 19.83.

## Certify Ozaki int8 products to drop one CRT modulus when bound allows

```diff
diff --git a/gp_emu_uqsa_amd/csrc/gpemu.hip b/gp_emu_uqsa_amd/csrc/gpemu.hip
--- a/gp_emu_uqsa_amd/csrc/gpemu.hip
+++ b/gp_emu_uqsa_amd/csrc/gpemu.hip
@@ -54,6 +54,7 @@
 };
 
 constexpr int OZ_CHOL_MIN = 8192;
+constexpr int OZ_CERT_MIN_NP = 4096;
 constexpr int OZ_CHOL_NEST_MIN = 12288;
 
 
@@ -140,6 +141,13 @@
   int8_t* dozp = nullptr;
   int8_t* dozr = nullptr;
   int* dozx = nullptr;
+  int oz_cert_on = 1, oz_cert_min_np = OZ_CERT_MIN_NP;
+  unsigned long long* dozs = nullptr;
+  int* dozf = nullptr;
+  unsigned long long* dozm = nullptr;
+  int oz_flag_cap = 0, oz_cert_used = 0;
+  OzConst oz_c15{};
+  std::vector<std::pair<int, double>> oz_cert_ops;
   unsigned* dozl = nullptr;
   double* dozt = nullptr;
   hipEvent_t ev_oz = nullptr;
@@ -823,6 +831,8 @@
                       double rscale, bool invert = true, bool objective = false, const Cols* cols = nullptr) {
   c->linv_valid = false;
   c->oz_l21_valid = false;
+  c->oz_cert_used = 0;
+  c->oz_cert_ops.clear();
   HIPCHK(c, hipStreamSynchronize(c->stream2));
   HIPCHK(c, hipMemsetAsync(c->dinfo, 0, sizeof(int), c->stream));
   CHK(build_plan(c, c->tr));
@@ -979,6 +989,19 @@
   CHK(dalloc(c, &c->dozp, planes));
   CHK(dalloc(c, &c->dozr, resid));
   CHK(dalloc(c, &c->dozx, nex));
+  c->oz_flag_cap = 0;
+  c->oz_cert_used = 0;
+  if (c->oz_cert_on && N == OZ_MAXMOD && c->n_pad >= c->oz_cert_min_np) {
+    const size_t nflag = 2 * c->oz_tri.size() + 8;
+    CHK(dalloc(c, &c->dozs, nex));
+    CHK(dalloc(c, &c->dozf, nflag));
+    CHK(dalloc(c, &c->dozm, 2 * nflag));
+    HIPCHK(c, hipMemset(c->dozm, 0, 2 * nflag * sizeof(unsigned long long)));
+    HIPCHK(c, hipMemset(c->dozs, 0, nex * sizeof(unsigned long long)));
+    HIPCHK(c, hipMemset(c->dozf, 0, nflag * sizeof(int)));
+    c->oz_flag_cap = (int)nflag;
+    c->oz_c15 = oz_consts_cert(np2);
+  }
   CHK(dalloc(c, &c->dozt, scratch));
   CHK(dalloc(c, &c->dozl, all.size()));
   HIPCHK(c, hipMemcpy(c->dozl, all.data(), all.size() * sizeof(unsigned), hipMemcpyHostToDevice));
@@ -987,6 +1010,13 @@
   c->oz_npad = c->n_pad;
   return GPE_OK;
 }
+
+OzCert oz_cert(gpe_ctx* c, const unsigned long long* sa, int na, const unsigned long long* sb, int nb) {
+  if (!c->oz_flag_cap || c->oz_cert_used >= c->oz_flag_cap) return OzCert{};
+  const int slot = c->oz_cert_used++;
+  return OzCert{sa, na, sb, nb, c->dozf + slot, &c->oz_c15, c->dozm + 2 * slot};
+}
+unsigned long long* oz_sums(gpe_ctx* c) { return c->oz_flag_cap ? c->dozs : nullptr; }
 
 int oz_gemm_crt(gpe_ctx* c, const OzConst& k, const OzProduct& p, double ops, double flops64,
                 hipStream_t st = nullptr) {
@@ -1007,6 +1037,7 @@
     c->oz_launches += 1.0;
     c->oz_ops += ops;
     c->oz_flops64 += flops64;
+    if (p.cert.flag && k.nmod == OZ_MAXMOD) c->oz_cert_ops.emplace_back((int)(p.cert.flag - c->dozf), ops);
   }
   return GPE_OK;
 }
@@ -1020,26 +1051,28 @@
     if (with_aug) CHK(launch_gemm_range(c, pl.launches[pl.aug_q], st));
     const long long ld = F.n_pad;
     c->oz_l21_valid = false;
-    oz_operand(st, c->oz_c, n.src(F.A + (long long)n.q * TILE, ld), n.Pb, n.K, c->dozx, c->dozp);
+    oz_operand(st, c->oz_c, n.src(F.A + (long long)n.q * TILE, ld), n.Pb, n.K, c->dozx, c->dozp, oz_sums(c));
     HIPCHK(c, hipGetLastError());
     const OzShape s = n.shape();
     const OzOpnd l{c->dozp, (long long)n.Pb * n.K, n.K, 0};
     return oz_gemm_crt(c, c->oz_c,
                        OzProduct{s, l, l, c->dozl + c->oz_nest_loff, c->oz_nest_llen, c->dozr, s.res_bytes(),
-                                 OzOut{c->dozx, c->dozx, F.A + (long long)n.q * TILE * (ld + 1), ld, n.Rb, n.cols, 1, -1.0, 1}},
+                                 OzOut{c->dozx, c->dozx, F.A + (long long)n.q * TILE * (ld + 1), ld, n.Rb, n.cols, 1, -1.0, 1},
+                                 oz_cert(c, c->dozs, n.Pb, c->dozs, n.Pb)},
                        c->oz_nest_ops, (double)n.cols * (2.0 * n.Rb - n.cols) * n.K, st);
   }
   const OzTriPair& q = c->oz_chol_q;
   if (!c->oz_chol_ready || q.h != pl.split_h) return fail(c, GPE_ERR_STATE, "internal error: split Cholesky without an int8 plan");
   if (with_aug) CHK(launch_gemm_range(c, pl.launches[pl.aug_mid], st));
   const long long ld = F.n_pad;
-  oz_operand(st, c->oz_c, q.l21(F.A + (long long)q.h * TILE, ld), q.Pb, q.Pa, c->dozx, c->dozp);
+  oz_operand(st, c->oz_c, q.l21(F.A + (long long)q.h * TILE, ld), q.Pb, q.Pa, c->dozx, c->dozp, oz_sums(c));
   HIPCHK(c, hipGetLastError());
   const OzShape s = q.shape_schur();
   const OzOpnd l21{c->dozp, (long long)q.Pb * q.Pa, q.Pa, 0};
   CHK(oz_gemm_crt(c, c->oz_c,
                   OzProduct{s, l21, l21, c->dozl + c->oz_chol_loff, c->oz_chol_llen, c->dozr, s.res_bytes(),
-                            OzOut{c->dozx, c->dozx, F.A + (long long)q.h * TILE * (ld + 1), ld, q.Rb, q.Rb, 1, -1.0, 1}},
+                            OzOut{c->dozx, c->dozx, F.A + (long long)q.h * TILE * (ld + 1), ld, q.Rb, q.Rb, 1, -1.0, 1},
+                            oz_cert(c, c->dozs, q.Pb, c->dozs, q.Pb)},
                   c->oz_chol_ops, (double)q.Rb * q.Rb * q.Ra, st));
   c->oz_l21_valid = true;
   return GPE_OK;
@@ -1049,12 +1082,13 @@
   CHK(oz_prepare(c, F));
   const int np = (int)F.n_pad, np2 = c->oz_np2;
   c->oz_l21_valid = false;
-  oz_operand_packed(c->stream, c->oz_c, F.B, (long long)F.n_pad, np, np2, c->dozx, c->dozp);
+  oz_operand_packed(c->stream, c->oz_c, F.B, (long long)F.n_pad, np, np2, c->dozx, c->dozp, oz_sums(c));
   const OzShape s = oz_lauum_shape(np2);
   const OzOpnd x{c->dozp, oz_plane_bytes(np2), 0, np2};
   return oz_gemm_crt(c, c->oz_c,
                      OzProduct{s, x, x, c->dozl, c->oz_list_len, c->dozr, s.res_bytes(),
-                               OzOut{c->dozx, c->dozx, F.A, (long long)F.n_pad, np, np, 1, 1.0}},
+                               OzOut{c->dozx, c->dozx, F.A, (long long)F.n_pad, np, np, 1, 1.0},
+                               oz_cert(c, c->dozs, np2, c->dozs, np2)},
                      c->oz_lauum_ops, (double)np * np * np / 3.0);
 }
 
@@ -1067,7 +1101,7 @@
 int oz_l21(gpe_ctx* c, Fact& F, const OzTriPair& q, hipStream_t st) {
   c->oz_l21_valid = false;
   oz_operand(st, c->oz_c, q.l21(F.A + (long long)q.h * TILE + (long long)q.t0 * TILE * F.n_pad, F.n_pad), q.Pb, q.Pa,
-             c->dozx, c->dozp);
+             c->dozx, c->dozp, oz_sums(c));
   HIPCHK(c, hipGetLastError());
   return GPE_OK;
 }
@@ -1097,7 +1131,10 @@
                        tile(F.B, h, t0), ld, c->dozt, c->dozp, c->dozr, c->dozx, l21 != 0,
                        [&](const OzProduct& p, double ops, double fl) {
                          if (rc == GPE_OK) rc = oz_gemm_crt(c, c->oz_c, p, ops, fl);
-                       }, part);
+                       }, part, oz_sums(c),
+                       [&](const unsigned long long* sa, int na, const unsigned long long* sb, int nb) {
+                         return oz_cert(c, sa, na, sb, nb);
+                       });
   CHK(rc);
   HIPCHK(c, hipGetLastError());
   return GPE_OK;
@@ -1196,6 +1233,8 @@
     if (const char* ec = std::getenv("GPEMU_OZAKI_CHOL_MIN")) c->oz_chol_min = std::max(256, std::atoi(ec));
     if (const char* ec = std::getenv("GPEMU_OZAKI_CHOL_NEST")) c->oz_nest = std::atoi(ec) != 0;
     if (const char* ec = std::getenv("GPEMU_OZAKI_CHOL_NEST_MIN")) c->oz_nest_min = std::max(256, std::atoi(ec));
+    if (const char* ec = std::getenv("GPEMU_OZAKI_CERT")) c->oz_cert_on = std::atoi(ec) != 0;
+    if (const char* ec = std::getenv("GPEMU_OZAKI_CERT_MIN_NP")) c->oz_cert_min_np = std::max(512, std::atoi(ec));
     if (const char* ea = std::getenv("GPEMU_TRTRI_AHEAD")) c->tri_ahead_on = std::atoi(ea) != 0;
     if (const char* es = std::getenv("GPEMU_POTRF_SB")) {
       c->sched.sb = std::max(1, std::min(8, std::atoi(es)));
@@ -1287,6 +1326,9 @@
   if (c->dozp) hipFree(c->dozp);
   if (c->dozr) hipFree(c->dozr);
   if (c->dozx) hipFree(c->dozx);
+  if (c->dozs) hipFree(c->dozs);
+  if (c->dozf) hipFree(c->dozf);
+  if (c->dozm) hipFree(c->dozm);
   if (c->dozl) hipFree(c->dozl);
   if (c->dozt) hipFree(c->dozt);
   if (c->ev_oz) hipEventDestroy(c->ev_oz);
@@ -1391,6 +1433,40 @@
   return GPE_OK;
 }
 
+int gpe_oz_cert_stats(gpe_ctx* c, int32_t* products_out, int32_t* certified_out) {
+  if (!c) return GPE_ERR_ARG;
+  HIPCHK(c, hipSetDevice(c->device));
+  int cert = 0;
+  if (c->oz_cert_used > 0) {
+    std::vector<int> fl((size_t)c->oz_cert_used);
+    HIPCHK(c, hipStreamSynchronize(c->stream));
+    HIPCHK(c, hipStreamSynchronize(c->stream2));
+    HIPCHK(c, hipMemcpy(fl.data(), c->dozf, fl.size() * sizeof(int), hipMemcpyDeviceToHost));
+    for (const int f : fl) cert += f != 0;
+  }
+  if (products_out) *products_out = c->oz_cert_used;
+  if (certified_out) *certified_out = cert;
+  return GPE_OK;
+}
+
+int gpe_oz_cert_sums(gpe_ctx* c, int32_t cap, uint64_t* a_out, uint64_t* b_out) {
+  if (!c) return GPE_ERR_ARG;
+  if (cap < 0 || (cap > 0 && (!a_out || !b_out))) return fail(c, GPE_ERR_ARG, "gpe_oz_cert_sums: NULL output");
+  HIPCHK(c, hipSetDevice(c->device));
+  const int n = std::min((int)cap, c->oz_cert_used);
+  if (n > 0) {
+    std::vector<unsigned long long> m(2 * (size_t)n);
+    HIPCHK(c, hipStreamSynchronize(c->stream));
+    HIPCHK(c, hipStreamSynchronize(c->stream2));
+    HIPCHK(c, hipMemcpy(m.data(), c->dozm, m.size() * sizeof(unsigned long long), hipMemcpyDeviceToHost));
+    for (int i = 0; i < n; ++i) {
+      a_out[i] = m[2 * (size_t)i];
+      b_out[i] = m[2 * (size_t)i + 1];
+    }
+  }
+  return GPE_OK;
+}
+
 int gpe_gemm_stats(gpe_ctx* c, double* ms_out, double* launches_out, double* flops_out) {
   if (!c) return GPE_ERR_ARG;
   if (ms_out) *ms_out = c->gemm_ms;
@@ -1539,6 +1615,13 @@
     g += ms;
   }
   c->oz_ms = g;
+  if (!c->oz_cert_ops.empty()) {
+    std::vector<int> fl((size_t)c->oz_flag_cap);
+    HIPCHK(c, hipMemcpy(fl.data(), c->dozf, fl.size() * sizeof(int), hipMemcpyDeviceToHost));
+    for (const auto& po : c->oz_cert_ops)
+      if (fl[(size_t)po.first]) c->oz_ops -= po.second / OZ_MAXMOD;
+    c->oz_cert_ops.clear();
+  }
   return GPE_OK;
 }
 
@@ -1566,6 +1649,7 @@
     c->gemm_launches = c->gemm_flops = c->gemm_ms = 0.0;
     c->oev_used = 0;
     c->oz_ms = c->oz_launches = c->oz_ops = c->oz_flops64 = 0.0;
+    c->oz_cert_ops.clear();
   }
   const bool one_launch = c->tiny;
   if (one_launch && c->NB == 1 && d <= TINY_DM && q + 1 <= TINY_DM)
@@ -1677,6 +1761,7 @@
     c->gemm_launches = c->gemm_flops = c->gemm_ms = 0.0;
     c->oev_used = 0;
     c->oz_ms = c->oz_launches = c->oz_ops = c->oz_flops64 = 0.0;
+    c->oz_cert_ops.clear();
   }
   const Cols cols{c->dFm, P, c->dZm};
   CHK(factor_and_invert(c, kernel, hp, o.nu, o.s2, o.rscale, want_grad != 0, true, &cols));
@@ -3352,8 +3437,11 @@
   int *exa = nullptr, *exb = nullptr;
   int8_t *pa = nullptr, *pb = nullptr, *res = nullptr;
   unsigned* list = nullptr;
+  unsigned long long *suma = nullptr, *sumb = nullptr;
+  int* flag = nullptr;
   ~OzTestBufs() {
-    for (void* p : {(void*)sa, (void*)sb, (void*)C, (void*)exa, (void*)exb, (void*)pa, (void*)pb, (void*)res, (void*)list})
+    for (void* p : {(void*)sa, (void*)sb, (void*)C, (void*)exa, (void*)exb, (void*)pa, (void*)pb, (void*)res, (void*)list,
+                    (void*)suma, (void*)sumb, (void*)flag})
       if (p) (void)hipFree(p);
   }
 };
@@ -3365,20 +3453,24 @@
 }
 
 static int oz_test_operand(gpe_ctx* c, const gpe_oz_operand& o, const OzConst& k, int P, int Kp, double** dsrc, int** dex,
-                           int8_t** dpl) {
+                           int8_t** dpl, unsigned long long** dsum = nullptr) {
+  if (dsum) CHK(dalloc(c, dsum, (size_t)P));
   CHK(dalloc(c, dsrc, (size_t)o.len));
   CHK(dalloc(c, dex, (size_t)P));
   CHK(dalloc(c, dpl, (size_t)k.nmod * P * Kp));
   HIPCHK(c, hipMemcpy(*dsrc, o.src, (size_t)o.len * sizeof(double), hipMemcpyHostToDevice));
-  oz_operand(c->stream, k, OzSrc{*dsrc + o.offset, (long long)o.ld, o.R, o.Kv, o.mask, o.trans != 0}, P, Kp, *dex, *dpl);
+  oz_operand(c->stream, k, OzSrc{*dsrc + o.offset, (long long)o.ld, o.R, o.Kv, o.mask, o.trans != 0}, P, Kp, *dex, *dpl,
+             dsum ? *dsum : nullptr);
   HIPCHK(c, hipGetLastError());
   return GPE_OK;
 }
 
 static int oz_test_product(gpe_ctx* c, const gpe_oz_operand& a, const gpe_oz_operand* b, gpe_oz_params p, double* C,
-                           int32_t* exa_out, int32_t* exb_out, int8_t* res_out) {
+                           int32_t* exa_out, int32_t* exb_out, int8_t* res_out, int32_t* nmod_used_out = nullptr) {
   const auto bad = [&](const char* what) { return fail(c, GPE_ERR_ARG, std::string("gpe_test_oz_product: ") + what); };
   if (p.nmod < 6 || p.nmod > OZ_MAXMOD) return bad("nmod outside [6, 16]");
+  const bool cert = nmod_used_out != nullptr;
+  if (cert && p.nmod != OZ_MAXMOD) return bad("a certificate needs nmod = 16");
   if (res_out && (p.res_mod < 0 || p.res_mod >= p.nmod)) return bad("res_mod is not a modulus number");
   if (a.R < 1 || a.R > (1 << 20)) return bad("bad operand rows");
   const int Pa = (a.R + OZ_T - 1) / OZ_T * OZ_T;
@@ -3407,6 +3499,7 @@
     return bad("C too small for rows x cols at ldc");
   const int K = p.K, ti0 = p.ti0, nti = Pa / OZ_T - ti0, ntj = Pb / OZ_T;
   const OzConst k = oz_consts(p.nmod, K);
+  const OzConst k15 = oz_consts_cert(K);
   const OzShape s{nti, p.tri ? (Pb < Pa ? ntj : 0) : ntj, ti0, p.tri ? 1 : 0, K, p.kbeg, p.kend, p.kdiv};
   OzTestBufs d;
   hipStream_t st = c->stream;
@@ -3415,15 +3508,16 @@
     CHK(dalloc(c, &d.sa, (size_t)a.len));
     CHK(dalloc(c, &d.exa, (size_t)Pa));
     CHK(dalloc(c, &d.pa, (size_t)k.nmod * oz_plane_bytes(Pa)));
+    if (cert) CHK(dalloc(c, &d.suma, (size_t)Pa));
     HIPCHK(c, hipMemcpy(d.sa, a.src, (size_t)a.len * sizeof(double), hipMemcpyHostToDevice));
-    oz_operand_packed(st, k, d.sa + a.offset, (long long)a.ld, a.R, Pa, d.exa, d.pa);
+    oz_operand_packed(st, k, d.sa + a.offset, (long long)a.ld, a.R, Pa, d.exa, d.pa, d.suma);
     HIPCHK(c, hipGetLastError());
     oa = ob = OzOpnd{d.pa, oz_plane_bytes(Pa), 0, Pa};
   } else {
-    CHK(oz_test_operand(c, a, k, Pa, K, &d.sa, &d.exa, &d.pa));
+    CHK(oz_test_operand(c, a, k, Pa, K, &d.sa, &d.exa, &d.pa, cert ? &d.suma : nullptr));
     oa = ob = OzOpnd{d.pa, (long long)Pa * K, K, 0};
     if (b) {
-      CHK(oz_test_operand(c, *b, k, Pb, K, &d.sb, &d.exb, &d.pb));
+      CHK(oz_test_operand(c, *b, k, Pb, K, &d.sb, &d.exb, &d.pb, cert ? &d.sumb : nullptr));
       ob = OzOpnd{d.pb, (long long)Pb * K, K, 0};
     }
   }
@@ -3436,8 +3530,19 @@
   HIPCHK(c, hipMemcpy(d.C, C, (size_t)p.c_len * sizeof(double), hipMemcpyHostToDevice));
   HIPCHK(c, hipMemsetAsync(d.res, 0, (size_t)k.nmod * rb, st));
   const OzOut out{d.exa, b ? d.exb : d.exa, d.C, (long long)p.ldc, p.rows, p.cols, p.lower128 ? 1 : 0, p.alpha, p.acc ? 1 : 0};
-  CHK(oz_gemm_crt(c, k, OzProduct{s, oa, ob, d.list, (int)list.size(), d.res, rb, out}, 0.0, 0.0));
+  OzCert ct{};
+  if (cert) {
+    CHK(dalloc(c, &d.flag, (size_t)1));
+    HIPCHK(c, hipMemsetAsync(d.flag, 0, sizeof(int), st));
+    ct = OzCert{d.suma, Pa, b ? d.sumb : d.suma, Pb, d.flag, &k15};
+  }
+  CHK(oz_gemm_crt(c, k, OzProduct{s, oa, ob, d.list, (int)list.size(), d.res, rb, out, ct}, 0.0, 0.0));
   HIPCHK(c, hipStreamSynchronize(st));
+  if (cert) {
+    int fl = 0;
+    HIPCHK(c, hipMemcpy(&fl, d.flag, sizeof(int), hipMemcpyDeviceToHost));
+    *nmod_used_out = fl ? OZ_CERT_NMOD : OZ_MAXMOD;
+  }
   HIPCHK(c, hipMemcpy(C, d.C, (size_t)p.c_len * sizeof(double), hipMemcpyDeviceToHost));
   if (exa_out) HIPCHK(c, hipMemcpy(exa_out, d.exa, (size_t)Pa * sizeof(int), hipMemcpyDeviceToHost));
   if (exb_out) HIPCHK(c, hipMemcpy(exb_out, b ? d.exb : d.exa, (size_t)Pb * sizeof(int), hipMemcpyDeviceToHost));
@@ -3468,6 +3573,18 @@
   const bool prof = c->prof;
   c->prof = false;
   const int rc = oz_test_product(c, *a, b, *p, C, exa_out, exb_out, res_out);
+  c->prof = prof;
+  return rc;
+}
+
+int gpe_test_oz_product_cert(gpe_ctx* c, const gpe_oz_operand* a, const gpe_oz_operand* b, const gpe_oz_params* p, double* C,
+                             int32_t* exa_out, int32_t* exb_out, int8_t* res_out, int32_t* nmod_used_out) {
+  if (!c) return GPE_ERR_ARG;
+  if (!a || !p || !nmod_used_out) return fail(c, GPE_ERR_ARG, "gpe_test_oz_product_cert: NULL operand, parameters or nmod_used_out");
+  HIPCHK(c, hipSetDevice(c->device));
+  const bool prof = c->prof;
+  c->prof = false;
+  const int rc = oz_test_product(c, *a, b, *p, C, exa_out, exb_out, res_out, nmod_used_out);
   c->prof = prof;
   return rc;
 }
diff --git a/gp_emu_uqsa_amd/csrc/gpemu_ozaki.hpp b/gp_emu_uqsa_amd/csrc/gpemu_ozaki.hpp
--- a/gp_emu_uqsa_amd/csrc/gpemu_ozaki.hpp
+++ b/gp_emu_uqsa_amd/csrc/gpemu_ozaki.hpp
@@ -27,6 +27,7 @@
   double rhi[OZ_MAXMOD];
   double rlo[OZ_MAXMOD];
   double Md;
+  double Mlo;
   int nmod;
   int beta;
 };
@@ -108,31 +109,89 @@
   return make_uint2(oz_pack4(v[0], v[1], v[2], v[3]), oz_pack4(v[4], v[5], v[6], v[7]));
 }
 
+constexpr int OZ_CERT_NMOD = OZ_MAXMOD - 1;
+constexpr unsigned long long OZ_T15_HI = 0x1b24e222aafull, OZ_T15_LO = 0xd866408f6fe8ec7eull;
+__host__ __device__ __forceinline__ unsigned long long oz_cert_term(double xr) {
+  const unsigned y = (unsigned)(fabs(xr) * 0x1p-32) + 1u;
+  return (unsigned long long)y * y;
+}
+__host__ __device__ inline bool oz_cert_ok(unsigned long long A, unsigned long long B) {
+  const unsigned long long a0 = A & 0xffffffffull, a1 = A >> 32, b0 = B & 0xffffffffull, b1 = B >> 32;
+  const unsigned long long p00 = a0 * b0, p01 = a0 * b1, p10 = a1 * b0, p11 = a1 * b1;
+  const unsigned long long mid = (p00 >> 32) + (p01 & 0xffffffffull) + (p10 & 0xffffffffull);
+  const unsigned long long lo = (p00 & 0xffffffffull) | (mid << 32);
+  const unsigned long long hi = p11 + (p01 >> 32) + (p10 >> 32) + (mid >> 32);
+  return hi < OZ_T15_HI || (hi == OZ_T15_HI && lo < OZ_T15_LO);
+}
+__device__ __forceinline__ void oz_cert_block_add(unsigned long long v, unsigned long long* __restrict__ sum, int r) {
+  __shared__ unsigned long long part[4];
+  for (int off = 32; off > 0; off >>= 1) v += __shfl_xor(v, off, 64);
+  if ((threadIdx.x & 63) == 0) part[threadIdx.x >> 6] = v;
+  __syncthreads();
+  if (threadIdx.x == 0) {
+    v = part[0] + part[1] + part[2] + part[3];
+    if (v) atomicAdd(sum + r, v);
+  }
+}
+static __global__ void __launch_bounds__(256) k_oz_cert(const unsigned long long* __restrict__ sa, int na,
+                                                        const unsigned long long* __restrict__ sb, int nb,
+                                                        int* __restrict__ flag, unsigned long long* __restrict__ mx) {
+  __shared__ unsigned long long pa[4], pb[4];
+  unsigned long long A = 0, B = 0;
+  for (int r = threadIdx.x; r < na; r += 256) A = sa[r] > A ? sa[r] : A;
+  for (int r = threadIdx.x; r < nb; r += 256) B = sb[r] > B ? sb[r] : B;
+  for (int off = 32; off > 0; off >>= 1) {
+    const unsigned long long oa = __shfl_xor(A, off, 64), ob = __shfl_xor(B, off, 64);
+    A = oa > A ? oa : A;
+    B = ob > B ? ob : B;
+  }
+  if ((threadIdx.x & 63) == 0) {
+    pa[threadIdx.x >> 6] = A;
+    pb[threadIdx.x >> 6] = B;
+  }
+  __syncthreads();
+  if (threadIdx.x == 0) {
+    for (int w = 1; w < 4; ++w) {
+      A = pa[w] > A ? pa[w] : A;
+      B = pb[w] > B ? pb[w] : B;
+    }
+    *flag = oz_cert_ok(A, B) ? 1 : 0;
+    if (mx) {
+      mx[0] = A;
+      mx[1] = B;
+    }
+  }
+}
+
 static __global__ void __launch_bounds__(256) k_oz_colexp(const double* __restrict__ X, long long ldx, int np,
-                                                          int np2, int beta, int* __restrict__ ex) {
+                                                          int np2, int beta, int* __restrict__ ex,
+                                                          unsigned long long* __restrict__ sum) {
   const int lane = threadIdx.x & 63, j = blockIdx.x * 4 + (threadIdx.x >> 6);
   if (j >= np2) return;
   double mx = 0.0;
   if (j < np)
     for (int k = j + lane; k < np; k += 64) mx = oz_pmax(mx, fabs(X[k + (long long)j * ldx]));
   for (int off = 32; off > 0; off >>= 1) mx = oz_pmax(mx, __shfl_xor(mx, off, 64));
-  if (lane == 0) ex[j] = oz_ex_of(mx, beta);
+  if (lane == 0) {
+    ex[j] = oz_ex_of(mx, beta);
+    if (sum) sum[j] = 0ull;
+  }
 }
 
 constexpr int OZ_SPLIT_ROWS = 8;
-static __global__ void __launch_bounds__(256) k_oz_split(const double* __restrict__ X, long long ldx, int np,
-                                                         int np2, const int* __restrict__ ex, int8_t* __restrict__ planes,
-                                                         long long plane_bytes, OzConst cst) {
-  const int j = blockIdx.x;
+template <bool CERT>
+__device__ __forceinline__ unsigned long long oz_split_thread(const double* __restrict__ X, long long ldx, int np, int np2,
+                                                              const int* __restrict__ ex, int8_t* __restrict__ planes,
+                                                              long long plane_bytes, const OzConst& cst, int j) {
   const int cb = j / OZ_T, r0 = cb * OZ_T;
   const int k0 = r0 + OZ_SPLIT_ROWS * ((int)blockIdx.y * 256 + (int)threadIdx.x);
-  if (k0 >= np2) return;
+  if (k0 >= np2) return 0ull;
   const int e = ex[j];
   const long long ld = np2 - r0;
   int8_t* dst = planes + oz_panel_off(cb, np2) + (long long)(j - r0) * ld + (k0 - r0);
   if (j >= np || k0 >= np || k0 + OZ_SPLIT_ROWS <= j || e == OZ_EX_NAN) {
     for (int l = 0; l < cst.nmod; ++l) *reinterpret_cast<uint2*>(dst + (long long)l * plane_bytes) = make_uint2(0u, 0u);
-    return;
+    return 0ull;
   }
   double xs[OZ_SPLIT_ROWS];
   if (k0 + OZ_SPLIT_ROWS <= np && k0 >= j) {
@@ -150,9 +209,23 @@
     }
   }
   OzDigits d[OZ_SPLIT_ROWS];
-#pragma unroll
-  for (int u = 0; u < OZ_SPLIT_ROWS; ++u) d[u] = oz_digits(rint(ldexp(xs[u], e)));
+  unsigned long long s = 0ull;
+#pragma unroll
+  for (int u = 0; u < OZ_SPLIT_ROWS; ++u) {
+    const double xr = rint(ldexp(xs[u], e));
+    d[u] = oz_digits(xr);
+    if constexpr (CERT) s += oz_cert_term(xr);
+  }
   for (int l = 0; l < cst.nmod; ++l) *reinterpret_cast<uint2*>(dst + (long long)l * plane_bytes) = oz_residues8(d, cst, l);
+  return s;
+}
+static __global__ void __launch_bounds__(256) k_oz_split(const double* __restrict__ X, long long ldx, int np,
+                                                         int np2, const int* __restrict__ ex, int8_t* __restrict__ planes,
+                                                         long long plane_bytes, OzConst cst,
+                                                         unsigned long long* __restrict__ sum) {
+  const int j = blockIdx.x;
+  if (sum) oz_cert_block_add(oz_split_thread<true>(X, ldx, np, np2, ex, planes, plane_bytes, cst, j), sum, j);
+  else oz_split_thread<false>(X, ldx, np, np2, ex, planes, plane_bytes, cst, j);
 }
 
 __device__ __forceinline__ void oz_glds16(const int8_t* src, int8_t* dst) {
@@ -191,6 +264,7 @@
   long long res_bytes;
   int kdiv = 1;
   int ti0 = 0;
+  const int* flag = nullptr;
 };
 __host__ __device__ __forceinline__ long long oz_res_tile(int tri, int ntj, int ti, int tj) {
   if (!tri) return (long long)ti * ntj + tj;
@@ -246,6 +320,7 @@
   extern __shared__ __attribute__((aligned(16))) double lds_d[];
   int8_t* lds = reinterpret_cast<int8_t*>(lds_d);
   const int l = (int)blockIdx.x / g.list_len;
+  if (l == OZ_CERT_NMOD && g.flag && *g.flag) return;
   const unsigned ent = g.list[(int)blockIdx.x - l * g.list_len];
   if (ent == 0xffffffffu) return;
   const int ti = (int)(ent >> 16), tj = (int)(ent & 0xffffu);
@@ -380,8 +455,8 @@
   int ti0 = 0;
   int acc = 0;
 };
-template <int NM>
-static __global__ void __launch_bounds__(256) k_oz_crt(OzCrt g, OzConst cst) {
+template <int NM, bool M2 = false>
+__device__ __forceinline__ void oz_crt_entries(const OzCrt& g, const OzConst& cst) {
   const int nmod = NM ? NM : cst.nmod;
   const int t = (int)blockIdx.x >> 4;
   const int u = ((int)blockIdx.x & 15) * 256 + (int)threadIdx.x;
@@ -437,7 +512,7 @@
         slo[r] = fma(cv, rl, slo[r]);
       }
     }
-  const double sc = g.alpha * cst.Md;
+  const double sc = g.alpha * cst.Md, scl = g.alpha * cst.Mlo;
 #pragma unroll
   for (int r = 0; r < 16; ++r) {
     const int gn = gn0 + (r & 3) + 8 * (r >> 2);
@@ -446,9 +521,31 @@
     const int en = ec[r >> 2][r & 3];
     double* dst = g.C + (gm - OZ_T * g.ti0 + (long long)gn * g.ldc);
     const double s = ldexp(sc, -(em + en));
-    if (em == OZ_EX_NAN || en == OZ_EX_NAN) *dst = __builtin_nan("");
-    else *dst = g.acc ? fma(v, s, *dst) : v * s;
-  }
+    if (em == OZ_EX_NAN || en == OZ_EX_NAN) {
+      *dst = __builtin_nan("");
+    } else if constexpr (M2) {
+      const double sl = ldexp(scl, -(em + en));
+      if (g.acc) {
+        const double c0 = *dst;
+        const double p = __dmul_rn(v, s), pe = fma(v, sl, fma(v, s, -p));
+        const double t = __dadd_rn(c0, p), bb = __dsub_rn(t, c0);
+        const double err = __dadd_rn(__dsub_rn(c0, __dsub_rn(t, bb)), __dsub_rn(p, bb));
+        *dst = __dadd_rn(t, __dadd_rn(err, pe));
+      } else {
+        *dst = fma(v, s, v * sl);
+      }
+    } else {
+      *dst = g.acc ? fma(v, s, *dst) : v * s;
+    }
+  }
+}
+template <int NM>
+static __global__ void __launch_bounds__(256) k_oz_crt(OzCrt g, OzConst cst) {
+  oz_crt_entries<NM>(g, cst);
+}
+static __global__ void __launch_bounds__(256) k_oz_crt_cert(OzCrt g, OzConst cst, OzConst c15, const int* __restrict__ flag) {
+  if (*flag) oz_crt_entries<OZ_CERT_NMOD, true>(g, c15);
+  else oz_crt_entries<OZ_MAXMOD>(g, cst);
 }
 
 __device__ __forceinline__ bool oz_keep(int mask, int r, int k) {
@@ -457,7 +554,8 @@
 
 template <bool TRANS>
 static __global__ void __launch_bounds__(256) k_oz_rowexp(const double* __restrict__ src, long long ld, int R, int Rp,
-                                                          int Kv, int mask, int beta, int* __restrict__ ex) {
+                                                          int Kv, int mask, int beta, int* __restrict__ ex,
+                                                          unsigned long long* __restrict__ sum) {
   if constexpr (!TRANS) {
     const int lane = threadIdx.x & 63, r = blockIdx.x * 4 + (threadIdx.x >> 6);
     if (r >= Rp) return;
@@ -466,7 +564,10 @@
       for (int k = lane; k < Kv; k += 64)
         if (oz_keep(mask, r, k)) mx = oz_pmax(mx, fabs(src[k + (long long)r * ld]));
     for (int off = 32; off > 0; off >>= 1) mx = oz_pmax(mx, __shfl_xor(mx, off, 64));
-    if (lane == 0) ex[r] = oz_ex_of(mx, beta);
+    if (lane == 0) {
+      ex[r] = oz_ex_of(mx, beta);
+      if (sum) sum[r] = 0ull;
+    }
   } else {
     __shared__ double red[4][64];
     const int rl = threadIdx.x & 63, q = threadIdx.x >> 6, r = blockIdx.x * 64 + rl;
@@ -487,20 +588,26 @@
     }
   }
 }
-static __global__ void __launch_bounds__(256) k_oz_il_to_ex(int* __restrict__ ex, int Rp, int beta) {
+static __global__ void __launch_bounds__(256) k_oz_il_to_ex(int* __restrict__ ex, int Rp, int beta,
+                                                            unsigned long long* __restrict__ sum) {
   const int r = blockIdx.x * 256 + threadIdx.x;
-  if (r < Rp) ex[r] = ex[r] >= OZ_IL_BAD ? OZ_EX_NAN : (ex[r] > 0 ? (beta - 1) - (ex[r] - 2048) : 0);
+  if (r < Rp) {
+    ex[r] = ex[r] >= OZ_IL_BAD ? OZ_EX_NAN : (ex[r] > 0 ? (beta - 1) - (ex[r] - 2048) : 0);
+    if (sum) sum[r] = 0ull;
+  }
 }
 
 template <bool TRANS>
 static __global__ void __launch_bounds__(256) k_oz_split_rect(const double* __restrict__ src, long long ld, int R,
                                                               int Kv, int mask, const int* __restrict__ ex,
                                                               int8_t* __restrict__ planes, long long plane_bytes,
-                                                              long long ldp, int Kp, OzConst cst) {
+                                                              long long ldp, int Kp, OzConst cst,
+                                                              unsigned long long* __restrict__ sum) {
   if constexpr (!TRANS) {
     const int r = blockIdx.x;
+    const auto thread8 = [&]() -> unsigned long long {
     const int k0 = ((int)blockIdx.y * 256 + (int)threadIdx.x) * 8;
-    if (k0 >= Kp) return;
+    if (k0 >= Kp) return 0ull;
     const int e = ex[r];
     const double* p = src + k0 + (long long)r * ld;
     const int side = mask == 1 ? (k0 >= r ? 1 : (k0 + 7 < r ? 0 : 2))
@@ -508,7 +615,7 @@
     int8_t* dst = planes + (long long)r * ldp + k0;
     if (side == 0 || r >= R || k0 >= Kv || e == OZ_EX_NAN) {
       for (int l = 0; l < cst.nmod; ++l) *reinterpret_cast<uint2*>(dst + (long long)l * plane_bytes) = make_uint2(0u, 0u);
-      return;
+      return 0ull;
     }
     double xs[8];
     if (k0 + 8 <= Kv && side == 1 && ((reinterpret_cast<uintptr_t>(p) & 15) == 0)) {
@@ -526,9 +633,18 @@
       }
     }
     OzDigits d[8];
-#pragma unroll
-    for (int u = 0; u < 8; ++u) d[u] = oz_digits(rint(ldexp(xs[u], e)));
+    unsigned long long s = 0ull;
+#pragma unroll
+    for (int u = 0; u < 8; ++u) {
+      const double xr = rint(ldexp(xs[u], e));
+      d[u] = oz_digits(xr);
+      if (sum) s += oz_cert_term(xr);
+    }
     for (int l = 0; l < cst.nmod; ++l) *reinterpret_cast<uint2*>(dst + (long long)l * plane_bytes) = oz_residues8(d, cst, l);
+    return s;
+    };
+    const unsigned long long s = thread8();
+    if (sum) oz_cert_block_add(s, sum, r);
   } else {
     constexpr int PL = 4;
     __shared__ __attribute__((aligned(16))) unsigned tr[PL][64 * 20];
@@ -566,10 +682,29 @@
       x1[u] = oz_keep(mask, r + 1, k) ? b : 0.0;
     }
     OzDigits d0[8], d1[8];
+    unsigned long long s0 = 0ull, s1 = 0ull;
 #pragma unroll
     for (int u = 0; u < 8; ++u) {
-      d0[u] = oz_digits(e0 == OZ_EX_NAN ? 0.0 : rint(ldexp(x0[u], e0)));
-      d1[u] = oz_digits(e1 == OZ_EX_NAN ? 0.0 : rint(ldexp(x1[u], e1)));
+      const double xr0 = e0 == OZ_EX_NAN ? 0.0 : rint(ldexp(x0[u], e0));
+      const double xr1 = e1 == OZ_EX_NAN ? 0.0 : rint(ldexp(x1[u], e1));
+      d0[u] = oz_digits(xr0);
+      d1[u] = oz_digits(xr1);
+      if (sum) {
+        s0 += oz_cert_term(xr0);
+        s1 += oz_cert_term(xr1);
+      }
+    }
+    if (sum) {
+      __shared__ unsigned long long rs[8][64];
+      rs[kg][2 * rp] = s0;
+      rs[kg][2 * rp + 1] = s1;
+      __syncthreads();
+      if (threadIdx.x < 64) {
+        unsigned long long t = 0ull;
+#pragma unroll
+        for (int q = 0; q < 8; ++q) t += rs[q][threadIdx.x];
+        atomicAdd(sum + (long long)blockIdx.x * 64 + threadIdx.x, t);
+      }
     }
     for (int l0 = 0; l0 < cst.nmod; l0 += PL) {
       if (l0 > 0) __syncthreads();
@@ -623,6 +758,16 @@
     k.rhi[l] = std::ldexp((double)Q, -41);
     k.rlo[l] = std::ldexp((double)R / (double)m, -41);
   }
+  return k;
+}
+
+inline OzConst oz_consts_cert(int np2) {
+  OzConst k = oz_consts(OZ_CERT_NMOD, np2);
+  const OzConst k16 = oz_consts(OZ_MAXMOD, np2);
+  const double last = (double)k16.m[OZ_CERT_NMOD];
+  k.beta = k16.beta;
+  k.Md = k16.Md / last;
+  k.Mlo = std::fma(-k.Md, last, k16.Md) / last;
   return k;
 }
 
@@ -673,33 +818,37 @@
   int R, Kv, mask;
   bool trans;
 };
-inline void oz_operand_exp(hipStream_t st, const OzConst& k, const OzSrc& o, int P, int* ex) {
+inline void oz_operand_exp(hipStream_t st, const OzConst& k, const OzSrc& o, int P, int* ex,
+                           unsigned long long* sum = nullptr) {
   if (o.trans) {
     (void)hipMemsetAsync(ex, 0, (size_t)P * sizeof(int), st);
     hipLaunchKernelGGL(k_oz_rowexp<true>, dim3(P / 64, (o.Kv + 255) / 256), dim3(256), 0, st, o.src, o.ld, o.R, P, o.Kv,
-                       o.mask, k.beta, ex);
-    hipLaunchKernelGGL(k_oz_il_to_ex, dim3((P + 255) / 256), dim3(256), 0, st, ex, P, k.beta);
+                       o.mask, k.beta, ex, sum);
+    hipLaunchKernelGGL(k_oz_il_to_ex, dim3((P + 255) / 256), dim3(256), 0, st, ex, P, k.beta, sum);
   } else {
-    hipLaunchKernelGGL(k_oz_rowexp<false>, dim3(P / 4), dim3(256), 0, st, o.src, o.ld, o.R, P, o.Kv, o.mask, k.beta, ex);
-  }
-}
-inline void oz_operand_split(hipStream_t st, const OzConst& k, const OzSrc& o, int P, int Kp, const int* ex, int8_t* planes) {
+    hipLaunchKernelGGL(k_oz_rowexp<false>, dim3(P / 4), dim3(256), 0, st, o.src, o.ld, o.R, P, o.Kv, o.mask, k.beta, ex,
+                       sum);
+  }
+}
+inline void oz_operand_split(hipStream_t st, const OzConst& k, const OzSrc& o, int P, int Kp, const int* ex, int8_t* planes,
+                             unsigned long long* sum = nullptr) {
   if (o.trans)
     hipLaunchKernelGGL(k_oz_split_rect<true>, dim3(P / 64, Kp / 64), dim3(256), 0, st, o.src, o.ld, o.R, o.Kv, o.mask, ex,
-                       planes, (long long)P * Kp, (long long)Kp, Kp, k);
+                       planes, (long long)P * Kp, (long long)Kp, Kp, k, sum);
   else
     hipLaunchKernelGGL(k_oz_split_rect<false>, dim3(P, (Kp + 2047) / 2048), dim3(256), 0, st, o.src, o.ld, o.R, o.Kv,
-                       o.mask, ex, planes, (long long)P * Kp, (long long)Kp, Kp, k);
-}
-inline void oz_operand(hipStream_t st, const OzConst& k, const OzSrc& o, int P, int Kp, int* ex, int8_t* planes) {
-  oz_operand_exp(st, k, o, P, ex);
-  oz_operand_split(st, k, o, P, Kp, ex, planes);
+                       o.mask, ex, planes, (long long)P * Kp, (long long)Kp, Kp, k, sum);
+}
+inline void oz_operand(hipStream_t st, const OzConst& k, const OzSrc& o, int P, int Kp, int* ex, int8_t* planes,
+                       unsigned long long* sum = nullptr) {
+  oz_operand_exp(st, k, o, P, ex, sum);
+  oz_operand_split(st, k, o, P, Kp, ex, planes, sum);
 }
 inline void oz_operand_packed(hipStream_t st, const OzConst& k, const double* X, long long ldx, int np, int np2, int* ex,
-                              int8_t* planes) {
-  hipLaunchKernelGGL(k_oz_colexp, dim3((np2 + 3) / 4), dim3(256), 0, st, X, ldx, np, np2, k.beta, ex);
+                              int8_t* planes, unsigned long long* sum = nullptr) {
+  hipLaunchKernelGGL(k_oz_colexp, dim3((np2 + 3) / 4), dim3(256), 0, st, X, ldx, np, np2, k.beta, ex, sum);
   hipLaunchKernelGGL(k_oz_split, dim3(np2, (np2 + 256 * OZ_SPLIT_ROWS - 1) / (256 * OZ_SPLIT_ROWS)), dim3(256), 0, st, X,
-                     ldx, np, np2, ex, planes, oz_plane_bytes(np2), k);
+                     ldx, np, np2, ex, planes, oz_plane_bytes(np2), k, sum);
 }
 
 struct OzShape {
@@ -741,6 +890,15 @@
   double alpha;
   int acc = 0;
 };
+struct OzCert {
+  const unsigned long long* sa = nullptr;
+  int na = 0;
+  const unsigned long long* sb = nullptr;
+  int nb = 0;
+  int* flag = nullptr;
+  const OzConst* c15 = nullptr;
+  unsigned long long* maxima = nullptr;
+};
 struct OzProduct {
   OzShape s;
   OzOpnd a, b;
@@ -749,19 +907,26 @@
   int8_t* res;
   long long res_bytes;
   OzOut out;
+  OzCert cert{};
 };
 inline hipError_t oz_product_launch(hipStream_t st, const OzConst& k, const OzProduct& p, hipEvent_t e0 = nullptr,
                                     hipEvent_t e1 = nullptr) {
   const OzShape& s = p.s;
   const int ntj = s.ntj;
-  const OzGemm g{p.a, p.b, p.list, p.list_len, s.K, s.kbeg, s.kend, s.tri, ntj, p.res, p.res_bytes, s.kdiv, s.ti0};
+  const OzCert& ct = p.cert;
+  const bool cert = ct.flag && ct.c15 && k.nmod == OZ_MAXMOD;
+  const OzGemm g{p.a, p.b, p.list, p.list_len, s.K, s.kbeg, s.kend, s.tri, ntj, p.res, p.res_bytes, s.kdiv, s.ti0,
+                 cert ? ct.flag : nullptr};
   const OzOut& o = p.out;
   const OzCrt r{p.res, p.res_bytes, s.tri, ntj, o.exr, o.exc, o.C, o.ldc, o.rows, o.cols, o.lower128, o.alpha, s.ti0, o.acc};
   hipError_t e;
+  if (cert) hipLaunchKernelGGL(k_oz_cert, dim3(1), dim3(256), 0, st, ct.sa, ct.na, ct.sb, ct.nb, ct.flag,
+                             ct.maxima);
   if (e0 && (e = hipEventRecord(e0, st)) != hipSuccess) return e;
   hipLaunchKernelGGL(k_oz_gemm, dim3((unsigned)(k.nmod * g.list_len)), dim3(256), OZ_LDS, st, g, k);
   if (e1 && (e = hipEventRecord(e1, st)) != hipSuccess) return e;
-  if (k.nmod == OZ_MAXMOD) hipLaunchKernelGGL(k_oz_crt<OZ_MAXMOD>, dim3((unsigned)(s.tiles() * 16)), dim3(256), 0, st, r, k);
+  if (cert) hipLaunchKernelGGL(k_oz_crt_cert, dim3((unsigned)(s.tiles() * 16)), dim3(256), 0, st, r, k, *ct.c15, ct.flag);
+  else if (k.nmod == OZ_MAXMOD) hipLaunchKernelGGL(k_oz_crt<OZ_MAXMOD>, dim3((unsigned)(s.tiles() * 16)), dim3(256), 0, st, r, k);
   else hipLaunchKernelGGL(k_oz_crt<0>, dim3((unsigned)(s.tiles() * 16)), dim3(256), 0, st, r, k);
   return hipGetLastError();
 }
@@ -831,35 +996,45 @@
   return n;
 }
 
-template <class GC>
+template <class GC, class CT>
 void oz_tri_pair_launches(hipStream_t st, const OzConst& k, const OzTriPair& q, const unsigned* lists, const double* L21,
                           const double* X11, const double* X22, double* X21, long long ld, double* T, int8_t* planes,
-                          int8_t* res, int* ex, bool l21_done, GC gc, int part = 0) {
+                          int8_t* res, int* ex, bool l21_done, GC gc, int part, unsigned long long* sum, CT cert) {
   int* exA = ex;
   int* exB = ex + q.Pb;
+  unsigned long long* sA = sum;
+  unsigned long long* sB = sum ? sum + q.Pb : nullptr;
   int8_t* PA = planes;
   const long long rb = q.shape_a().res_bytes();
   if (part != 2) {
     const long long pA = (long long)q.Pb * q.Pa, pB = (long long)q.Pa * q.Pa;
     int8_t* PB = planes + (size_t)k.nmod * pA;
-    if (!l21_done) oz_operand(st, k, q.l21(L21, ld), q.Pb, q.Pa, exA, PA);
-    oz_operand(st, k, OzSrc{X11, ld, q.Ra, q.Ra, 1, false}, q.Pa, q.Pa, exB, PB);
+    if (!l21_done) oz_operand(st, k, q.l21(L21, ld), q.Pb, q.Pa, exA, PA, sA);
+    oz_operand(st, k, OzSrc{X11, ld, q.Ra, q.Ra, 1, false}, q.Pa, q.Pa, exB, PB, sB);
     gc(OzProduct{q.shape_a(), OzOpnd{PA, pA, q.Pa, 0}, OzOpnd{PB, pB, q.Pa, 0}, lists + q.la_off, q.la_len, res, rb,
-                 OzOut{exA, exB, T, (long long)q.Pb, q.Rb, q.Ra, 0, 1.0}},
+                 OzOut{exA, exB, T, (long long)q.Pb, q.Rb, q.Ra, 0, 1.0}, sum ? cert(sA, q.Pb, sB, q.Pa) : OzCert{}},
        q.ops_a, (double)q.Ra * q.Ra * q.Rb);
   }
   if (part != 1) {
     const long long pA = (long long)q.Pb * q.Pb, pB = (long long)q.Pa * q.Pb;
     int8_t* PB = planes + (size_t)k.nmod * pA;
     const OzSrc x22{X22, ld, q.Rb, q.Rb, 2, true}, t{T, (long long)q.Pb, q.Ra, q.Rb, 0, false};
-    oz_operand_exp(st, k, x22, q.Pb, exA);
-    oz_operand_exp(st, k, t, q.Pa, exB);
-    oz_operand_split(st, k, x22, q.Pb, q.Pb, exA, PA);
-    oz_operand_split(st, k, t, q.Pa, q.Pb, exB, PB);
+    oz_operand_exp(st, k, x22, q.Pb, exA, sA);
+    oz_operand_exp(st, k, t, q.Pa, exB, sB);
+    oz_operand_split(st, k, x22, q.Pb, q.Pb, exA, PA, sA);
+    oz_operand_split(st, k, t, q.Pa, q.Pb, exB, PB, sB);
     gc(OzProduct{q.shape_b(), OzOpnd{PA, pA, q.Pb, 0}, OzOpnd{PB, pB, q.Pb, 0}, lists + q.lb_off, q.lb_len, res, rb,
-                 OzOut{exA, exB, X21, ld, q.Rb, q.Ra, 0, -1.0}},
+                 OzOut{exA, exB, X21, ld, q.Rb, q.Ra, 0, -1.0}, sum ? cert(sA, q.Pb, sB, q.Pa) : OzCert{}},
        q.ops_b, (double)q.Rb * q.Rb * q.Ra);
   }
 }
 
-}
+template <class GC>
+void oz_tri_pair_launches(hipStream_t st, const OzConst& k, const OzTriPair& q, const unsigned* lists, const double* L21,
+                          const double* X11, const double* X22, double* X21, long long ld, double* T, int8_t* planes,
+                          int8_t* res, int* ex, bool l21_done, GC gc, int part = 0) {
+  oz_tri_pair_launches(st, k, q, lists, L21, X11, X22, X21, ld, T, planes, res, ex, l21_done, gc, part, nullptr,
+                       [](const unsigned long long*, int, const unsigned long long*, int) { return OzCert{}; });
+}
+
+}
diff --git a/gp_emu_uqsa_amd/native.py b/gp_emu_uqsa_amd/native.py
--- a/gp_emu_uqsa_amd/native.py
+++ b/gp_emu_uqsa_amd/native.py
@@ -55,6 +55,10 @@
     "gpe_test_oz_product": (_ct.c_int, [_VP, _ct.POINTER(OzOperand), _ct.POINTER(OzOperand),
                                         _ct.POINTER(OzParams), _D, _ct.POINTER(_ct.c_int32),
                                         _ct.POINTER(_ct.c_int32), _ct.POINTER(_ct.c_int8)]),
+    "gpe_test_oz_product_cert": (_ct.c_int, [_VP, _ct.POINTER(OzOperand), _ct.POINTER(OzOperand),
+                                             _ct.POINTER(OzParams), _D, _ct.POINTER(_ct.c_int32),
+                                             _ct.POINTER(_ct.c_int32), _ct.POINTER(_ct.c_int8),
+                                             _ct.POINTER(_ct.c_int32)]),
     "gpe_test_oz_planes": (_ct.c_int, [_VP, _ct.POINTER(OzOperand), _ct.c_int32, _ct.c_int32, _ct.c_int32,
                                        _ct.POINTER(_ct.c_int32), _ct.POINTER(_ct.c_int8)]),
     "gpe_abi_version": (_ct.c_int, []),
@@ -117,6 +121,8 @@
     "gpe_phase_times": (_ct.c_int, [_VP, _D, _ct.c_int32]),
     "gpe_gemm_stats": (_ct.c_int, [_VP, _D, _D, _D]),
     "gpe_ozaki_stats": (_ct.c_int, [_VP, _D, _D, _D, _D]),
+    "gpe_oz_cert_stats": (_ct.c_int, [_VP, _ct.POINTER(_ct.c_int32), _ct.POINTER(_ct.c_int32)]),
+    "gpe_oz_cert_sums": (_ct.c_int, [_VP, _ct.c_int32, _ct.POINTER(_ct.c_uint64), _ct.POINTER(_ct.c_uint64)]),
     "gpe_dist_unique_id": (_ct.c_int, [_ct.c_char_p, _ct.c_int32]),
     "gpe_dist_create": (_VP, [_ct.c_int32, _ct.c_int32, _ct.c_int32, _ct.c_char_p]),
     "gpe_dist_destroy": (None, [_VP]),
@@ -598,7 +604,7 @@
 
     def test_oz_product(self, a, b=None, *, C, ldc, packed=False, K=0, kbeg=0, kend=0, kdiv=1, ti0=0,
                         tri=False, lower128=False, alpha=1.0, acc=False, nmod=16, rows=0, cols=0,
-                        res_mod=None):
+                        res_mod=None, cert=False):
         keep = []
 
         def opnd(o):
@@ -620,10 +626,14 @@
         exb = _np.zeros(max(Pb, 1), dtype=_np.int32)
         res = None if res_mod is None else _np.zeros((max(Pa - 256 * int(ti0), 1), max(Pb, 1)), dtype=_np.int8)
         i32 = _ct.POINTER(_ct.c_int32)
-        self._check(self.lib.gpe_test_oz_product(
-            self._h, _ct.byref(oa), _ct.byref(ob) if ob is not None else None, _ct.byref(p), _ptr(Cc),
-            exa.ctypes.data_as(i32), exb.ctypes.data_as(i32),
-            None if res is None else res.ctypes.data_as(_ct.POINTER(_ct.c_int8))), "gpe_test_oz_product")
+        args = (self._h, _ct.byref(oa), _ct.byref(ob) if ob is not None else None, _ct.byref(p), _ptr(Cc),
+                exa.ctypes.data_as(i32), exb.ctypes.data_as(i32),
+                None if res is None else res.ctypes.data_as(_ct.POINTER(_ct.c_int8)))
+        if cert:
+            used = _ct.c_int32(0)
+            self._check(self.lib.gpe_test_oz_product_cert(*args, _ct.byref(used)), "gpe_test_oz_product_cert")
+            return {"C": Cc, "exa": exa, "exb": exb, "res": res, "nmod_used": used.value}
+        self._check(self.lib.gpe_test_oz_product(*args), "gpe_test_oz_product")
         return {"C": Cc, "exa": exa, "exb": exb, "res": res}
 
     def test_oz_planes(self, a, *, packed=False, K=0, nmod=16):
@@ -691,6 +701,19 @@
                     "gpe_ozaki_stats")
         return {"ms": ms.value, "launches": nl.value, "int8_ops": ops.value, "fp64_flops": fl.value}
 
+    def oz_cert_stats(self):
+        n, k = _ct.c_int32(0), _ct.c_int32(0)
+        self._check(self.lib.gpe_oz_cert_stats(self._h, _ct.byref(n), _ct.byref(k)), "gpe_oz_cert_stats")
+        return {"products": n.value, "certified": k.value}
+
+    def oz_cert_sums(self):
+        n = self.oz_cert_stats()["products"]
+        a, b = _np.zeros(max(n, 1), dtype=_np.uint64), _np.zeros(max(n, 1), dtype=_np.uint64)
+        u64 = _ct.POINTER(_ct.c_uint64)
+        self._check(self.lib.gpe_oz_cert_sums(self._h, n, a.ctypes.data_as(u64), b.ctypes.data_as(u64)),
+                    "gpe_oz_cert_sums")
+        return [(int(a[i]), int(b[i])) for i in range(n)]
+
 
 _default_ctx = None
 _ctx_lock = _threading.Lock()
diff --git a/include/gpemu.h b/include/gpemu.h
--- a/include/gpemu.h
+++ b/include/gpemu.h
@@ -142,6 +142,10 @@
 int gpe_test_oz_product(gpe_ctx* ctx, const gpe_oz_operand* a, const gpe_oz_operand* b,
                         const gpe_oz_params* p, double* C, int32_t* exa_out, int32_t* exb_out,
                         int8_t* res_out);
+
+int gpe_test_oz_product_cert(gpe_ctx* ctx, const gpe_oz_operand* a, const gpe_oz_operand* b,
+                             const gpe_oz_params* p, double* C, int32_t* exa_out, int32_t* exb_out,
+                             int8_t* res_out, int32_t* nmod_used_out);
 
 int gpe_test_oz_planes(gpe_ctx* ctx, const gpe_oz_operand* a, int32_t packed, int32_t K,
                        int32_t nmod, int32_t* ex_out, int8_t* planes_out);
@@ -189,6 +193,10 @@
 int gpe_ozaki_stats(gpe_ctx* ctx, double* ms_out, double* launches_out, double* int8_ops_out,
                     double* fp64_flops_out);
 
+int gpe_oz_cert_stats(gpe_ctx* ctx, int32_t* products_out, int32_t* certified_out);
+
+int gpe_oz_cert_sums(gpe_ctx* ctx, int32_t cap, uint64_t* a_out, uint64_t* b_out);
+
 #ifdef __cplusplus
 }
 #endif
```

Result: faster. 20.53, median of 6 (+3.6%).
